# IvanIZ/BenchPush

Hardware: AMD Instinct MI355X
Metric: env-steps/sec at N=4096 envs (ship-ice-v0), 1/2/4/8 MI355X (higher is better)
Workload: dtype f64

## Files before the change

benchpush_amd/csrc/bp_capi.hip:

```cpp
#include <hip/hip_runtime.h>

#include <cstdio>
#include <cstdlib>
#include <algorithm>
#include <cstring>
#include <map>
#include <mutex>
#include <string>
#include <vector>

#include <fcntl.h>
#include <sys/file.h>
#include <sys/stat.h>
#include <unistd.h>

#include "bp_host_bd.hpp"
#include "bp_boxdelivery.hpp"
#include "bp_policy.hpp"
#include "bp_render.hpp"
#include "bp_state.hpp"
#include "bp_swath.hpp"
#include "bp_lattice.hpp"
#include "bp_track.hpp"
#include "bp_rrt.hpp"
#include "bp_gtsp.hpp"
#include "bp_asyncq.hpp"
#include "bp_replay.hpp"

typedef void (*StepKernel)(const DevParams, const DevPtrs, const double *, double *, unsigned char *, unsigned char *, double *);
typedef void (*ResidentKernel)(const DevParams *, const DevPtrs *, const double *, double *, unsigned char *, unsigned char *, double *);
typedef void (*ResetKernel)(const DevParams, const DevPtrs, const unsigned char *, double *, const int);
struct RigidKernels {
    StepKernel step = nullptr;
    StepKernel sched = nullptr;
    ResidentKernel resident = nullptr;
    ResetKernel reset = nullptr;
};

struct bp_handle {
    bp_config cfg;
    int num_envs = 0;
    long long env_offset = 0;
    int device = 0;
    int nbcap = 0;
    int num_trials = 0;
    bool loaded = false, was_reset = false;
    int *order_buf = nullptr;
    bool steps_done = false;
    bool resettle = false;
    bool damp = false;
    RigidKernels k;
    BpLaunchPolicy pol = {};
    int pair_mode = 0;
    int pair_resident = 0;
    int sched_persist = 0;
    void *pd_buf = nullptr;
    int sched_chunk = 0;
    std::string dev_lock_key;
    bool resident_auto = false;
    bool device_shared = false;
    unsigned launches = 0;
    int num_cus = 0;
    hipStream_t st_aux = nullptr;
    hipStream_t st_aux2 = nullptr;
    hipEvent_t ev_fork = nullptr, ev_join = nullptr, ev_join2 = nullptr;
    hipStream_t st_aux3 = nullptr;
    hipEvent_t ev_join3 = nullptr;
    int bd_budget = 0;
    bool async_open = false;
    int as_epoch = 0;
    int q_batch = 0;
    BdQueue q = {};
    DevParams P;
    DevPtrs D;
    std::vector<void *> allocs;
    size_t lds_bytes = 0, obs_lds_bytes = 0;
    size_t sched_lds = 0;
    std::string err;
    std::vector<double> goal_raw;
    bp_bd_config bdcfg;
    BdParams B;
    BdPtrs Q;
    size_t bd_rmap_lds = 0;
    size_t bd_lds = 0, bd_obs_lds = 0;
    std::vector<bpgeom::BdMaps> bd_maps;
    std::vector<int> bd_map_of_trial;
    bool timing = false;
    std::vector<hipEvent_t> ev;
    size_t ev_used = 0;
    unsigned long long *cost_ring = nullptr;
    int cost_n = 0;
    int *r_order = nullptr;
    unsigned *r_rgb = nullptr;
    bp_render_prim *r_prims = nullptr;
    int r_nunder = 0, r_nover = 0;
    bool r_table = false;
    unsigned long long scen_hash = 0xCBF29CE484222325ull;
    BpStateLayout st_layout;
    BpStateSeg *st_table = nullptr;
    unsigned long long st_layout_id = 0;
};
#define BP_COST_RING 1024

static int fail(bp_handle *h, int code, const std::string &msg)
{
    if (h) h->err = msg;
    return code;
}
#define HIPCHK(h, call)                                                                                       \
    do {                                                                                                      \
        hipError_t _e = (call);                                                                               \
        if (_e != hipSuccess) return fail((h), BP_EHIP, std::string(#call) + ": " + hipGetErrorString(_e));    \
    } while (0)

struct DevGuard {
    int prev = -1;
    bool changed = false, ok = true;
    explicit DevGuard(int d)
    {
        if (hipGetDevice(&prev) != hipSuccess) prev = -1;
        if (prev != d) { ok = hipSetDevice(d) == hipSuccess; changed = ok; }
    }
    ~DevGuard() { if (changed && prev >= 0) (void)hipSetDevice(prev); }
};
#define BP_DEVICE(h) DevGuard _dg((h)->device); if (!_dg.ok) return fail((h), BP_EHIP, "hipSetDevice failed")

template <typename T>
static int dalloc(bp_handle *h, T **p, size_t n, int fill_byte = 0)
{
    void *q = nullptr;
    const size_t bytes = (n ? n : 1) * sizeof(T);
    hipError_t e = hipMalloc(&q, bytes);
    if (e != hipSuccess) return fail(h, BP_ENOMEM, std::string("hipMalloc: ") + hipGetErrorString(e));
    e = hipMemset(q, fill_byte, bytes);
    if (e != hipSuccess) return fail(h, BP_EHIP, std::string("hipMemset: ") + hipGetErrorString(e));
    h->allocs.push_back(q);
    *p = (T *)q;
    return BP_OK;
}

struct DevTable { const void *src; size_t bytes; void *dev; };
template <typename T>
static DevTable dev_table(const std::vector<T> &v) { return {v.data(), sizeof(T) * v.size(), nullptr}; }
static int upload_tables(bp_handle *h, DevTable *tab, int n)
{
    for (int k = 0; k < n; k++) {
        unsigned char *q;
        if (int rc = dalloc(h, &q, tab[k].bytes)) return rc;
        tab[k].dev = q;
    }
    for (int k = 0; k < n; k++) HIPCHK(h, hipMemcpy(tab[k].dev, tab[k].src, tab[k].bytes, hipMemcpyHostToDevice));
    return BP_OK;
}

static int mvcap_for(int nbcap) { return nbcap > 192 ? nbcap : 192; }
#ifdef BP_PROF
#define BP_PROF_HOST true
#else
#define BP_PROF_HOST false
#endif
static size_t lds_bytes_for(int nbcap, bool box) { return bp_lds_map(nbcap, mvcap_for(nbcap), box, BP_PROF_HOST).total; }

static unsigned sched_yield_mask(bool solo_launch, int steps, int chunk)
{
    if (const char *ev = getenv("BP_SCHED_YMASK")) return (unsigned)strtoul(ev, nullptr, 0);
    if (!solo_launch || chunk <= 0) return 0xFFFFFFFFu;
    const int first = (2 * steps + 5 * chunk - 1) / (5 * chunk);
    return first >= 32 ? 0u : (0xFFFFFFFFu << first);
}
static int sched_image_setup(bp_handle *h)
{
    const int want = getenv("BP_SCHED_IMAGE") ? atoi(getenv("BP_SCHED_IMAGE")) : 0;
    h->P.sq_image = 0; h->D.sq_img = nullptr;
    if (!want || h->P.pair_mode == 2) return BP_OK;
    h->P.sq_img_lds = (unsigned)h->sched_lds;
    h->P.sq_img_stride = bp_img_bytes(h->P.sq_img_lds);
    unsigned char *d_img;
    int rc = dalloc(h, &d_img, (size_t)h->num_envs * h->P.sq_img_stride);
    if (rc) return rc;
    h->D.sq_img = d_img; h->P.sq_image = 1;
    return BP_OK;
}
struct ResidentLock { int fd = -1; int refs = 0; };
static std::mutex g_res_mu;
static std::map<std::string, ResidentLock> g_res_locks;

static void resident_acquire(bp_handle *h)
{
    char bus[64] = {0};
    if (hipDeviceGetPCIBusId(bus, (int)sizeof(bus), h->device) != hipSuccess) return;
    for (char *c = bus; *c; c++) if (*c == ':' || *c == '/' || *c == '.') *c = '_';
    const char *dir = getenv("BP_LOCK_DIR");
    const std::string key = std::string(dir ? dir : "/tmp") + "/benchpush_amd.resident." + bus + ".lock";
    std::lock_guard<std::mutex> g(g_res_mu);
    ResidentLock &L = g_res_locks[key];
    if (L.fd < 0) {
        const mode_t um = umask(0);
        L.fd = open(key.c_str(), O_RDWR | O_CREAT | O_CLOEXEC, 0666);
        umask(um);
        if (L.fd < 0) { g_res_locks.erase(key); return; }
// ... 215 lines not shown
    if ((rc = dalloc(h, &D.wv, EB * BP_MAXV))) return rc;
    if ((rc = dalloc(h, &D.wn, EB * BP_MAXV))) return rc;
    if ((rc = dalloc(h, &D.pv, EB * BP_MAXV))) return rc;
    if ((rc = dalloc(h, &D.bb, EB))) return rc;
    if ((rc = dalloc(h, &D.fat, EB))) return rc;
    if ((rc = dalloc(h, &D.adj, EB * BP_KADJ))) return rc;
    if ((rc = dalloc(h, &D.adjn, EB))) return rc;
    if ((rc = dalloc(h, &D.hint, EB * BP_KADJ))) return rc;
    if ((rc = dalloc(h, &D.a_key, E * BP_ACAP, 0xFF))) return rc;
    if ((rc = dalloc(h, &D.a_stamp, E * BP_ACAP))) return rc;
    if ((rc = dalloc(h, &D.a_sc, E * BP_ACAP))) return rc;
    if ((rc = dalloc(h, &D.a_h0, E * BP_ACAP))) return rc;
    if ((rc = dalloc(h, &D.a_h1, E * BP_ACAP))) return rc;
    if ((rc = dalloc(h, &D.a_d, E * BP_ACAP * 14))) return rc;
    if ((rc = dalloc(h, &D.e_lastrew, E))) return rc;
    if ((rc = dalloc(h, &D.e_lastflag, E))) return rc;
    if ((rc = dalloc(h, &D.m_acc, E * 8))) return rc;
    if ((rc = dalloc(h, &D.m_rows, E * BP_EPM_COUNT))) return rc;
    if ((rc = dalloc(h, &D.m_ring, E * BP_EPM_RING * BP_EPM_COUNT))) return rc;
    if ((rc = dalloc(h, &D.m_sum, E * BP_EPM_COUNT))) return rc;
    if ((rc = dalloc(h, &D.m_count, E))) return rc;
    if ((rc = dalloc(h, &D.m_open, E))) return rc;
    if ((rc = dalloc(h, &D.clk, (size_t)16))) return rc;
    HIPCHK(h, hipMemset(D.clk, 0, 16 * sizeof(unsigned long long)));
    D.dbg = nullptr; D.dbg_env = -1; D.prof = nullptr;
    return BP_OK;
}
static void pair_limits(bp_handle *h)
{
    auto envint = [](const char *name, int dflt) { const char *v = getenv(name); return v ? atoi(v) : dflt; };
    h->P.pair_mode = 2;
    BpLaunchPolicy &pol = h->pol;
    if (pol.pair_mode != 2)
        bp_policy_pair_limits(pol, 2LL * h->num_envs < (long long)BP_POLICY_LOOSE_FROM_HALF_ROUNDS * pol.wave_slots, h->num_envs);
    h->P.pair_solo = std::min(h->num_envs, std::max(0, envint("BP_PAIR_SOLO", pol.pair_solo)));
    h->P.pp_max_keys = std::min(30, envint("BP_PP_KEYS", 26));
    h->P.pp_max_slots = std::min(PP_NSLOT - 4, envint("BP_PP_SLOTS", 34));
    h->P.pp_max_mv = std::min(PP_MVCAP - 4, envint("BP_PP_MV", 40));
    h->P.pp_max_act = envint("BP_PP_ACT", pol.pp_max_act);
    h->P.pp_max_work = envint("BP_PP_WORK", pol.pp_max_work);
    h->P.pp_rate = envint("BP_PP_RATE", pol.pp_rate);
    h->P.pp_snake = envint("BP_PP_SNAKE", 0);
    h->P.pp_heavy_only = envint("BP_PP_HEAVY_ONLY", 0);
}
static int pair_resident_setup(bp_handle *h)
{
    HIPCHK(h, hipFuncSetAttribute((const void *)k_physics_step_schedr, hipFuncAttributeMaxDynamicSharedMemorySize, (int)h->sched_lds));
    const int pr = getenv("BP_PAIR_RESIDENT") ? atoi(getenv("BP_PAIR_RESIDENT")) : 1;
    if (pr > 0) {
        h->pair_resident = std::min(h->num_envs, h->pol.wave_slots * pr);
        if (!h->pd_buf) HIPCHK(h, hipMalloc(&h->pd_buf, sizeof(DevParams) + sizeof(DevPtrs)));
        if (!getenv("BP_PAIR_RESIDENT")) { h->resident_auto = true; resident_acquire(h); h->device_shared = resident_device_shared(h); }
    }
    return BP_OK;
}
static int sched_setup(bp_handle *h, bool maze)
{
    int rc;
    int ch = h->pol.chunk ? h->pol.chunk : (h->pair_mode == 2 ? 100 : 0);
    if (const char *ev = getenv("BP_SCHED")) ch = atoi(ev);
    if (!(ch > 0 && (h->P.steps + ch - 1) / ch <= SQ_MAXLEV && h->num_envs < (1 << 24))) return BP_OK;
    h->sched_chunk = ch;
    h->P.sq_chunk = ch; h->P.sq_levels = (h->P.steps + ch - 1) / ch;
    if (!maze) {
        h->P.sq_hold = 0;
        h->P.sq_lrpt = 0;
        h->P.sq_bw = 9000;
        h->P.sq_hyst = 1;
        h->P.sq_floor = 150;
        h->P.sq_cls = 0;
        h->P.sq_parts = 1;
        h->P.sq_part = 0;
    }
    h->P.sq_dynprio = getenv("BP_SCHED_DYNPRIO") ? atoi(getenv("BP_SCHED_DYNPRIO")) : 115;
    h->P.sq_cap = h->num_envs;
    int *d_items, *d_ctr; unsigned *d_carry; unsigned char *d_moved;
    if ((rc = dalloc(h, &d_items, (size_t)SQ_NX * SQ_MAXLEV * h->P.sq_cap))) return rc;
    if ((rc = dalloc(h, &d_ctr, (size_t)SQ_NX * (SQ_MAXLEV + 2) * 2))) return rc;
    if ((rc = dalloc(h, &d_carry, (size_t)h->num_envs * 4))) return rc;
    if ((rc = dalloc(h, &d_moved, (size_t)h->num_envs * h->nbcap))) return rc;
    h->D.sq_items = d_items; h->D.sq_ctr = d_ctr; h->D.sq_carry = d_carry; h->D.sq_moved = d_moved;
    int *d_done, *d_lev, *d_warn, *d_resc;
    if ((rc = dalloc(h, &d_resc, (size_t)1 + SQ_RESCUE))) return rc;
    h->D.sq_rescue = d_resc;
    if ((rc = dalloc(h, &d_done, (size_t)h->num_envs))) return rc;
    if ((rc = dalloc(h, &d_lev, (size_t)h->num_envs))) return rc;
    if ((rc = dalloc(h, &d_warn, (size_t)2))) return rc;
    HIPCHK(h, hipMemset(d_warn, 0, 2 * sizeof(int)));
    h->D.sq_done = d_done; h->D.sq_lev = d_lev; h->D.sq_warn = d_warn;
    unsigned *d_thr;
    if ((rc = dalloc(h, &d_thr, (size_t)1))) return rc;
    HIPCHK(h, hipMemset(d_thr, 0xFF, sizeof(unsigned)));
    h->D.sq_thr = d_thr;
    int *d_sub;
    if ((rc = dalloc(h, &d_sub, (size_t)h->num_envs))) return rc;
    h->D.sq_sub = d_sub;
    if (!maze) {
        int *d_pst;
        if ((rc = dalloc(h, &d_pst, (size_t)8))) return rc;
        HIPCHK(h, hipMemset(d_pst, 0, 8 * sizeof(int)));
        h->D.sq_pairstat = d_pst;
    }
#ifdef BP_DEBUG_PATHS
    if (const char *ev2 = getenv("BP_SCHED_DEBUG_DROP")) h->P.sq_debug = atoi(ev2);
#endif
    if (h->pair_mode == 2) pair_limits(h);
    h->sched_lds = h->pair_mode == 2 ? std::max(h->lds_bytes, (size_t)(2 * PL_HALF)) : h->lds_bytes;
    h->P.sq_ymask = sched_yield_mask(h->P.pair_mode != 2, h->P.steps, h->P.sq_chunk);
    if ((rc = sched_image_setup(h))) return rc;
    if (maze) {
        HIPCHK(h, hipFuncSetAttribute((const void *)k_physics_step_sched_maze, hipFuncAttributeMaxDynamicSharedMemorySize, (int)h->sched_lds));
        HIPCHK(h, hipFuncSetAttribute((const void *)k_physics_step_schedl_maze, hipFuncAttributeMaxDynamicSharedMemorySize, (int)h->sched_lds));
    } else {
        HIPCHK(h, hipFuncSetAttribute((const void *)k_physics_step_sched, hipFuncAttributeMaxDynamicSharedMemorySize, (int)h->sched_lds));
        HIPCHK(h, hipFuncSetAttribute((const void *)k_physics_step_schedp, hipFuncAttributeMaxDynamicSharedMemorySize, (int)h->sched_lds));
        HIPCHK(h, hipFuncSetAttribute((const void *)k_physics_step_schedl, hipFuncAttributeMaxDynamicSharedMemorySize, (int)h->sched_lds));
    }
    return h->P.pair_mode == 2 ? pair_resident_setup(h) : sched_persist_setup(h);
}
static int ship_plan(bp_handle *h, const std::vector<std::vector<bpgeom::Shape>> &trials)
{
    const int T = (int)trials.size(), nbcap = h->nbcap;
    bool plain = true;
    for (int t = 0; t < T && plain; t++)
        for (int b = 0; b < (int)trials[t].size(); b++) {
            const int kd = trials[t][b].kind;
            const int bt = (kd >> 16) & 3, grp = (kd >> 8) & 0xFF;
            if (grp != 0 || bt != (b == 0 ? 1 : 0)) { plain = false; break; }
        }
    const bool can_pair = plain && nbcap <= PP_NBCAP &&
                          ((size_t)h->num_envs + (size_t)T) * (size_t)nbcap * BP_MAXV * sizeof(d2) < (size_t)0xFFFFFFFF &&
                          ((size_t)h->num_envs + (size_t)T) * (size_t)nbcap * BP_KADJ * sizeof(unsigned long long) < (size_t)0xFFFFFFFF;
    if (int rc = device_cus(h)) return rc;
    h->pol = bp_launch_policy(h->num_envs, h->num_cus, can_pair, false);
    h->pair_mode = h->pol.pair_mode;
    if (const char *evp = getenv("BP_PAIR")) h->pair_mode = can_pair ? atoi(evp) : 0;
    if (h->pair_mode == 1) {
        h->P.pair_mode = 1;
        if (const char *evs = getenv("BP_PAIR_SNAKE")) h->P.pair_solo = atoi(evs);
        HIPCHK(h, hipFuncSetAttribute((const void *)k_physics_step_pair, hipFuncAttributeMaxDynamicSharedMemorySize, (int)(2 * PL_HALF)));
    }
    if (plain) { if (int rc = sched_setup(h, false)) return rc; }
    if (h->pair_mode == 2 && h->P.pair_mode != 2) h->pair_mode = 0;
    return BP_OK;
}
static RigidKernels rigid_kernels(const bp_handle *h, bool maze8)
{
    RigidKernels k;
    if (h->damp) { k.step = k_physics_step_damp; k.reset = k_physics_reset_damp; }
    else if (maze8) { k.step = k_physics_step_maze; k.sched = k_physics_step_sched_maze; k.resident = k_physics_step_schedl_maze; k.reset = k_physics_reset_maze; }
    else { k.step = k_physics_step; k.sched = k_physics_step_sched; k.resident = h->P.pair_mode == 2 ? k_physics_step_schedr : k_physics_step_schedl; k.reset = k_physics_reset; }
    return k;
}
static int settle_templates(bp_handle *h)
{
    hipLaunchKernelGGL(h->k.reset, dim3(h->num_trials), dim3(64), h->lds_bytes, 0, h->P, h->D, (const unsigned char *)nullptr, (double *)nullptr, 1);
    HIPCHK(h, hipGetLastError());
    HIPCHK(h, hipDeviceSynchronize());
    h->loaded = true;
    return BP_OK;
}
static int upload_trials(bp_handle *h, const std::vector<std::vector<bpgeom::Shape>> &trials, bool settle = true)
{
    const int T = (int)trials.size();
    int maxnb = 1;
    for (const auto &b : trials) maxnb = std::max(maxnb, (int)b.size());
    if (maxnb > 60000) return fail(h, BP_EINVAL, "too many bodies");
    const int nbcap = (maxnb + 7) / 8 * 8;
    h->nbcap = nbcap;
    h->num_trials = T;
    h->P.nbcap = nbcap;
    h->P.mvcap = mvcap_for(nbcap);
    h->P.num_trials = T;
    h->lds_bytes = lds_bytes_for(nbcap, h->P.env_kind == BP_ENV_BOX);
    if (h->lds_bytes > 160 * 1024) return fail(h, BP_EINVAL, "nb_cap too large for LDS");
    if (nbcap >= (1 << BP_CC_IDX_BITS)) return fail(h, BP_EINVAL, "nb_cap exceeds the candidate cache's body-index field (16384 bodies per env)");
    int rc;
    TrialTables tt;
    if ((rc = pack_trials(h, trials, nbcap, tt))) return rc;
    if ((rc = upload_trial_tables(h, tt))) return rc;
    if ((rc = alloc_env_state(h, T))) return rc;
    HIPCHK(h, hipDeviceSynchronize());
    HIPCHK(h, hipFuncSetAttribute((const void *)k_physics_step, hipFuncAttributeMaxDynamicSharedMemorySize, (int)h->lds_bytes));
    HIPCHK(h, hipFuncSetAttribute((const void *)k_physics_reset, hipFuncAttributeMaxDynamicSharedMemorySize, (int)h->lds_bytes));
    h->damp = h->P.damping_pow != 0.0;
    if (h->damp) {
        HIPCHK(h, hipFuncSetAttribute((const void *)k_physics_step_damp, hipFuncAttributeMaxDynamicSharedMemorySize, (int)h->lds_bytes));
        HIPCHK(h, hipFuncSetAttribute((const void *)k_physics_reset_damp, hipFuncAttributeMaxDynamicSharedMemorySize, (int)h->lds_bytes));
    } else if (h->P.env_kind == BP_ENV_SHIP_ICE && h->P.nkin == 1 && nbcap < 16384) {
        if ((rc = ship_plan(h, trials))) return rc;
    }
    if (!settle) return BP_OK;
    bool maze8 = !h->damp && h->P.env_kind == BP_ENV_MAZE;
    for (int v : tt.nv) if (v > 8) maze8 = false;
    if (maze8) {
        if ((rc = device_cus(h))) return rc;
        h->pol = bp_launch_policy(h->num_envs, h->num_cus, false, true);
        if ((rc = sched_setup(h, true))) return rc;
        HIPCHK(h, hipFuncSetAttribute((const void *)k_physics_step_maze, hipFuncAttributeMaxDynamicSharedMemorySize, (int)h->lds_bytes));
        HIPCHK(h, hipFuncSetAttribute((const void *)k_physics_reset_maze, hipFuncAttributeMaxDynamicSharedMemorySize, (int)h->lds_bytes));
    }
    h->k = rigid_kernels(h, maze8);
    return settle_templates(h);
}

static int state_setup(bp_handle *h)
{
    const bool box = h->P.env_kind == BP_ENV_BOX;
    const int cells = box ? h->B.SH * h->B.SW : 0;
    h->st_layout = bp_state_layout(h->D, h->Q, h->nbcap, box, cells);
    const BpStateLayout &L = h->st_layout;
    if (L.nseg >= BP_STATE_MAXSEG || (L.bytes >> 4) >= 0xFFFFFFFFull) return fail(h, BP_EINVAL, "state record layout out of range");
    unsigned long long id = bp_state_structure_id(L, h->P.env_kind, box ? h->bdcfg.task : 0, h->nbcap, cells);
    if (box) id = bp_fnv1a(&h->bdcfg, sizeof(h->bdcfg), id);
    else id = bp_fnv1a(&h->cfg, sizeof(h->cfg), id);
    h->st_layout_id = bp_fnv1a_i64((long long)h->scen_hash, id);
    int rc = dalloc(h, &h->st_table, (size_t)BP_STATE_MAXSEG);
    if (rc) return rc;
    HIPCHK(h, hipMemcpy(h->st_table, L.seg, sizeof(BpStateSeg) * L.nseg, hipMemcpyHostToDevice));
    return BP_OK;
}

static int kind_of(int ctype, int group, int btype) { return ctype | (group << 8) | (btype << 16); }

int bp_load_scenarios(bp_handle *h, int32_t T, int32_t F, int32_t V, const double *verts, const int32_t *counts,
                      const double *centres, const double *starts, const int32_t *nfloes)
{
    if (!h || T <= 0 || F < 0 || V <= 0 || !starts || !nfloes) return BP_EINVAL;
    if (h->loaded) return fail(h, BP_ESTATE, "scenarios already loaded");
    if (h->P.env_kind != BP_ENV_SHIP_ICE) return fail(h, BP_ESTATE, "handle was created for another environment");
    BP_DEVICE(h);
    using namespace bpgeom;
    std::vector<std::vector<Shape>> trials(T);
    for (int t = 0; t < T; t++) {
        std::vector<Shape> &bodies = trials[t];
        Shape ship;
        build_ship(h->cfg.ship_verts, h->cfg.num_ship_verts, starts[3 * t], starts[3 * t + 1], starts[3 * t + 2], ship);
        ship.radius = h->cfg.poly_radius; ship.e = h->cfg.elasticity; ship.u = h->cfg.friction;
        ship.kind = kind_of(1, 0, BODY_KINEMATIC);
        bodies.push_back(ship);
        if (nfloes[t] > F) return fail(h, BP_EINVAL, "nfloes > F");
        for (int f = 0; f < nfloes[t]; f++) {
            const int n = counts[(size_t)t * F + f];
            if (n < 3) continue;
            if (n > V) return fail(h, BP_EINVAL, "vertex count > V");
            Shape s;
            if (!build_floe(verts + ((size_t)t * F + f) * V * 2, n, centres[((size_t)t * F + f) * 2],
                            centres[((size_t)t * F + f) * 2 + 1], h->cfg.density, h->cfg.poly_radius, s))
                continue;
            s.radius = h->cfg.poly_radius; s.e = h->cfg.elasticity; s.u = h->cfg.friction;
            s.kind = kind_of(2, 0, BODY_DYNAMIC);
            bodies.push_back(s);
        }
    }
    const int rc_up = upload_trials(h, trials);
    return rc_up ? rc_up : state_setup(h);
}

int bp_load_maze(bp_handle *h, int32_t T, int32_t nbox, const double *centres, int32_t nwalls, const double *walls, const double *start)
{
    if (!h || T <= 0 || nbox < 0 || nwalls < 0 || nwalls > 16 || !walls || !start || (nbox > 0 && !centres)) return BP_EINVAL;
    if (h->loaded) return fail(h, BP_ESTATE, "scenarios already loaded");
    if (h->P.env_kind != BP_ENV_MAZE) return fail(h, BP_ESTATE, "handle was created for another environment");
    BP_DEVICE(h);
    using namespace bpgeom;
    const bp_config &cf = h->cfg;
    std::vector<std::vector<Shape>> trials(T);
    for (int t = 0; t < T; t++) {
        std::vector<Shape> &bodies = trials[t];
        for (int k = 0; k <= cf.num_wheels; k++) {
            Shape s;
            const double *st3 = start + 3 * (size_t)t;
            if (k == 0) build_kinematic_part(cf.ship_verts, cf.num_ship_verts, st3[0], st3[1], st3[2], s);
            else build_kinematic_part(cf.wheel_verts[k - 1], 4, st3[0], st3[1], st3[2], s);
            s.radius = cf.poly_radius; s.e = cf.elasticity; s.u = 0.0;
            s.kind = kind_of(k == 0 ? 1 : 0, 1, BODY_KINEMATIC);
            bodies.push_back(s);
        }
        for (int b = 0; b < nbox; b++) {
            const double ox = centres[((size_t)t * nbox + b) * 2], oy = centres[((size_t)t * nbox + b) * 2 + 1], sz = cf.obstacle_size;
            const double raw[8] = {ox + sz, oy + sz, ox - sz, oy + sz, ox - sz, oy - sz, ox + sz, oy - sz};
            Shape s;
            if (!build_floe(raw, 4, ox, oy, cf.density, cf.poly_radius, s)) continue;
            s.radius = cf.poly_radius; s.e = cf.elasticity; s.u = cf.friction;
            s.kind = kind_of(2, 0, BODY_DYNAMIC);
            bodies.push_back(s);
        }
        for (int w = 0; w < nwalls; w++) {
            Shape s;
            build_wall(walls[4 * w], walls[4 * w + 1], walls[4 * w + 2], walls[4 * w + 3], s);
            s.radius = cf.wall_radius; s.e = 0.5; s.u = 0.5;
            s.kind = kind_of(3, 0, BODY_STATIC);
            bodies.push_back(s);
        }
    }
    std::vector<unsigned char> wall;
    std::vector<double> norm;
    maze_maps(walls, nwalls, cf.wall_radius, cf.map_w, cf.map_h, h->P.grid_h, h->P.grid_w, cf.goal_x, cf.goal_y, wall, norm, h->goal_raw);
    int rc;
    DevTable maps[2] = {dev_table(norm), dev_table(wall)};
    if ((rc = upload_tables(h, maps, 2))) return rc;
    h->D.dist_map = (const double *)maps[0].dev; h->D.wall_map = (const unsigned char *)maps[1].dev;
    {
        std::vector<double> packed(norm.size());
        for (size_t i = 0; i < norm.size(); i++) packed[i] = wall[i] ? -norm[i] : norm[i];
        DevTable pk = dev_table(packed);
        if ((rc = upload_tables(h, &pk, 1))) return rc;
        h->D.maze_obs_map = (const double *)pk.dev;
    }
    DevTable raw = dev_table(h->goal_raw);
    if ((rc = upload_tables(h, &raw, 1))) return rc;
    h->D.goal_raw = (const double *)raw.dev;
    h->scen_hash = bp_fnv1a(wall.data(), wall.size(), h->scen_hash);
    h->scen_hash = bp_fnv1a(norm.data(), sizeof(double) * norm.size(), h->scen_hash);
    h->scen_hash = bp_fnv1a(h->goal_raw.data(), sizeof(double) * h->goal_raw.size(), h->scen_hash);
    const int rc_up = upload_trials(h, trials);
    return rc_up ? rc_up : state_setup(h);
}

int bp_get_goal_map(bp_handle *h, double *out_host, int32_t *grid_h, int32_t *grid_w)
{
    if (!h) return BP_EINVAL;
    if (h->goal_raw.empty()) return fail(h, BP_ESTATE, "no goal map (not a maze handle or not loaded)");
    if (out_host) memcpy(out_host, h->goal_raw.data(), sizeof(double) * h->goal_raw.size());
    if (grid_h) *grid_h = h->P.grid_h;
    if (grid_w) *grid_w = h->P.grid_w;
    return BP_OK;
}

__device__ __forceinline__ double bp_round2(double x)
{
    const double y = x * 100.0;
    const double e = __builtin_fma(x, 100.0, -y);
    double k = __builtin_rint(y);
    if (__builtin_fabs(y - k) == 0.5 && e != 0.0) { const double lo = __builtin_floor(y); k = (e > 0.0) ? lo + 1.0 : lo; }
    return k / 100.0;
}
__global__ __launch_bounds__(256) void k_debug_round2(const double *__restrict__ in, double *__restrict__ out, int n)
{
    const int i = blockIdx.x * blockDim.x + threadIdx.x;
    if (i < n) out[i] = bp_round2(in[i]);
}

__device__ __forceinline__ void episode_metrics_env(const DevParams &P, const DevPtrs &D, const int mode, const unsigned char *__restrict__ mask, const int env)
{
    if (env >= P.num_envs) return;
    double *a = D.m_acc + (size_t)env * 8;
    const d2 p = D.pxy[(size_t)env * P.nbcap];
    const double x = bp_round2(p.x), y = bp_round2(p.y);
    auto emit = [&](double success) {
        const double l0 = a[1], L = a[4], work = a[6];
        const double own = P.ship_mass * l0;
        double *r = D.m_rows + (size_t)env * BP_EPM_COUNT;
        r[BP_EPM_EFFICIENCY] = (success != 0.0) ? L / l0 : 0.0;
        r[BP_EPM_EFFORT] = own / (own + work);
// ... 40 lines not shown
}

#include "bp_taskmetric.hpp"

enum { MODE_ASYNC = 2, MODE_DRAIN = 3 };
struct StepOut { unsigned char *obs; double *reward; unsigned char *term, *trunc; double *info; };
struct AsyncArgs {
    int budget;
    unsigned char *ready;
    int *slices;
};
static int bd_side_streams(bp_handle *h, bool two_pass)
{
    if (!h->st_aux) HIPCHK(h, hipStreamCreateWithFlags(&h->st_aux, hipStreamNonBlocking));
    if (!h->ev_fork) HIPCHK(h, hipEventCreateWithFlags(&h->ev_fork, hipEventDisableTiming));
    if (!h->ev_join) HIPCHK(h, hipEventCreateWithFlags(&h->ev_join, hipEventDisableTiming));
    if (!two_pass) return BP_OK;
    if (!h->st_aux2) HIPCHK(h, hipStreamCreateWithFlags(&h->st_aux2, hipStreamNonBlocking));
    if (!h->ev_join2) HIPCHK(h, hipEventCreateWithFlags(&h->ev_join2, hipEventDisableTiming));
    if (!h->st_aux3) HIPCHK(h, hipStreamCreateWithFlags(&h->st_aux3, hipStreamNonBlocking));
    if (!h->ev_join3) HIPCHK(h, hipEventCreateWithFlags(&h->ev_join3, hipEventDisableTiming));
    return BP_OK;
}
static int bd_finish(bp_handle *h, const BdParams &Bx, hipStream_t s, const StepOut &out, int init = 0)
{
    const dim3 grid(init ? h->num_trials : h->num_envs);
    if (h->B.task == 1) hipLaunchKernelGGL(k_ac_finish, grid, dim3(64), h->bd_lds, s, h->P, h->D, Bx, h->Q, init, init, out.reward, out.term, out.trunc, out.info);
    else hipLaunchKernelGGL(k_bd_finish, grid, dim3(64), h->bd_lds, s, h->P, h->D, Bx, h->Q, init, init, out.reward, out.term, out.trunc, out.info);
    HIPCHK(h, hipGetLastError());
    return BP_OK;
}
static int bd_observe(bp_handle *h, const BdParams &Bx, hipStream_t s, const unsigned char *mask, unsigned char *obs)
{
    hipLaunchKernelGGL(k_bd_observe, dim3(h->num_envs), dim3(BDO_THREADS), h->bd_obs_lds, s, h->P, h->D, Bx, h->Q, mask, obs);
    HIPCHK(h, hipGetLastError());
    return BP_OK;
}
static int bd_tail(bp_handle *h, const BdParams &Bx, hipStream_t st, hipStream_t side, const StepOut &out, unsigned char *obs)
{
    if (side != st) HIPCHK(h, hipStreamWaitEvent(side, h->ev_fork, 0));
    hipLaunchKernelGGL(k_bd_robot_map, dim3(h->num_envs), dim3(BDR_THREADS), h->bd_rmap_lds, side, h->P, h->D, Bx, h->Q, 0);
    if (side != st) {
        HIPCHK(h, hipGetLastError());
        HIPCHK(h, hipEventRecord(h->ev_join, side));
    }
    if (int rc = bd_finish(h, Bx, st, out)) return rc;
    if (side != st) HIPCHK(h, hipStreamWaitEvent(st, h->ev_join, 0));
    return obs ? bd_observe(h, Bx, st, nullptr, obs) : BP_OK;
}
static int bd_physics(bp_handle *h, const BdParams &Bx, hipStream_t s)
{
    if (h->damp) hipLaunchKernelGGL(k_bd_physics_damp, dim3(h->num_envs), dim3(64), h->lds_bytes, s, h->P, h->D, Bx, h->Q);
    else hipLaunchKernelGGL(k_bd_physics, dim3(h->num_envs), dim3(64), h->lds_bytes, s, h->P, h->D, Bx, h->Q);
    HIPCHK(h, hipGetLastError());
    return BP_OK;
}
static int bd_step_two_pass(bp_handle *h, hipStream_t st, const StepOut &out, unsigned char *obs)
{
    const int E = h->num_envs;
    BdParams B0 = h->B, B1 = h->B, Bs0 = h->B, Bs1 = h->B;
    B0.budget = h->bd_budget; B0.pass = 0; B1.pass = 1; Bs0.sel_want = 0; Bs1.sel_want = 1;
    if (int rc = bd_physics(h, B0, st)) return rc;
    HIPCHK(h, hipEventRecord(h->ev_fork, st));
    HIPCHK(h, hipStreamWaitEvent(h->st_aux2, h->ev_fork, 0));
    if (!h->damp && h->B.cycle_skip > 0) {
        BdParams B1p = B1, B1s = B1;
        B1p.resume_sel = 1; B1s.resume_sel = 2;
        HIPCHK(h, hipStreamWaitEvent(h->st_aux3, h->ev_fork, 0));
        hipLaunchKernelGGL(k_bd_physics_resume, dim3(E), dim3(64), h->lds_bytes, h->st_aux3, h->P, h->D, B1p, h->Q);
        HIPCHK(h, hipGetLastError());
        HIPCHK(h, hipEventRecord(h->ev_join3, h->st_aux3));
        hipLaunchKernelGGL(k_bd_physics, dim3(E), dim3(64), h->lds_bytes, h->st_aux2, h->P, h->D, B1s, h->Q);
        HIPCHK(h, hipGetLastError());
        HIPCHK(h, hipStreamWaitEvent(h->st_aux2, h->ev_join3, 0));
        HIPCHK(h, hipGetLastError());
    } else if (int rc = bd_physics(h, B1, h->st_aux2)) return rc;
    if (int rc = bd_tail(h, Bs1, h->st_aux2, h->st_aux2, out, obs)) return rc;
    HIPCHK(h, hipEventRecord(h->ev_join2, h->st_aux2));
    if (int rc = bd_tail(h, Bs0, st, h->st_aux, out, obs)) return rc;
    HIPCHK(h, hipStreamWaitEvent(st, h->ev_join2, 0));
    return BP_OK;
}
static int bd_step_slice(bp_handle *h, int mode, const double *actions, hipStream_t st, const StepOut &out, unsigned char *obs, const AsyncArgs &as)
{
    const int E = h->num_envs;
    if (int rc = bd_side_streams(h, false)) return rc;
    const int epoch = ++h->as_epoch;
    BdParams Bp = h->B, Bl = h->B, Bt = h->B;
    Bp.pass = Bl.pass = (mode == MODE_ASYNC) ? 2 : 3;
    Bp.budget = Bl.budget = (mode == MODE_ASYNC) ? as.budget : 0;
    Bp.resume_sel = 1; Bl.resume_sel = 2; Bt.sel_want = 0;
    if (mode == MODE_ASYNC) {
        hipLaunchKernelGGL(k_bd_plan_async, dim3(E), dim3(64), h->bd_lds, st, h->P, h->D, h->B, h->Q, actions);
        HIPCHK(h, hipGetLastError());
    }
    if (h->B.cycle_skip > 0) {
        hipLaunchKernelGGL(k_bd_slice_resume, dim3(E), dim3(64), h->lds_bytes, st, h->P, h->D, Bp, h->Q, as.ready, as.slices, epoch);
        HIPCHK(h, hipGetLastError());
    } else Bl.resume_sel = 0;
    hipLaunchKernelGGL(k_bd_slice, dim3(E), dim3(64), h->lds_bytes, st, h->P, h->D, Bl, h->Q, as.ready, as.slices, epoch);
    HIPCHK(h, hipGetLastError());
    HIPCHK(h, hipEventRecord(h->ev_fork, st));
    if (int rc = bd_tail(h, Bt, st, h->st_aux, out, nullptr)) return rc;
    hipLaunchKernelGGL(k_task_metrics, dim3((E + 255) / 256), dim3(256), 0, st, h->P, h->B, h->D, h->Q, 0, (const unsigned char *)nullptr, (const unsigned char *)as.ready);
    HIPCHK(h, hipGetLastError());
    return obs ? bd_observe(h, Bt, st, nullptr, obs) : BP_OK;
}
static int launch_box(bp_handle *h, int mode, const double *actions, const unsigned char *mask, const StepOut &out, hipStream_t st, bool physics, bool raster,
                      const AsyncArgs *as, hipEvent_t e1, hipEvent_t e2)
{
    const int E = h->num_envs;
    unsigned char *obs = raster ? out.obs : nullptr;
    if (physics && mode == MODE_STEP) {
        if (h->steps_done) {
            hipLaunchKernelGGL(k_make_order, dim3(1), dim3(1024), 0, st, (const unsigned *)h->D.e_cost, h->order_buf, E, (unsigned *)nullptr);
            HIPCHK(h, hipGetLastError());
            h->D.order = h->order_buf;
        }
        h->steps_done = true;
        hipLaunchKernelGGL(k_bd_plan, dim3(E), dim3(64), h->bd_lds, st, h->P, h->D, h->B, h->Q, actions);
        HIPCHK(h, hipGetLastError());
        if (int rc = bd_side_streams(h, true)) return rc;
        if (h->bd_budget > 0) {
            if (int rc = bd_step_two_pass(h, st, out, obs)) return rc;
            obs = nullptr;
        } else {
            if (int rc = bd_physics(h, h->B, st)) return rc;
            HIPCHK(h, hipEventRecord(h->ev_fork, st));
            if (int rc = bd_tail(h, h->B, st, h->st_aux, out, nullptr)) return rc;
        }
        hipLaunchKernelGGL(k_task_metrics, dim3((E + 255) / 256), dim3(256), 0, st, h->P, h->B, h->D, h->Q, 0, (const unsigned char *)nullptr, (const unsigned char *)nullptr);
        HIPCHK(h, hipGetLastError());
    } else if (physics && (mode == MODE_ASYNC || mode == MODE_DRAIN)) {
        if (int rc = bd_step_slice(h, mode, actions, st, out, obs, *as)) return rc;
        obs = nullptr;
    } else if (physics) {
        hipLaunchKernelGGL(k_reset_copy, dim3(E), dim3(256), 0, st, h->P, h->D, mask, (double *)nullptr);
        HIPCHK(h, hipGetLastError());
        hipLaunchKernelGGL(k_bd_reset_copy, dim3(E), dim3(256), 0, st, h->P, h->D, h->B, h->Q, mask, out.info);
        HIPCHK(h, hipGetLastError());
        hipLaunchKernelGGL(k_task_metrics, dim3((E + 255) / 256), dim3(256), 0, st, h->P, h->B, h->D, h->Q, 1, mask, (const unsigned char *)nullptr);
        HIPCHK(h, hipGetLastError());
    }
    if (e1) HIPCHK(h, hipEventRecord(e1, st));
    if (obs) { if (int rc = bd_observe(h, h->B, st, mask, obs)) return rc; }
    if (e2) HIPCHK(h, hipEventRecord(e2, st));
    return BP_OK;
}
static int launch_rigid(bp_handle *h, int mode, const double *actions, const unsigned char *mask, const StepOut &out, hipStream_t st, bool physics, bool raster,
                        hipEvent_t e1, hipEvent_t e2)
{
    unsigned char *obs = out.obs, *term = out.term, *trunc = out.trunc;
    double *reward = out.reward, *info = out.info;
    if (physics) {
        if (mode == MODE_STEP && h->steps_done) {
            hipLaunchKernelGGL(k_make_order, dim3(1), dim3(1024), 0, st, (const unsigned *)h->D.e_cost, h->order_buf, h->num_envs, h->D.sq_thr);
            HIPCHK(h, hipGetLastError());
            h->D.order = h->order_buf;
        }
        if (mode == MODE_STEP) h->steps_done = true;
        if (mode == MODE_STEP && h->pair_mode == 1 && h->D.dbg == nullptr)
            hipLaunchKernelGGL(k_physics_step_pair, dim3((h->num_envs + 1) / 2), dim3(64), 2 * PL_HALF, st, h->P, h->D, actions, reward, term, trunc, info);
        else if (mode == MODE_STEP && h->sched_chunk > 0 && h->D.dbg == nullptr) {
            hipLaunchKernelGGL(k_sched_init, dim3(16), dim3(1024), 0, st, h->P, h->D);
            HIPCHK(h, hipGetLastError());
            if (h->resident_auto && (++h->launches & 63u) == 0) h->device_shared = resident_device_shared(h);
            const bool resident_ok = !(h->resident_auto && h->device_shared);
            const int resident = !resident_ok ? 0 : h->P.pair_mode == 2 ? h->pair_resident : h->sched_persist;
            if (resident > 0) {
                DevParams *Pg = (DevParams *)h->pd_buf;
                DevPtrs *Dg = (DevPtrs *)((char *)h->pd_buf + sizeof(DevParams));
                hipLaunchKernelGGL(k_store_params, dim3(1), dim3(64), 0, st, h->P, h->D, Pg, Dg);
                HIPCHK(h, hipGetLastError());
                hipLaunchKernelGGL(h->k.resident, dim3(resident), dim3(64), h->sched_lds, st, Pg, Dg, actions, reward, term, trunc, info);
            } else if (h->P.pair_mode == 2) {
                if (!h->st_aux) {
                    HIPCHK(h, hipStreamCreateWithFlags(&h->st_aux, hipStreamNonBlocking));
                    HIPCHK(h, hipEventCreateWithFlags(&h->ev_fork, hipEventDisableTiming));
                    HIPCHK(h, hipEventCreateWithFlags(&h->ev_join, hipEventDisableTiming));
                }
                if (h->P.pair_solo > 0) {
                    HIPCHK(h, hipEventRecord(h->ev_fork, st));
                    HIPCHK(h, hipStreamWaitEvent(h->st_aux, h->ev_fork, 0));
                    hipLaunchKernelGGL(k_physics_step_sched, dim3(h->P.pair_solo), dim3(64), h->sched_lds, h->st_aux, h->P, h->D, actions, reward, term, trunc, info);
                    HIPCHK(h, hipGetLastError());
                    HIPCHK(h, hipEventRecord(h->ev_join, h->st_aux));
                }
                hipLaunchKernelGGL(k_physics_step_schedp, dim3(h->num_envs * h->P.sq_levels), dim3(64), h->sched_lds, st, h->P, h->D, actions, reward, term, trunc, info);
                HIPCHK(h, hipGetLastError());
                if (h->P.pair_solo > 0) HIPCHK(h, hipStreamWaitEvent(st, h->ev_join, 0));
            } else
                hipLaunchKernelGGL(h->k.sched, dim3(h->num_envs * h->P.sq_levels), dim3(64), h->sched_lds, st, h->P, h->D, actions, reward, term, trunc, info);
            HIPCHK(h, hipGetLastError());
#ifdef BP_DEBUG_PATHS
            static const bool completion = !(getenv("BP_SCHED_COMPLETION") && atoi(getenv("BP_SCHED_COMPLETION")) == 0);
#else
            constexpr bool completion = true;
#endif
            if (completion) {
                hipLaunchKernelGGL(k_sched_scan, dim3(1), dim3(256), 0, st, h->P, h->D);
                HIPCHK(h, hipGetLastError());
                DevParams PC = h->P;
                PC.sq_mode = 1;
                hipLaunchKernelGGL(h->k.sched, dim3(std::min(h->num_envs, SQ_RESCUE)), dim3(64), h->sched_lds, st, PC, h->D, actions, reward, term, trunc, info);
            }
        }
        else if (mode == MODE_STEP)
            hipLaunchKernelGGL(h->k.step, dim3(h->num_envs), dim3(64), h->lds_bytes, st, h->P, h->D, actions, reward, term, trunc, info);
        else if (h->resettle)
            hipLaunchKernelGGL(h->k.reset, dim3(h->num_envs), dim3(64), h->lds_bytes, st, h->P, h->D, mask, info, 0);
        else
            hipLaunchKernelGGL(k_reset_copy, dim3(h->num_envs), dim3(256), 0, st, h->P, h->D, mask, info);
        HIPCHK(h, hipGetLastError());
        if (mode == MODE_STEP && h->timing && h->cost_ring && h->cost_n < BP_COST_RING) {
            hipLaunchKernelGGL(k_cost_stats, dim3(1), dim3(1024), 0, st, (const unsigned *)h->D.e_cost, h->num_envs, h->cost_ring, h->cost_n);
            HIPCHK(h, hipGetLastError());
            h->cost_n++;
        }
        hipLaunchKernelGGL(k_episode_metrics, dim3((h->num_envs + 255) / 256), dim3(256), 0, st, h->P, h->D, mode == MODE_STEP ? 0 : 1, mask);
        HIPCHK(h, hipGetLastError());
    }
    if (h->timing) HIPCHK(h, hipEventRecord(e1, st));
    if (raster && obs) {
        if (h->P.env_kind == BP_ENV_MAZE)
            hipLaunchKernelGGL(k_observe_maze, dim3(h->num_envs), dim3(OBS_THREADS), h->obs_lds_bytes, st, h->P, h->D, mask, obs);
        else
            hipLaunchKernelGGL(k_observe, dim3(h->num_envs), dim3(OBS_THREADS_SHIP), h->obs_lds_bytes, st, h->P, h->D, mask, obs);
        HIPCHK(h, hipGetLastError());
    }
    if (h->timing) HIPCHK(h, hipEventRecord(e2, st));
    return BP_OK;
}
static int launch(bp_handle *h, int mode, const double *actions, const unsigned char *mask, const StepOut &out, hipStream_t st, bool physics, bool raster,
                  const AsyncArgs *as = nullptr)
{
    hipEvent_t e0 = nullptr, e1 = nullptr, e2 = nullptr;
    if (h->timing) {
        if (h->ev_used + 3 > h->ev.size()) {
            for (int k = 0; k < 3; k++) { hipEvent_t e; HIPCHK(h, hipEventCreate(&e)); h->ev.push_back(e); }
        }
        e0 = h->ev[h->ev_used]; e1 = h->ev[h->ev_used + 1]; e2 = h->ev[h->ev_used + 2];
        h->ev_used += 3;
        HIPCHK(h, hipEventRecord(e0, st));
    }
    if (h->P.env_kind == BP_ENV_BOX) return launch_box(h, mode, actions, mask, out, st, physics, raster, as, e1, e2);
    return launch_rigid(h, mode, actions, mask, out, st, physics, raster, e1, e2);
}
static int launch_reset_untimed(bp_handle *h, const unsigned char *mask, unsigned char *obs, double *info, hipStream_t st)
{
    const bool save = h->timing;
    h->timing = false;
    const int rc = launch(h, MODE_RESET, nullptr, mask, StepOut{obs, nullptr, nullptr, nullptr, info}, st, true, true);
    h->timing = save;
    return rc;
}

int bp_reset(bp_handle *h, const uint8_t *env_mask, uint8_t *obs, double *info, void *stream)
{
    if (!h) return BP_EINVAL;
    if (!h->loaded) return fail(h, BP_ESTATE, "bp_load_scenarios has not been called");
    if (h->q_batch > 0 && env_mask != nullptr)
        return fail(h, BP_ESTATE, "bp_reset with a mask while a ready queue is open: envs are reset through bp_bd_queue_send (bp_bd_queue_close or a reset of all envs closes the queue)");
    BP_DEVICE(h);
    if (h->async_open && env_mask != nullptr) {
        hipLaunchKernelGGL(k_bd_async_cancel, dim3((h->num_envs + 255) / 256), dim3(256), 0, (hipStream_t)stream, h->Q, env_mask, h->num_envs);
        HIPCHK(h, hipGetLastError());
    }
    const int rc = launch_reset_untimed(h, env_mask, obs, info, (hipStream_t)stream);
    if (rc == BP_OK) h->was_reset = true;
    if (rc == BP_OK && env_mask == nullptr) { h->async_open = false; h->q_batch = 0; }
    return rc;
}

int bp_step(bp_handle *h, const double *actions, uint8_t *obs, double *reward, uint8_t *terminated, uint8_t *truncated,
            double *info, void *stream)
{
    if (!h || !actions) return BP_EINVAL;
    if (!h->loaded || !h->was_reset) return fail(h, BP_ESTATE, "bp_step before bp_load_scenarios/bp_reset");
    if (h->async_open) return fail(h, BP_ESTATE, "bp_step while an asynchronous slice is open (bp_bd_async_drain or a reset of all envs closes it)");
    BP_DEVICE(h);
    return launch(h, MODE_STEP, actions, nullptr, StepOut{obs, reward, terminated, truncated, info}, (hipStream_t)stream, true, true);
}

int bp_step_physics(bp_handle *h, const double *actions, double *reward, uint8_t *terminated, uint8_t *truncated, double *info,
                    void *stream)
{
    if (!h || !actions) return BP_EINVAL;
    if (!h->loaded || !h->was_reset) return fail(h, BP_ESTATE, "bp_step_physics before bp_load_scenarios/bp_reset");
    if (h->async_open) return fail(h, BP_ESTATE, "bp_step_physics while an asynchronous slice is open (bp_bd_async_drain or a reset of all envs closes it)");
    BP_DEVICE(h);
    return launch(h, MODE_STEP, actions, nullptr, StepOut{nullptr, reward, terminated, truncated, info}, (hipStream_t)stream, true, false);
}

static int async_ready(bp_handle *h, const char *what)
{
    if (!h->loaded || !h->was_reset) return fail(h, BP_ESTATE, std::string(what) + " before bp_bd_load / bp_reset");
    if (h->P.env_kind != BP_ENV_BOX || h->Q.unfin == nullptr) return fail(h, BP_EINVAL, std::string(what) + ": not a box-delivery / area-clearing handle (the steps of the other environments have a fixed length)");
    if (h->damp) return fail(h, BP_EINVAL, std::string(what) + ": handles with sim.damping != 0 have no asynchronous step");
    return BP_OK;
}

static int slice_open(bp_handle *h, bool clear_unfin, hipStream_t st)
{
    if (!h->async_open) {
        if (clear_unfin) HIPCHK(h, hipMemsetAsync(h->Q.unfin, 0, (size_t)h->num_envs, st));
        if (h->as_epoch > 0x7FFF0000) {
            HIPCHK(h, hipMemsetAsync(h->Q.rs_i, 0, sizeof(int) * 16 * (size_t)h->num_envs, st));
            h->as_epoch = 0;
        }
    }
    h->async_open = true;
    return BP_OK;
}
static int launch_drain(bp_handle *h, const StepOut &out, unsigned char *ready, int *slices, hipStream_t st)
{
    const AsyncArgs as = {0, ready, slices};
    return launch(h, MODE_DRAIN, nullptr, nullptr, out, st, true, true, &as);
}

int bp_bd_step_async(bp_handle *h, const double *actions, int32_t budget, uint8_t *obs, double *reward, uint8_t *terminated, uint8_t *truncated,
                     double *info, uint8_t *ready, int32_t *slices, void *stream)
{
    if (!h || !actions || !reward || !terminated || !truncated || !info || !ready || !slices) return BP_EINVAL;
    if (int rc = async_ready(h, "bp_bd_step_async")) return rc;
    if (budget < 1) return fail(h, BP_EINVAL, "bp_bd_step_async: budget < 1 sim step");
    if (h->q_batch > 0) return fail(h, BP_ESTATE, "bp_bd_step_async while a ready queue is open (bp_bd_queue_recv steps the envs; bp_bd_queue_close or a reset of all envs closes it)");
    BP_DEVICE(h);
    if (int rc = slice_open(h, true, (hipStream_t)stream)) return rc;
    const AsyncArgs as = {budget, ready, slices};
    return launch(h, MODE_ASYNC, actions, nullptr, StepOut{obs, reward, terminated, truncated, info}, (hipStream_t)stream, true, true, &as);
}

int bp_bd_async_drain(bp_handle *h, uint8_t *obs, double *reward, uint8_t *terminated, uint8_t *truncated, double *info, uint8_t *ready,
                      int32_t *slices, void *stream)
{
    if (!h || !reward || !terminated || !truncated || !info || !ready || !slices) return BP_EINVAL;
    if (int rc = async_ready(h, "bp_bd_async_drain")) return rc;
    if (h->q_batch > 0) return fail(h, BP_ESTATE, "bp_bd_async_drain while a ready queue is open (bp_bd_queue_close drains and closes it)");
    BP_DEVICE(h);
    if (!h->async_open) {
        HIPCHK(h, hipMemsetAsync(ready, 0, (size_t)h->num_envs, (hipStream_t)stream));
        return BP_OK;
    }
    const int rc = launch_drain(h, StepOut{obs, reward, terminated, truncated, info}, ready, slices, (hipStream_t)stream);
    if (rc == BP_OK) h->async_open = false;
    return rc;
}

int32_t bp_bd_async_open(bp_handle *h) { return (h && h->async_open) ? 1 : 0; }

static int queue_ready(bp_handle *h, const char *what)
{
    if (int rc = async_ready(h, what)) return rc;
    if (h->q_batch < 1) return fail(h, BP_ESTATE, std::string(what) + ": no ready queue is open (bp_bd_queue_open)");
    return BP_OK;
}
static int queue_action_dim(const bp_handle *h) { return h->B.action_type == 2 ? 2 : 1; }

int bp_bd_queue_open(bp_handle *h, int32_t batch, void *stream)
{
    if (!h) return BP_EINVAL;
    if (int rc = async_ready(h, "bp_bd_queue_open")) return rc;
    if (h->async_open) return fail(h, BP_ESTATE, "bp_bd_queue_open while an asynchronous slice is open (bp_bd_async_drain, bp_bd_queue_close or a reset of all envs closes it)");
    const int E = h->num_envs;
    if (batch < 1 || batch > E) return fail(h, BP_EINVAL, "bp_bd_queue_open: batch outside [1, num_envs]");
    BP_DEVICE(h);
    hipStream_t st = (hipStream_t)stream;
    if (h->q.ring == nullptr) {
        BdQueue q = {};
        int rc;
        if ((rc = dalloc(h, &q.hdr, (size_t)4))) return rc;
        if ((rc = dalloc(h, &q.where, (size_t)E))) return rc;
        if ((rc = dalloc(h, &q.fresh, (size_t)E))) return rc;
        if ((rc = dalloc(h, &q.rmask, (size_t)E))) return rc;
        if ((rc = dalloc(h, &q.win, (size_t)E))) return rc;
        if ((rc = dalloc(h, &q.actions, (size_t)E * 2))) return rc;
// ... 1337 lines not shown
```

benchpush_amd/csrc/bp_kernels.hpp:

```cpp
#pragma once
#include "bp_physics.hpp"

enum { MODE_STEP = 0, MODE_RESET = 1 };

extern __shared__ double2 bp_smem[];

__device__ __forceinline__ double poly_area_seq(const d2 *v, int n)
{
    double d1 = 0.0, d2_ = 0.0;
    for (int i = 0; i < n; i++) {
        const int p = (i - 1 + n) % n;
        d1 += v[i].x * v[p].y;
        d2_ += v[i].y * v[p].x;
    }
    return 0.5 * __builtin_fabs(d1 - d2_);
}
__device__ __forceinline__ d2 poly_centroid_seq(const d2 *v, int n)
{
    const double A = poly_area_seq(v, n);
    double sx = 0.0, sy = 0.0;
    for (int i = 0; i < n; i++) {
        const int p = (i - 1 + n) % n;
        const double u = v[i].x * v[p].y - v[p].x * v[i].y;
        sx += (v[i].x + v[p].x) * u;
// ... 612 lines not shown
                const double d = __builtin_sqrt((ca.x - cb.x) * (ca.x - cb.x) + (ca.y - cb.y) * (ca.y - cb.y));
                contrib = d * area;
                for (int q = 0; q < n; q++) prev[q] = nowv[q];
            }
            unsigned long long m = ballot(mvd);
            while (m) {
                const int l = __ffsll((long long)m) - 1;
                m &= m - 1;
                work += __shfl(contrib, l);
            }
        }
    } else {
        for (int base = 0; base < E.nb * BP_MAXV; base += 64) {
            const int q = base + lane;
            if (q < E.nb * BP_MAXV) gE(E.pv, q) = gE(E.wv, q);
        }
    }
    __syncthreads();

    store_state(P, D, L, A, env);
#ifdef BP_PRED
    if (D.prof != nullptr && lane == 0 && mode == MODE_STEP) {
        unsigned long long *o = D.prof + (size_t)env * BP_PROFN;
        o[0] = S.costp; o[1] = S.costp - pr_c200; o[2] = S.costp - pr_c100; o[3] = S.costp - pr_c50; o[4] = S.costp - pr_c10;
        o[5] = (unsigned long long)S.nmv; o[6] = (unsigned long long)__popcll(S.prev_amask); o[7] = (unsigned long long)S.nslots;
        o[8] = __builtin_amdgcn_s_memtime() - t_begin;
    }
#endif
#ifdef BP_PROF
    if (D.prof != nullptr) {
        if (lane == 0) L.prof[23] = __builtin_amdgcn_s_memtime() - _t_kernel0;
        lds_sync();
        if (lane < BP_PROFN) D.prof[(size_t)env * BP_PROFN + lane] += L.prof[lane];
    }
#endif
    const int err_any = (ballot((S.err & BP_ERR_ADJ_OVERFLOW) != 0) ? BP_ERR_ADJ_OVERFLOW : 0) |
                        (ballot((S.err & BP_ERR_ARB_OVERFLOW) != 0) ? BP_ERR_ARB_OVERFLOW : 0) |
                        (ballot((S.err & BP_ERR_LEVEL_OVERFLOW) != 0) ? BP_ERR_LEVEL_OVERFLOW : 0);
    if (lane == 0) {
        const d2 sp = gE(E.pxy, 0);
        const double sa = gE(E.ang, 0);
        D.e_stamp[env] = S.stamp; D.e_currdt[env] = S.curr_dt;
        if (mode == MODE_STEP) D.e_cost[env] = (unsigned)((__builtin_amdgcn_s_memtime() - t_begin) >> 8) + ((CHUNKED && c_sub > 0) ? D.sq_carry[(size_t)env * 4 + 3] : 0u);
        D.e_ke[env] = S.total_ke; D.e_imp[env] = S.total_imp;
        D.e_cnt[env * 4 + 0] = S.n_post; D.e_cnt[env * 4 + 1] = S.n_contact; D.e_cnt[env * 4 + 2] = S.n_first;
        if (err_any) atomicOr(&D.e_err[env], err_any);
        double total_work;
        if (mode == MODE_RESET) {
            D.e_trial[env] = trial; D.e_episode[env] = episode; D.e_nb[env] = E.nb;
            total_work = 0.0;
            D.e_total_work[env] = 0.0;
            D.e_flags[env] = 0; D.e_prevdist[env] = 0.0;
            if (KIND == BP_ENV_BOX) D.e_flags[env] = S.robot_hit;
            if (info) {
                double *o = info + (size_t)env * BP_INFO_COUNT;
                for (int k = 0; k < BP_INFO_COUNT; k++) o[k] = 0.0;
                o[BP_I_X] = sp.x; o[BP_I_Y] = sp.y; o[BP_I_THETA] = sa;
                o[BP_I_KE] = S.total_ke; o[BP_I_IMPULSE] = S.total_imp;
                o[BP_I_NPOST] = (double)S.n_post; o[BP_I_NCONTACT] = (double)S.n_contact; o[BP_I_NFIRST] = (double)S.n_first;
            }
        } else if (P.env_kind == BP_ENV_MAZE) {
            total_work = D.e_total_work[env] + work;
            D.e_total_work[env] = total_work;
            const double gdx = sp.x - P.goal_x, gdy = sp.y - P.goal_y;
            const double gd = __builtin_sqrt(gdx * gdx + gdy * gdy);
            const int goal = gd <= P.goal_reach;
            const int wall = S.wall_flag;
            const int term = goal || wall;
            int px = (int)(sp.x * P.m_to_pix), py = (int)(sp.y * P.m_to_pix);
            px = px < 0 ? 0 : (px > P.grid_w - 1 ? P.grid_w - 1 : px);
            py = py < 0 ? 0 : (py > P.grid_h - 1 ? P.grid_h - 1 : py);
            const double dist_value = D.dist_map[(size_t)py * P.grid_w + px];
            int fl = D.e_flags[env];
            double dinc = 0.0;
            if (sp.x != P.goal_x || sp.y != P.goal_y) {
                if (fl & 2) dinc = (D.e_prevdist[env] - dist_value) * P.k_increment;
                D.e_prevdist[env] = dist_value;
                fl |= 2;
            }
            D.e_flags[env] = (fl & ~1) | (wall ? 1 : 0);
            const double coll = -work;
            double rwd = P.beta * coll + dinc;
            if (S.boundary_violated || wall) rwd += P.boundary_penalty;
            int success = 0;
            if (term && !wall) { rwd += P.terminal_reward; success = 1; }
            if (reward) reward[env] = rwd;
            if (terminated) terminated[env] = (unsigned char)term;
            if (truncated) truncated[env] = 0;
            D.e_lastrew[env] = rwd; D.e_lastflag[env] = term | (success << 1);
            if (info) {
                double *o = info + (size_t)env * BP_INFO_COUNT;
                o[BP_I_X] = sp.x; o[BP_I_Y] = sp.y; o[BP_I_THETA] = sa; o[BP_I_TOTAL_WORK] = total_work; o[BP_I_WORK] = work;
                o[BP_I_COLL_REWARD] = coll; o[BP_I_SCALED_COLL] = coll * P.beta; o[BP_I_DIST_REWARD] = dinc;
                o[BP_I_SUCCESS] = success; o[BP_I_BOUNDARY] = S.boundary_violated; o[BP_I_YAW] = wall;
                o[BP_I_KE] = S.total_ke; o[BP_I_IMPULSE] = S.total_imp;
                o[BP_I_NPOST] = (double)S.n_post; o[BP_I_NCONTACT] = (double)S.n_contact; o[BP_I_NFIRST] = (double)S.n_first;
            }
        } else {
            total_work = D.e_total_work[env] + work;
            D.e_total_work[env] = total_work;
            int boundary_terminal = 0;
            if (sp.x < 0.0 && __builtin_fabs(sp.x - 0.0) >= 0.0) boundary_terminal = 1;
            if (sp.x > P.map_w && __builtin_fabs(sp.x - P.map_w) >= 0.0) boundary_terminal = 1;
            int term = 0;
            if (sp.y >= P.goal_y) term = 1;
            else if (boundary_terminal) term = 1;
            double dist_reward = 0.0;
            if (sp.y < P.goal_y) {
                const d2 r = gE(E.rot, 0);
                dist_reward = 1.0 * (r.x * 0.0 + r.y * 1.0);
            }
            const double coll = -work;
            double rwd = P.beta * coll + dist_reward;
            if (S.yaw_violated) rwd += 0.0;
            if (S.boundary_violated) rwd += P.boundary_penalty;
            int success = 0;
            if (term && !boundary_terminal) { rwd += P.terminal_reward; success = 1; }
            if (reward) reward[env] = rwd;
            if (terminated) terminated[env] = (unsigned char)term;
            if (truncated) truncated[env] = 0;
            D.e_lastrew[env] = rwd; D.e_lastflag[env] = term | (success << 1);
            if (info) {
                double *o = info + (size_t)env * BP_INFO_COUNT;
                o[BP_I_X] = sp.x; o[BP_I_Y] = sp.y; o[BP_I_THETA] = sa; o[BP_I_TOTAL_WORK] = total_work; o[BP_I_WORK] = work;
                o[BP_I_COLL_REWARD] = coll; o[BP_I_SCALED_COLL] = coll * P.beta; o[BP_I_DIST_REWARD] = dist_reward;
                o[BP_I_SUCCESS] = success; o[BP_I_BOUNDARY] = S.boundary_violated; o[BP_I_YAW] = S.yaw_violated;
                o[BP_I_KE] = S.total_ke; o[BP_I_IMPULSE] = S.total_imp;
                o[BP_I_NPOST] = (double)S.n_post; o[BP_I_NCONTACT] = (double)S.n_contact; o[BP_I_NFIRST] = (double)S.n_first;
            }
        }
    }
    return true;
}

__global__ __launch_bounds__(64, 2) void k_physics_step(const DevParams P, const DevPtrs D, const double *__restrict__ actions,
                                                     double *__restrict__ reward, unsigned char *__restrict__ terminated,
                                                     unsigned char *__restrict__ truncated, double *__restrict__ info)
{
    physics_body<MODE_STEP, 0>(P, D, actions, nullptr, reward, terminated, truncated, info, 0);
}
__global__ __launch_bounds__(64, 2) void k_physics_step_pair(const DevParams P, const DevPtrs D, const double *__restrict__ actions,
                                                          double *__restrict__ reward, unsigned char *__restrict__ terminated,
                                                          unsigned char *__restrict__ truncated, double *__restrict__ info)
{
    const int p0 = P.pair_solo ? (int)blockIdx.x : 2 * (int)blockIdx.x, p1 = P.pair_solo ? P.num_envs - 1 - (int)blockIdx.x : p0 + 1;
    const int e0 = D.order != nullptr ? D.order[p0] : p0;
    const int e1 = (p1 < P.num_envs && p1 != p0) ? (D.order != nullptr ? D.order[p1] : p1) : -1;
    PairLimits Q;
    Q.max_keys = Q.max_slots = Q.max_mv = Q.max_act = Q.max_work = 0x7FFFFFFF;
    Q.gc_slots = PP_NSLOT - 12; Q.max_rate = 0x7FFFFFFF;
    int it, score, heavy;
    pair_task<false>(P, D, actions, reward, terminated, truncated, info, e0, e1, Q, it, score, heavy, [](const int) { return false; });
}
__global__ void k_sched_init(const DevParams P, const DevPtrs D)
{
    const int tid = blockIdx.x * blockDim.x + threadIdx.x, nthr = gridDim.x * blockDim.x;
    const int nrows = P.sq_lrpt ? SQ_MAXLEV : P.sq_levels;
    for (int i = tid; i < SQ_NX * nrows * P.sq_cap; i += nthr) {
        const int xk = i / (nrows * P.sq_cap), r = i - xk * (nrows * P.sq_cap);
        D.sq_items[(size_t)xk * SQ_MAXLEV * P.sq_cap + r] = -1;
    }
    for (int i = tid; i < SQ_NX * (SQ_MAXLEV + 2) * 2; i += nthr) D.sq_ctr[i] = 0;
    for (int i = tid; i < P.num_envs; i += nthr) { D.sq_done[i] = 0; D.sq_lev[i] = 0; D.sq_sub[i] = 0; }
}
#define SQ_RESCUE 256
__global__ __launch_bounds__(256) void k_sched_scan(const DevParams P, const DevPtrs D)
{
    __shared__ int cnt;
    if (threadIdx.x == 0) cnt = 0;
    __syncthreads();
    if (sq_ld(sq_finished(D)) < P.num_envs)
        for (int e = threadIdx.x; e < P.num_envs; e += blockDim.x)
            if (D.sq_done[e] == 0) { const int pos = atomicAdd(&cnt, 1); if (pos < SQ_RESCUE) D.sq_rescue[1 + pos] = e; }
    __syncthreads();
    if (threadIdx.x == 0) {
        D.sq_rescue[0] = min(cnt, SQ_RESCUE);
        if (cnt > SQ_RESCUE) atomicOr(&D.e_err[0], BP_ERR_SCHED_TIMEOUT);
    }
}
struct SchedTraceCtx { unsigned long long trw; int idle, first, home; };
template <int KIND>
__device__ __forceinline__ int sched_paired_block(const DevParams &P, const DevPtrs &D, const double *__restrict__ actions, double *__restrict__ reward,
                                                  unsigned char *__restrict__ terminated, unsigned char *__restrict__ truncated, double *__restrict__ info,
                                                  const int pe0, const int pe1, const int x, const bool first)
{
    const int lane = lane_id();
    {
        __builtin_amdgcn_fence(__ATOMIC_ACQUIRE, "agent");
        PairLimits Q;
        Q.max_keys = P.pp_max_keys; Q.max_slots = P.pp_max_slots; Q.max_mv = P.pp_max_mv; Q.max_act = P.pp_max_act; Q.max_work = P.pp_max_work;
        Q.gc_slots = P.pp_max_slots - 6; Q.max_rate = P.pp_rate;
        int it_half = 0, score_half = 0, heavy_half = 0;
        auto behind = [&](const int level) -> bool {
            int y = 0;
            if (lane == 0) y = (((P.sq_ymask >> level) & 1u) && sq_someone_behind(P, D, x, level)) ? 1 : 0;
            return __builtin_amdgcn_readfirstlane(y) != 0;
        };
        const int st_half = pair_task<true>(P, D, actions, reward, terminated, truncated, info, pe0, pe1, Q, it_half, score_half, heavy_half, behind);
        const int st0 = __builtin_amdgcn_readlane(st_half, 0), st1 = __builtin_amdgcn_readlane(st_half, 32);
        const int it0 = __builtin_amdgcn_readlane(it_half, 0), it1 = __builtin_amdgcn_readlane(it_half, 32);
        const int sc0 = __builtin_amdgcn_readlane(score_half, 0), sc1 = __builtin_amdgcn_readlane(score_half, 32);
        const int hv0 = __builtin_amdgcn_readlane(heavy_half, 0), hv1 = __builtin_amdgcn_readlane(heavy_half, 32);
        pair_gsync();
        __builtin_amdgcn_fence(__ATOMIC_RELEASE, "agent");
        const int nfin = (st0 == 1 ? 1 : 0) + (st1 == 1 ? 1 : 0);
        if (lane == 0) {
            if (st0 == 1) D.sq_done[pe0] = 1;
            if (st1 == 1) D.sq_done[pe1] = 1;
            if (nfin) atomicAdd(sq_finished(D), nfin);
        }
        const bool pk0 = st0 == 2, pk1 = st1 == 2;
        if (lane == 0 && D.sq_pairstat != nullptr) {
            atomicAdd(&D.sq_pairstat[first ? 0 : 1], 1);
            if (nfin) atomicAdd(&D.sq_pairstat[2], nfin);
        }
        if (!pk0 && !pk1) return -1;
        const bool c0 = pk0 && hv0 && (!(pk1 && hv1) || sc0 >= sc1), c1 = !c0 && pk1 && hv1;
        if (lane == 0) {
            if (pk0 && !c0) { D.sq_lev[pe0] = it0 / P.sq_chunk; sq_push(P, D, x + (hv0 ? 0 : 8), it0 / P.sq_chunk, pe0); }
            if (pk1 && !c1) { D.sq_lev[pe1] = it1 / P.sq_chunk; sq_push(P, D, x + (hv1 ? 0 : 8), it1 / P.sq_chunk, pe1); }
            if (D.sq_pairstat != nullptr) {
                if (c0 || c1) atomicAdd(&D.sq_pairstat[3], 1);
                const int qh = ((pk0 && !c0 && hv0) ? 1 : 0) + ((pk1 && !c1 && hv1) ? 1 : 0), ql = ((pk0 && !c0 && !hv0) ? 1 : 0) + ((pk1 && !c1 && !hv1) ? 1 : 0);
                if (qh) atomicAdd(&D.sq_pairstat[4], qh);
                if (ql) atomicAdd(&D.sq_pairstat[5], ql);
            }
        }
        if (!c0 && !c1) return -1;
        __syncthreads();
        return ((c0 ? pe0 : pe1) | (3 << 24)) | (((c0 ? it0 : it1) / P.sq_chunk) << 26);
    }
}
template <int KIND>
__device__ __forceinline__ void sched_solo_block(const DevParams &P, const DevPtrs &D, const double *__restrict__ actions, double *__restrict__ reward,
                                                 unsigned char *__restrict__ terminated, unsigned char *__restrict__ truncated, double *__restrict__ info,
                                                 const int item, const int lev, const int x, const bool completion, const SchedTraceCtx &T)
{
    const int lane = lane_id();
    const int env = item & 0xFFFFFF;
    if ((item >> 24) == 3) __builtin_amdgcn_s_setprio(3);
    else if ((item >> 24) == 1) __builtin_amdgcn_s_setprio(1);
    __builtin_amdgcn_fence(__ATOMIC_ACQUIRE, "agent");
#ifdef BP_SCHED_TRACE
    const unsigned long long _tr0 = __builtin_amdgcn_s_memrealtime();
#endif
    int lev_out = lev + 1, light_out = 0;
    const bool done = physics_body<MODE_STEP, KIND, true>(P, D, actions, nullptr, reward, terminated, truncated, info, 0, 0, env, lev, x, &lev_out, completion,
                                                          &light_out, P.sq_hold != 0 && (item >> 24) == 3);
    __syncthreads();
    __builtin_amdgcn_fence(__ATOMIC_RELEASE, "agent");
#ifdef BP_SCHED_TRACE
    if (lane == 0 && D.prof != nullptr) {
        const unsigned long long _tr1 = __builtin_amdgcn_s_memrealtime();
        const unsigned long long idx = atomicAdd(&D.prof[0], 1ull);
        unsigned long long *o = D.prof + 8 + 4 * idx;
        o[0] = (unsigned long long)(unsigned)env | ((unsigned long long)(unsigned)lev << 32) | ((unsigned long long)(unsigned)(done ? 255 : lev_out) << 40) | ((unsigned long long)(unsigned)T.home << 48) |
               ((unsigned long long)(unsigned)x << 52) | ((unsigned long long)(T.first ? 1u : 0u) << 56);
        unsigned hwid;
        asm volatile("s_getreg_b32 %0, hwreg(HW_REG_HW_ID)" : "=s"(hwid));
        o[1] = _tr0; o[2] = _tr1;
        o[3] = ((_tr0 - T.trw) << 32) | ((unsigned long long)(hwid & 0xFFFFu) << 16) | (unsigned long long)(unsigned)min(T.idle, 65535);
    }
#endif
    if (lane == 0) {
        if (done) { D.sq_done[env] = 1; if (!completion) atomicAdd(sq_finished(D), 1); }
        else {
            D.sq_lev[env] = lev_out;
            if (!(P.sq_debug && env == 1 && lev_out == 1)) sq_push(P, D, x + ((P.pair_mode == 2 && !completion && light_out) ? 8 : 0), lev_out, item);
        }
    }
}
template <int KIND, int ROLE = 0>
__device__ __forceinline__ bool sched_body(const DevParams &P, const DevPtrs &D, const double *__restrict__ actions,
                                           double *__restrict__ reward, unsigned char *__restrict__ terminated,
                                           unsigned char *__restrict__ truncated, double *__restrict__ info, const int bid_in = -1)
{
    const int lane = lane_id();
    const int home = sq_xcc_id();
#ifdef BP_SCHED_TRACE
    const unsigned long long _trw = __builtin_amdgcn_s_memrealtime();
    int _tr_idle = 0;
#endif
    int item = -1, lev = 0, x = home;
    int pe0 = -1, pe1 = -1;
    const bool completion = P.sq_mode == 1;
    const bool pairing = ROLE == 1 && KIND == BP_ENV_SHIP_ICE && P.pair_mode == 2 && !completion;
    const int npairs = pairing ? (P.num_envs - P.pair_solo + 1) / 2 : 0;
    const int nfirst_part = (ROLE == 0 && P.sq_parts > 1) ? (P.num_envs - P.sq_part + P.sq_parts - 1) / P.sq_parts : 0;
    const int bid = (bid_in >= 0) ? bid_in : (ROLE == 1) ? (int)blockIdx.x + P.pair_solo
                  : (P.sq_parts > 1) ? (((int)blockIdx.x < nfirst_part) ? (int)blockIdx.x * P.sq_parts + P.sq_part : P.num_envs + (int)blockIdx.x)
                  : (int)blockIdx.x;
    const int nfirst = pairing ? P.pair_solo + npairs : P.num_envs;
    if (completion) {
        if ((int)blockIdx.x >= D.sq_rescue[0]) return true;
        item = D.sq_rescue[1 + blockIdx.x]; lev = D.sq_lev[item];
        if (lane == 0) atomicAdd(&D.sq_warn[1], 1);
    } else if (pairing && bid >= P.pair_solo && bid < nfirst) {
        const int p0 = P.pp_snake ? bid : P.pair_solo + 2 * (bid - P.pair_solo), p1 = P.pp_snake ? P.num_envs - 1 - (bid - P.pair_solo) : p0 + 1;
        pe0 = D.order != nullptr ? D.order[p0] : p0;
        pe1 = (p1 < P.num_envs && p1 != p0) ? (D.order != nullptr ? D.order[p1] : p1) : -1;
        if (lane == 0) atomicAdd(sq_started(D), pe1 >= 0 ? 2 : 1);
    } else if (bid < nfirst) {
        const int pos = bid;
        const int cls = (pos < P.num_envs / 4) ? 3 : (pos < P.num_envs / 2) ? 1 : 0;
        item = (D.order != nullptr ? D.order[pos] : pos) | (cls << 24);
        if (lane == 0) atomicAdd(sq_started(D), 1);
    } else {
        int kind = 0, mate = -1;
        if (lane == 0) {
// ... 2 lines not shown
                item = sq_pop(P, D, home, lev, kind);
                if (item < 0 && (idle & 3) == 3)
                    for (int o = 1; o < 8 && item < 0; o++) { const int y = (home + o) & 7; item = sq_pop(P, D, y, lev, kind); if (item >= 0) x = y; }
#ifdef BP_SCHED_TRACE
                _tr_idle = idle;
#endif
                if (item >= 0 || sq_ld(sq_finished(D)) >= P.num_envs || sq_ld(sq_abort(D)) != 0) break;
                if (idle > limit) { if (atomicExch(sq_abort(D), 1) == 0) atomicAdd(&D.sq_warn[0], 1); break; }
                for (int q = 0; q < 4; q++) __builtin_amdgcn_s_sleep(127);
            }
            if (ROLE == 1 && item >= 0 && kind == 1 && sq_ld(sq_waiting(D, x + 8)) > 0)
                for (int l = lev; l < P.sq_levels && mate < 0; l++) mate = sq_pop_level(P, D, x + 8, l);
        }
        item = __builtin_amdgcn_readfirstlane(item); lev = __builtin_amdgcn_readfirstlane(lev); x = __builtin_amdgcn_readfirstlane(x);
        mate = __builtin_amdgcn_readfirstlane(mate);
        if (item < 0) return true;
        if (mate >= 0) { pe0 = item & 0xFFFFFF; pe1 = mate & 0xFFFFFF; item = -1; }
    }
    SchedTraceCtx T;
    T.trw = 0ull; T.idle = 0; T.first = bid < nfirst ? 1 : 0; T.home = home;
#ifdef BP_SCHED_TRACE
    T.trw = _trw; T.idle = _tr_idle;
#endif
    if (ROLE == 1 && pe0 >= 0) {
        const int r = sched_paired_block<KIND>(P, D, actions, reward, terminated, truncated, info, pe0, pe1, x, bid < nfirst);
        if (r < 0) return false;
        item = r & 0x3FFFFFF; lev = (int)((unsigned)r >> 26);
    }
    sched_solo_block<KIND>(P, D, actions, reward, terminated, truncated, info, item, lev, x, completion, T);
    return false;
}
__device__ __forceinline__ int *sq_nextpos(const DevPtrs &D) { return sq_row(D, 2, SQ_MAXLEV + 1); }
template <int KIND, int ROLE>
__device__ __forceinline__ void sched_resident(const DevParams *Pg, const DevPtrs *Dg, const double *__restrict__ actions,
                                               double *__restrict__ reward, unsigned char *__restrict__ terminated,
                                               unsigned char *__restrict__ truncated, double *__restrict__ info)
{
    for (;;) {
        unsigned long long pa = (unsigned long long)Pg, da = (unsigned long long)Dg;
        asm volatile("" : "+s"(pa), "+s"(da));
        const DevParams &P = *(const DevParams *)(const __attribute__((address_space(4))) DevParams *)pa;
        const DevPtrs &D = *(const DevPtrs *)(const __attribute__((address_space(4))) DevPtrs *)da;
        __builtin_amdgcn_s_setprio(0);
        const bool pairing = ROLE == 1 && KIND == BP_ENV_SHIP_ICE && P.pair_mode == 2;
        const int nfirst = pairing ? P.pair_solo + (P.num_envs - P.pair_solo + 1) / 2 : P.num_envs;
        int bid = nfirst;
        if (lane_id() == 0 && sq_ld(sq_nextpos(D)) < nfirst) bid = min(atomicAdd(sq_nextpos(D), 1), nfirst);
        bid = __builtin_amdgcn_readfirstlane(bid);
        if (sched_body<KIND, ROLE>(P, D, actions, reward, terminated, truncated, info, bid)) return;
        __syncthreads();
    }
}
#ifndef BP_SCHED_WAVES
#define BP_SCHED_WAVES 2
#endif
__global__ __launch_bounds__(64, BP_SCHED_WAVES) void k_physics_step_schedl(const DevParams *Pg, const DevPtrs *Dg, const double *__restrict__ actions,
                                                             double *__restrict__ reward, unsigned char *__restrict__ terminated,
                                                             unsigned char *__restrict__ truncated, double *__restrict__ info)
{
    sched_resident<0, 0>(Pg, Dg, actions, reward, terminated, truncated, info);
}
__global__ __launch_bounds__(64, 2) void k_physics_step_schedl_maze(const DevParams *Pg, const DevPtrs *Dg, const double *__restrict__ actions,
                                                                 double *__restrict__ reward, unsigned char *__restrict__ terminated,
                                                                 unsigned char *__restrict__ truncated, double *__restrict__ info)
{
    sched_resident<BP_ENV_MAZE, 0>(Pg, Dg, actions, reward, terminated, truncated, info);
}
#define BP_UNIFORM_PTR(T, p) ((T)(((unsigned long long)(unsigned)__builtin_amdgcn_readfirstlane((int)((unsigned long long)(p) >> 32)) << 32) | \
                                  (unsigned long long)(unsigned)__builtin_amdgcn_readfirstlane((int)(unsigned long long)(p))))
template <int KIND>
__device__ __attribute__((noinline)) int sched_fn_pair(const DevParams *Pg_, const DevPtrs *Dg_, const double *actions_, double *reward_, unsigned char *terminated_,
                                                       unsigned char *truncated_, double *info_, int pe0, int pe1, int x, int first)
{
    const DevParams &P = *(const DevParams *)(const __attribute__((address_space(4))) DevParams *)BP_UNIFORM_PTR(unsigned long long, Pg_);
    const DevPtrs &D = *(const DevPtrs *)(const __attribute__((address_space(4))) DevPtrs *)BP_UNIFORM_PTR(unsigned long long, Dg_);
    return sched_paired_block<KIND>(P, D, BP_UNIFORM_PTR(const double *, actions_), BP_UNIFORM_PTR(double *, reward_), BP_UNIFORM_PTR(unsigned char *, terminated_),
                                    BP_UNIFORM_PTR(unsigned char *, truncated_), BP_UNIFORM_PTR(double *, info_), __builtin_amdgcn_readfirstlane(pe0),
                                    __builtin_amdgcn_readfirstlane(pe1), __builtin_amdgcn_readfirstlane(x), __builtin_amdgcn_readfirstlane(first) != 0);
}
template <int KIND>
__device__ __attribute__((noinline)) void sched_fn_solo(const DevParams *Pg_, const DevPtrs *Dg_, const double *actions_, double *reward_, unsigned char *terminated_,
                                                        unsigned char *truncated_, double *info_, int item, int lev, int x)
{
    const DevParams &P = *(const DevParams *)(const __attribute__((address_space(4))) DevParams *)BP_UNIFORM_PTR(unsigned long long, Pg_);
    const DevPtrs &D = *(const DevPtrs *)(const __attribute__((address_space(4))) DevPtrs *)BP_UNIFORM_PTR(unsigned long long, Dg_);
    SchedTraceCtx T;
    T.trw = 0ull; T.idle = 0; T.first = 0; T.home = 0;
    sched_solo_block<KIND>(P, D, BP_UNIFORM_PTR(const double *, actions_), BP_UNIFORM_PTR(double *, reward_), BP_UNIFORM_PTR(unsigned char *, terminated_),
                           BP_UNIFORM_PTR(unsigned char *, truncated_), BP_UNIFORM_PTR(double *, info_), __builtin_amdgcn_readfirstlane(item),
                           __builtin_amdgcn_readfirstlane(lev), __builtin_amdgcn_readfirstlane(x), false, T);
}
template <int KIND>
__device__ __forceinline__ void sched_resident_pairing(const DevParams *Pg, const DevPtrs *Dg, const double *__restrict__ actions,
                                                       double *__restrict__ reward, unsigned char *__restrict__ terminated,
                                                       unsigned char *__restrict__ truncated, double *__restrict__ info)
{
    const int lane = lane_id();
    const int home = sq_xcc_id();
    for (;;) {
        unsigned long long pa = (unsigned long long)Pg, da = (unsigned long long)Dg;
        asm volatile("" : "+s"(pa), "+s"(da));
        const DevParams &P = *(const DevParams *)(const __attribute__((address_space(4))) DevParams *)pa;
        const DevPtrs &D = *(const DevPtrs *)(const __attribute__((address_space(4))) DevPtrs *)da;
        __builtin_amdgcn_s_setprio(0);
        const int npairs = (P.num_envs - P.pair_solo + 1) / 2, nfirst = P.pair_solo + npairs;
        int bid = nfirst;
        if (lane == 0 && sq_ld(sq_nextpos(D)) < nfirst) bid = min(atomicAdd(sq_nextpos(D), 1), nfirst);
        bid = __builtin_amdgcn_readfirstlane(bid);
        int item = -1, lev = 0, x = home, pe0 = -1, pe1 = -1;
        if (bid >= P.pair_solo && bid < nfirst) {
            const int p0 = P.pp_snake ? bid : P.pair_solo + 2 * (bid - P.pair_solo), p1 = P.pp_snake ? P.num_envs - 1 - (bid - P.pair_solo) : p0 + 1;
            pe0 = D.order != nullptr ? D.order[p0] : p0;
            pe1 = (p1 < P.num_envs && p1 != p0) ? (D.order != nullptr ? D.order[p1] : p1) : -1;
            if (lane == 0) atomicAdd(sq_started(D), pe1 >= 0 ? 2 : 1);
        } else if (bid < nfirst) {
            const int cls = (bid < P.num_envs / 4) ? 3 : (bid < P.num_envs / 2) ? 1 : 0;
            item = (D.order != nullptr ? D.order[bid] : bid) | (cls << 24);
            if (lane == 0) atomicAdd(sq_started(D), 1);
        } else {
            int kind = 0, mate = -1;
            if (lane == 0) {
                const int limit = P.sq_debug ? 64 : (1 << 20);
                for (int idle = 0;; idle++) {
                    item = sq_pop(P, D, home, lev, kind);
                    if (item < 0 && (idle & 3) == 3)
                        for (int o = 1; o < 8 && item < 0; o++) { const int y = (home + o) & 7; item = sq_pop(P, D, y, lev, kind); if (item >= 0) x = y; }
                    if (item >= 0 || sq_ld(sq_finished(D)) >= P.num_envs || sq_ld(sq_abort(D)) != 0) break;
                    if (idle > limit) { if (atomicExch(sq_abort(D), 1) == 0) atomicAdd(&D.sq_warn[0], 1); break; }
                    for (int q = 0; q < 4; q++) __builtin_amdgcn_s_sleep(127);
                }
                if (item >= 0 && kind == 1 && sq_ld(sq_waiting(D, x + 8)) > 0)
                    for (int l = lev; l < P.sq_levels && mate < 0; l++) mate = sq_pop_level(P, D, x + 8, l);
            }
            item = __builtin_amdgcn_readfirstlane(item); lev = __builtin_amdgcn_readfirstlane(lev); x = __builtin_amdgcn_readfirstlane(x);
            mate = __builtin_amdgcn_readfirstlane(mate);
            if (item < 0) return;
            if (mate >= 0) { pe0 = item & 0xFFFFFF; pe1 = mate & 0xFFFFFF; item = -1; }
        }
        if (pe0 >= 0) {
            const int r = sched_fn_pair<KIND>(Pg, Dg, actions, reward, terminated, truncated, info, pe0, pe1, x, bid < nfirst ? 1 : 0);
            if (r < 0) { __syncthreads(); continue; }
            item = r & 0x3FFFFFF; lev = (int)((unsigned)r >> 26);
        }
        sched_fn_solo<KIND>(Pg, Dg, actions, reward, terminated, truncated, info, item, lev, x);
        __syncthreads();
    }
}
__global__ __launch_bounds__(64, 2) void k_physics_step_schedr(const DevParams *Pg, const DevPtrs *Dg, const double *__restrict__ actions,
                                                            double *__restrict__ reward, unsigned char *__restrict__ terminated,
                                                            unsigned char *__restrict__ truncated, double *__restrict__ info)
{
    sched_resident_pairing<0>(Pg, Dg, actions, reward, terminated, truncated, info);
}
__global__ void k_store_params(const DevParams P, const DevPtrs D, DevParams *Pg, DevPtrs *Dg)
{
    static_assert(sizeof(DevParams) % 4 == 0 && sizeof(DevPtrs) % 4 == 0, "copied as 32-bit words");
    const unsigned *sp = (const unsigned *)&P, *sd = (const unsigned *)&D;
    for (unsigned i = threadIdx.x; i < sizeof(DevParams) / 4; i += blockDim.x) ((unsigned *)Pg)[i] = sp[i];
    for (unsigned i = threadIdx.x; i < sizeof(DevPtrs) / 4; i += blockDim.x) ((unsigned *)Dg)[i] = sd[i];
}
__global__ __launch_bounds__(64, BP_SCHED_WAVES) void k_physics_step_sched(const DevParams P, const DevPtrs D, const double *__restrict__ actions,
                                                           double *__restrict__ reward, unsigned char *__restrict__ terminated,
                                                           unsigned char *__restrict__ truncated, double *__restrict__ info)
{
    sched_body<0, 0>(P, D, actions, reward, terminated, truncated, info);
}
__global__ __launch_bounds__(64, 2) void k_physics_step_schedp(const DevParams P, const DevPtrs D, const double *__restrict__ actions,
                                                            double *__restrict__ reward, unsigned char *__restrict__ terminated,
                                                            unsigned char *__restrict__ truncated, double *__restrict__ info)
{
    sched_body<0, 1>(P, D, actions, reward, terminated, truncated, info);
}
__global__ __launch_bounds__(64, 2) void k_physics_step_sched_maze(const DevParams P, const DevPtrs D, const double *__restrict__ actions,
                                                                double *__restrict__ reward, unsigned char *__restrict__ terminated,
                                                                unsigned char *__restrict__ truncated, double *__restrict__ info)
{
    sched_body<BP_ENV_MAZE>(P, D, actions, reward, terminated, truncated, info);
}
__global__ __launch_bounds__(64, 2) void k_physics_reset(const DevParams P, const DevPtrs D, const unsigned char *__restrict__ mask,
                                                      double *__restrict__ info, const int tmpl)
{
    physics_body<MODE_RESET, 0>(P, D, nullptr, mask, nullptr, nullptr, nullptr, tmpl ? nullptr : info, tmpl);
}
__global__ __launch_bounds__(64, 2) void k_physics_step_damp(const DevParams P, const DevPtrs D, const double *__restrict__ actions,
                                                          double *__restrict__ reward, unsigned char *__restrict__ terminated,
                                                          unsigned char *__restrict__ truncated, double *__restrict__ info)
{
    physics_body<MODE_STEP, 0, false, true>(P, D, actions, nullptr, reward, terminated, truncated, info, 0);
}
__global__ __launch_bounds__(64, 2) void k_physics_reset_damp(const DevParams P, const DevPtrs D, const unsigned char *__restrict__ mask,
                                                           double *__restrict__ info, const int tmpl)
{
    physics_body<MODE_RESET, 0, false, true>(P, D, nullptr, mask, nullptr, nullptr, nullptr, tmpl ? nullptr : info, tmpl);
}
__global__ __launch_bounds__(64, 2) void k_physics_step_maze(const DevParams P, const DevPtrs D, const double *__restrict__ actions,
                                                          double *__restrict__ reward, unsigned char *__restrict__ terminated,
                                                          unsigned char *__restrict__ truncated, double *__restrict__ info)
{
    physics_body<MODE_STEP, BP_ENV_MAZE>(P, D, actions, nullptr, reward, terminated, truncated, info, 0);
}
__global__ __launch_bounds__(64, 2) void k_physics_reset_maze(const DevParams P, const DevPtrs D, const unsigned char *__restrict__ mask,
                                                           double *__restrict__ info, const int tmpl)
{
    physics_body<MODE_RESET, BP_ENV_MAZE>(P, D, nullptr, mask, nullptr, nullptr, nullptr, tmpl ? nullptr : info, tmpl);
}
__global__ __launch_bounds__(64, 2) void k_bd_settle(const DevParams P, const DevPtrs D, const unsigned char *__restrict__ mask,
                                                  double *__restrict__ info, const int tmpl)
{
    physics_body<MODE_RESET, BP_ENV_BOX>(P, D, nullptr, mask, nullptr, nullptr, nullptr, tmpl ? nullptr : info, tmpl);
}
__global__ __launch_bounds__(64, 2) void k_bd_settle_damp(const DevParams P, const DevPtrs D, const unsigned char *__restrict__ mask,
                                                       double *__restrict__ info, const int tmpl)
{
    physics_body<MODE_RESET, BP_ENV_BOX, false, true>(P, D, nullptr, mask, nullptr, nullptr, nullptr, tmpl ? nullptr : info, tmpl);
}

__global__ __launch_bounds__(1024) void k_make_order(const unsigned *__restrict__ cost, int *__restrict__ order, int n, unsigned *__restrict__ thr)
{
    __shared__ unsigned hist[257];
    __shared__ unsigned smax;
    const int tid = threadIdx.x;
    if (tid < 257) hist[tid] = 0;
    if (tid == 0) smax = 1;
    __syncthreads();
    unsigned mx = 0;
    for (int i = tid; i < n; i += blockDim.x) mx = max(mx, cost[i]);
    atomicMax(&smax, mx);
    __syncthreads();
    const unsigned long long m = smax;
    for (int i = tid; i < n; i += blockDim.x) {
        const unsigned b = 255u - (unsigned)(((unsigned long long)cost[i] * 255ull) / m);
        atomicAdd(&hist[b], 1u);
    }
    __syncthreads();
    if (tid == 0) {
        unsigned acc = 0;
        const unsigned rank = (unsigned)max(1, n / 256);
        int tb = -1;
        for (int b = 0; b < 256; b++) { const unsigned c = hist[b]; hist[b] = acc; acc += c; if (tb < 0 && acc >= rank) tb = b; }
        if (thr != nullptr) thr[0] = (unsigned)((m * (unsigned long long)(255 - max(tb, 0))) / 255ull);
    }
    __syncthreads();
    for (int i = tid; i < n; i += blockDim.x) {
        const unsigned b = 255u - (unsigned)(((unsigned long long)cost[i] * 255ull) / m);
        const unsigned pos = atomicAdd(&hist[b], 1u);
        order[pos] = i;
    }
}


__global__ __launch_bounds__(1024) void k_cost_stats(const unsigned *__restrict__ cost, int n, unsigned long long *__restrict__ ring, int slot)
{
    __shared__ unsigned long long ssum;
    __shared__ unsigned smax;
    if (threadIdx.x == 0) { ssum = 0ull; smax = 0u; }
    __syncthreads();
    unsigned long long s = 0ull;
    unsigned mx = 0u;
    for (int i = threadIdx.x; i < n; i += blockDim.x) { const unsigned c = cost[i]; s += c; mx = max(mx, c); }
    atomicAdd(&ssum, s);
    atomicMax(&smax, mx);
    __syncthreads();
    if (threadIdx.x == 0) { ring[2 * slot] = ssum; ring[2 * slot + 1] = smax; }
}

template <typename T>
__device__ __forceinline__ void copy_span(T *dst, const T *src, size_t n, int tid, int nt)
{
    for (size_t i = tid; i < n; i += nt) dst[i] = src[i];
}
__global__ __launch_bounds__(256) void k_reset_copy(const DevParams P, const DevPtrs D, const unsigned char *__restrict__ mask,
                                                    double *__restrict__ info)
{
    const int env = blockIdx.x;
    if (mask != nullptr && mask[env] == 0) return;
    const int tid = threadIdx.x, nt = blockDim.x;
    const int episode = D.e_episode[env] + 1;
    const int trial = (int)(((long long)P.env_offset + env + episode) % P.num_trials);
    const size_t nb = P.nbcap, d = (size_t)env * nb, s = (size_t)(P.num_envs + trial) * nb;
    copy_span(D.pxy + d, D.pxy + s, nb, tid, nt);
    copy_span(D.ang + d, D.ang + s, nb, tid, nt);
    copy_span(D.rot + d, D.rot + s, nb, tid, nt);
    copy_span(D.velv + d, D.velv + s, nb, tid, nt);
    copy_span(D.velw + d, D.velw + s, nb, tid, nt);
    copy_span(D.velb + d, D.velb + s, nb, tid, nt);
    copy_span(D.wv + d * BP_MAXV, D.wv + s * BP_MAXV, nb * BP_MAXV, tid, nt);
    copy_span(D.wn + d * BP_MAXV, D.wn + s * BP_MAXV, nb * BP_MAXV, tid, nt);
    copy_span(D.pv + d * BP_MAXV, D.pv + s * BP_MAXV, nb * BP_MAXV, tid, nt);
    copy_span(D.bb + d, D.bb + s, nb, tid, nt);
    copy_span(D.fat + d, D.fat + s, nb, tid, nt);
    copy_span((unsigned long long *)(D.adj + d * BP_KADJ), (const unsigned long long *)(D.adj + s * BP_KADJ), nb * BP_KADJ / 4, tid, nt);
    copy_span(D.hint + d * BP_KADJ, D.hint + s * BP_KADJ, nb * BP_KADJ, tid, nt);
    copy_span((unsigned long long *)(D.adjn + d), (const unsigned long long *)(D.adjn + s), nb / 8, tid, nt);
    const size_t ad = (size_t)env * BP_ACAP, as = (size_t)(P.num_envs + trial) * BP_ACAP;
    copy_span(D.a_key + ad, D.a_key + as, BP_ACAP, tid, nt);
    copy_span(D.a_stamp + ad, D.a_stamp + as, BP_ACAP, tid, nt);
    copy_span(D.a_sc + ad, D.a_sc + as, BP_ACAP, tid, nt);
    copy_span(D.a_h0 + ad, D.a_h0 + as, BP_ACAP, tid, nt);
    copy_span(D.a_h1 + ad, D.a_h1 + as, BP_ACAP, tid, nt);
    copy_span(D.a_d + ad * 14, D.a_d + as * 14, (size_t)BP_ACAP * 14, tid, nt);
    if (tid == 0) {
        const int se = P.num_envs + trial;
        D.e_trial[env] = trial; D.e_episode[env] = episode; D.e_nb[env] = D.e_nb[se];
        D.e_stamp[env] = D.e_stamp[se]; D.e_currdt[env] = D.e_currdt[se];
        D.e_total_work[env] = 0.0; D.e_ke[env] = D.e_ke[se]; D.e_imp[env] = D.e_imp[se];
        D.e_flags[env] = 0; D.e_prevdist[env] = 0.0;
        for (int q = 0; q < 4; q++) D.e_cnt[env * 4 + q] = D.e_cnt[se * 4 + q];
        if (D.e_err[se]) atomicOr(&D.e_err[env], D.e_err[se]);
        if (info) {
            double *o = info + (size_t)env * BP_INFO_COUNT;
            for (int q = 0; q < BP_INFO_COUNT; q++) o[q] = 0.0;
            o[BP_I_X] = D.pxy[s].x; o[BP_I_Y] = D.pxy[s].y; o[BP_I_THETA] = D.ang[s];
            o[BP_I_KE] = D.e_ke[se]; o[BP_I_IMPULSE] = D.e_imp[se];
            o[BP_I_NPOST] = (double)D.e_cnt[se * 4 + 0]; o[BP_I_NCONTACT] = (double)D.e_cnt[se * 4 + 1]; o[BP_I_NFIRST] = (double)D.e_cnt[se * 4 + 2];
        }
    }
}

#define OBS_THREADS 256
#ifndef OBS_THREADS_SHIP
#define OBS_THREADS_SHIP 512
#endif
#define OBS_MAXCAND 96
#define OBS_CHUNK 32
#ifndef OBS_SNAP_Y
#define OBS_SNAP_Y 1e-6
#define OBS_SNAP_X 1e-6
#endif

__device__ __forceinline__ bool pip_arrays(const double *xp, const double *yp, int n, double x, double y)
{
    const double eps = 1e-12;
    unsigned l_cross = 0, r_cross = 0;
    double x1 = xp[n - 1] - x, y1 = yp[n - 1] - y;
    for (int i = 0; i < n; i++) {
        const double x0 = xp[i] - x, y0 = yp[i] - y;
        if ((-eps < x0 && x0 < eps) && (-eps < y0 && y0 < eps)) return true;
        const bool up = (y0 > 0) != (y1 > 0), dn = (y0 < 0) != (y1 < 0);
        if (up || dn) {
            const double num = x0 * y1 - x1 * y0, den = y1 - y0;
            const bool pos = (num > 0 && den > 0) || (num < 0 && den < 0);
            const bool neg = (num > 0 && den < 0) || (num < 0 && den > 0);
            if (up && pos) r_cross++;
            if (dn && neg) l_cross++;
        }
        x1 = x0; y1 = y0;
    }
    if ((r_cross & 1) != (l_cross & 1)) return true;
    return (r_cross & 1) != 0;
}

__device__ __forceinline__ long long to_u16(double v) { return ((long long)v) & 0xFFFF; }

__device__ __forceinline__ bool clip_line(long long W, long long H, long long &x1, long long &y1, long long &x2, long long &y2)
{
    const long long right = W - 1, bottom = H - 1;
    int c1 = (x1 < 0) + (x1 > right) * 2 + (y1 < 0) * 4 + (y1 > bottom) * 8;
    int c2 = (x2 < 0) + (x2 > right) * 2 + (y2 < 0) * 4 + (y2 > bottom) * 8;
    if ((c1 & c2) == 0 && (c1 | c2) != 0) {
        long long a;
        if (c1 & 12) {
            a = c1 < 8 ? 0 : bottom;
            x1 += (long long)((double)(a - y1) * (double)(x2 - x1) / (double)(y2 - y1));
            y1 = a;
            c1 = (x1 < 0) + (x1 > right) * 2;
        }
        if (c2 & 12) {
            a = c2 < 8 ? 0 : bottom;
            x2 += (long long)((double)(a - y2) * (double)(x2 - x1) / (double)(y2 - y1));
            y2 = a;
            c2 = (x2 < 0) + (x2 > right) * 2;
        }
        if ((c1 & c2) == 0 && (c1 | c2) != 0) {
            if (c1) {
                a = c1 == 1 ? 0 : right;
                y1 += (long long)((double)(a - x1) * (double)(y2 - y1) / (double)(x2 - x1));
                x1 = a;
                c1 = 0;
            }
            if (c2) {
                a = c2 == 1 ? 0 : right;
                y2 += (long long)((double)(a - x2) * (double)(y2 - y1) / (double)(x2 - x1));
                x2 = a;
                c2 = 0;
            }
        }
    }
    return (c1 | c2) == 0;
}

struct LineSpec { int valid; long long x0, y0, dx, dy, sx, sy; int vert; };

__device__ __forceinline__ LineSpec make_line(long long W, long long H, long long x1, long long y1, long long x2, long long y2)
{
    LineSpec s;
    s.valid = 1;
    if ((unsigned long long)x1 >= (unsigned long long)W || (unsigned long long)x2 >= (unsigned long long)W ||
        (unsigned long long)y1 >= (unsigned long long)H || (unsigned long long)y2 >= (unsigned long long)H) {
        if (!clip_line(W, H, x1, y1, x2, y2)) { s.valid = 0; }
    }
    long long dx = x2 - x1, dy = y2 - y1;
    long long px = x1, py = y1;
    if (dx < 0) { dx = -dx; dy = -dy; px = x2; py = y2; }
    long long sy = 1;
    if (dy < 0) { dy = -dy; sy = -1; }
    s.x0 = px; s.y0 = py; s.dx = dx; s.dy = dy; s.sx = 1; s.sy = sy; s.vert = dy > dx;
    return s;
}
__device__ __forceinline__ bool on_line(const LineSpec &s, long long x, long long y)
{
    if (!s.valid) return false;
    const long long ax = (x - s.x0) * s.sx, ay = (y - s.y0) * s.sy;
    long long t, m, dmaj, dmin;
    if (!s.vert) { t = ax; m = ay; dmaj = s.dx; dmin = s.dy; }
    else { t = ay; m = ax; dmaj = s.dy; dmin = s.dx; }
    if (t < 0 || t > dmaj || m < 0 || m > dmin) return false;
    if (dmaj == 0) return m == 0;
    const long long mt = (2 * dmin * t + dmaj - 1) / (2 * dmaj);
    return m == mt;
}

__device__ __forceinline__ d2 poly_centroid_xy(const double *x, const double *y, int n)
{
    double d1 = 0.0, d2_ = 0.0;
    for (int i = 0; i < n; i++) {
        const int p = (i == 0) ? n - 1 : i - 1;
        d1 += x[i] * y[p];
        d2_ += y[i] * x[p];
    }
    const double A = 0.5 * __builtin_fabs(d1 - d2_);
    double sx = 0.0, sy = 0.0;
    for (int i = 0; i < n; i++) {
        const int p = (i == 0) ? n - 1 : i - 1;
        const double u = x[i] * y[p] - x[p] * y[i];
        sx += (x[i] + x[p]) * u;
        sy += (y[i] + y[p]) * u;
    }
    const double f = 1.0 / (6.0 * A);
    return mk2(__builtin_fabs(f * sx), __builtin_fabs(f * sy));
}

__device__ __forceinline__ unsigned obs_upto(int k) { return k <= 0 ? 0u : (k >= 4 ? 0xFFFFFFFFu : ((1u << (8 * k)) - 1u)); }
__device__ __forceinline__ void obs_or_bytes(unsigned *img32, int b0, int b1, unsigned char flag)
{
    for (int w = b0 >> 2; w <= (b1 >> 2); w++) {
        const int lo = max(b0, 4 * w) - 4 * w, hi = min(b1, 4 * w + 3) - 4 * w;
        atomicOr(&img32[w], (obs_upto(hi + 1) & ~obs_upto(lo)) & ((unsigned)flag * 0x01010101u));
    }
}

template <bool OR_BITS>
__device__ __forceinline__ void raster_row_convex(const double *xp, const double *yp, int n, int gi, int c0, int c1, unsigned char *row,
                                                  unsigned char flag, const int off = 0)
{
    const double y = (double)gi;
    bool slow = false;
    int ncross = 0, ia = 0, ib = 0;
    double y1 = yp[n - 1] - y;
    for (int i = 0; i < n; i++) {
        const double y0 = yp[i] - y;
        if (__builtin_fabs(y0) < OBS_SNAP_Y) slow = true;
        if ((y0 > 0) != (y1 > 0)) {
            if (ncross == 0) ia = i; else ib = i;
            ncross++;
        }
        y1 = y0;
    }
    double xa = 0.0, xb = 0.0;
    if (ncross == 2) {
        const int pa = (ia == 0) ? n - 1 : ia - 1, pb = (ib == 0) ? n - 1 : ib - 1;
        { const double x0 = xp[ia], y0 = yp[ia] - y, x1 = xp[pa], y1_ = yp[pa] - y; xa = x0 - y0 * ((x1 - x0) / (y1_ - y0)); }
        { const double x0 = xp[ib], y0 = yp[ib] - y, x1 = xp[pb], y1_ = yp[pb] - y; xb = x0 - y0 * ((x1 - x0) / (y1_ - y0)); }
    }
    if (slow || (ncross != 0 && ncross != 2)) {
        for (int gj = c0; gj <= c1; gj++)
            if (pip_arrays(xp, yp, n, (double)gj, y)) { if (OR_BITS) obs_or_bytes((unsigned *)row, off + gj, off + gj, flag); else row[gj] = flag; }
        return;
    }
    if (ncross == 0) return;
    const double xl = fmin(xa, xb), xr = fmax(xa, xb);
    int first, last;
    {
        const double rl = __builtin_rint(xl);
        if (__builtin_fabs(xl - rl) < OBS_SNAP_X) first = pip_arrays(xp, yp, n, rl, y) ? (int)rl : (int)rl + 1;
        else first = (int)__builtin_ceil(xl);
        const double rr = __builtin_rint(xr);
        if (__builtin_fabs(xr - rr) < OBS_SNAP_X) last = pip_arrays(xp, yp, n, rr, y) ? (int)rr : (int)rr - 1;
        else last = (int)__builtin_floor(xr);
    }
    first = max(first, c0); last = min(last, c1);
    if (OR_BITS) { if (last >= first) obs_or_bytes((unsigned *)row, off + first, off + last, flag); return; }
    unsigned char *p = row + first, *const pe = row + last + 1;
    while (p < pe && ((uintptr_t)p & 3u)) *p++ = flag;
    const unsigned w4 = (unsigned)flag * 0x01010101u;
    for (; p + 4 <= pe; p += 4) *(unsigned *)p = w4;
    while (p < pe) *p++ = flag;
}


#ifdef BP_PROF
#define OPROF(k) { if (tid == 0 && D.prof != nullptr) D.prof[(size_t)env * BP_PROFN + 56 + (k)] = __builtin_amdgcn_s_memtime(); }
#else
#define OPROF(k)
#endif
#define OBS_F_OCC 1u
#define OBS_F_SHIP 2u
#define OBS_F_LINE 4u
#define OBS_F_HEAD 8u

__global__ __launch_bounds__(OBS_THREADS_SHIP, 8) void k_observe(const DevParams P, const DevPtrs D, const unsigned char *__restrict__ mask,
                                                         unsigned char *__restrict__ obs)
{
    const int env = blockIdx.x;
    if (mask != nullptr && mask[env] == 0) return;
    const int tid = threadIdx.x;
    const int nbcap = P.nbcap;
    const size_t eb = (size_t)env * nbcap;
    const int nb = D.e_nb[env];
    const d2 *wv = D.wv + eb * BP_MAXV;
    const int *nv = D.sc_nv + (size_t)D.e_trial[env] * nbcap;
    const int Hg = P.grid_h, Wg = P.grid_w, LH = P.obs_h, LW = P.obs_w;
    const int npix = LH * LW;

    extern __shared__ double2 obs_smem[];
    unsigned char *s_img = (unsigned char *)obs_smem;
    unsigned char *s_edt = s_img + ((npix + 15) & ~15);
    double *s_px = (double *)(s_edt + ((LH + 15) & ~15));
    double *s_py = s_px + OBS_CHUNK * BP_MAXV;
    __shared__ int s_npass;
    __shared__ unsigned short s_list[OBS_MAXCAND];
    __shared__ int s_bbx[OBS_CHUNK][4];
    __shared__ unsigned char s_cn[OBS_CHUNK];
    __shared__ double s_fr[BP_MAX_SHIP_VERTS], s_fc[BP_MAX_SHIP_VERTS];
    __shared__ int s_fcnt, s_fbb[4];
    OPROF(0)
    const double4 bb_first = D.bb[eb + min(1 + tid, nbcap - 1)];
    if (tid == 0) s_npass = 0;
    for (int w = tid; w < (npix + 3) / 4; w += OBS_THREADS_SHIP) ((unsigned *)s_img)[w] = 0u;
    __syncthreads();
    OPROF(1)

    const d2 sp = D.pxy[eb];
    const d2 srot = D.rot[eb];
    const double m2gx = (double)Wg / P.map_w, m2gy = (double)Hg / P.map_h;
    const int wx = (int)(sp.x * m2gx);
    const int wy = (int)((sp.y + P.vshift) * m2gy);
    const int gi0 = (int)((double)(0 + wy) - ((double)LH / 2)), gj0 = (int)((double)(0 + wx) - ((double)LW / 2));
    const int gi1 = gi0 + LH - 1, gj1 = gj0 + LW - 1;
    const int bh = (int)(P.map_h * P.m_to_pix), bw = (int)(P.map_w * P.m_to_pix);
    for (int s = 1 + tid; s < nb; s += OBS_THREADS_SHIP) {
        const double4 b = (s == 1 + tid) ? bb_first : D.bb[eb + s];
        if (__builtin_floor(b.y * P.m_to_pix) - 1.0 > (double)gi1 || __builtin_ceil(b.w * P.m_to_pix) + 1.0 < (double)gi0 ||
            __builtin_floor(b.x * P.m_to_pix) - 1.0 > (double)gj1 || __builtin_ceil(b.z * P.m_to_pix) + 1.0 < (double)gj0) continue;
        const int slot = atomicAdd(&s_npass, 1);
        if (slot < OBS_MAXCAND) s_list[slot] = (unsigned short)s;
    }
    LineSpec line;
    long long hpx, hpy;
    {
        const double ch = srot.x, sh = srot.y;
        if (tid == 0) {
            int cnt = 0;
            double rmin = BP_INF, rmax = -BP_INF, cmin = BP_INF, cmax = -BP_INF;
            for (int i = 0; i < P.num_ship_verts; i++) {
                const double vx = P.ship_verts[i][0] * ch + P.ship_verts[i][1] * -sh + sp.x;
                const double vy = P.ship_verts[i][0] * sh + P.ship_verts[i][1] * ch + sp.y;
                const double gx = vx * m2gx, gy = vy * m2gy;
                if (gy < 0 || gy >= Hg || gx < 0 || gx >= Wg) continue;
                s_fr[cnt] = gy; s_fc[cnt] = gx; cnt++;
                rmin = fmin(rmin, gy); rmax = fmax(rmax, gy); cmin = fmin(cmin, gx); cmax = fmax(cmax, gx);
            }
            s_fcnt = cnt;
            if (cnt > 0) {
                s_fbb[0] = (int)(long long)fmax(0.0, rmin); s_fbb[1] = (int)(long long)__builtin_ceil(rmax);
                s_fbb[2] = (int)(long long)fmax(0.0, cmin); s_fbb[3] = (int)(long long)__builtin_ceil(cmax);
            }
        }
        line.valid = 0; hpx = hpy = 0;
        if (tid >= 64 && tid < 128) {
            const double hx = P.ship_head[0] * ch + P.ship_head[1] * -sh + sp.x, hy = P.ship_head[0] * sh + P.ship_head[1] * ch + sp.y;
            const double tx = P.ship_tail[0] * ch + P.ship_tail[1] * -sh + sp.x, ty = P.ship_tail[0] * sh + P.ship_tail[1] * ch + sp.y;
            hpx = to_u16(hx * m2gx); hpy = to_u16(hy * m2gy);
            const long long tpx = to_u16(tx * m2gx), tpy = to_u16(ty * m2gy);
            line = make_line(Wg, Hg, hpx, hpy, tpx, tpy);
            hpx = hpx < 0 ? 0 : (hpx > Wg - 1 ? Wg - 1 : hpx);
            hpy = hpy < 0 ? 0 : (hpy > Hg - 1 ? Hg - 1 : hpy);
        }
    }
    const double g2m = P.map_h / (double)Hg;
    for (int li = tid; li < LH; li += OBS_THREADS_SHIP) {
        const int gi = gi0 + li;
        unsigned char e = 255;
        if (gi >= 0 && gi < Hg) {
            double dd = P.goal_y - gi * g2m;
            if (dd < 0) dd = 0;
            e = (unsigned char)((dd / P.goal_y) * 255);
        }
        s_edt[li] = e;
    }
    __syncthreads();
    OPROF(2)
    const int ncand_all = min(s_npass, OBS_MAXCAND);
    if (tid == 0 && s_npass > OBS_MAXCAND) atomicOr(&D.e_err[env], BP_ERR_LEVEL_OVERFLOW);
    for (int cbase = 0; cbase < ncand_all; cbase += OBS_CHUNK) {
    const int ncand = min(OBS_CHUNK, ncand_all - cbase);
    for (int idx = tid; idx < ncand * BP_MAXV; idx += OBS_THREADS_SHIP) {
        const int k = idx / BP_MAXV, q = idx - k * BP_MAXV;
        const int s = s_list[cbase + k];
        const d2 v = wv[(size_t)s * BP_MAXV + q];
        const int n = nv[s];
        if (q == 0) s_cn[k] = (unsigned char)n;
        if (q < n) { s_px[idx] = v.x; s_py[idx] = v.y; }
    }
    __syncthreads();
    OPROF(3)
    if (tid < ncand) {
        const int k = tid;
        const int n = s_cn[k];
        double *xp = s_px + k * BP_MAXV, *yp = s_py + k * BP_MAXV;
        bool keep = true;
        double d1 = 0.0, d2_ = 0.0, sx = 0.0, sy = 0.0;
        double rmin = BP_INF, rmax = -BP_INF, cmin = BP_INF, cmax = -BP_INF;
        double xq = xp[n - 1], yq = yp[n - 1];
        for (int i = 0; i < n; i++) {
            const double xi = xp[i], yi = yp[i];
            const double a = xi * yq, b = yi * xq;
            d1 += a; d2_ += b;
            const double u = a - xq * yi;
            sx += (xi + xq) * u;
            sy += (yi + yq) * u;
            const double r = yi * P.m_to_pix, cc = xi * P.m_to_pix;
            xp[i] = cc; yp[i] = r;
            rmin = fmin(rmin, r); rmax = fmax(rmax, r); cmin = fmin(cmin, cc); cmax = fmax(cmax, cc);
            xq = xi; yq = yi;
        }
        {
            const double A = 0.5 * __builtin_fabs(d1 - d2_);
            const double f = 1.0 / (6.0 * A);
            const double cx = __builtin_fabs(__builtin_fabs(f * sx)), cy = __builtin_fabs(__builtin_fabs(f * sy));
            if (__builtin_fabs(sp.x - cx) > P.obs_range || __builtin_fabs(sp.y - cy) > P.obs_range) keep = false;
        }
        long long minr = (long long)fmax(0.0, rmin), maxr = (long long)__builtin_ceil(rmax);
        long long minc = (long long)fmax(0.0, cmin), maxc = (long long)__builtin_ceil(cmax);
        if (maxr > bh - 1) maxr = bh - 1;
        if (maxc > bw - 1) maxc = bw - 1;
        if (maxr < gi0 || minr > gi1 || maxc < gj0 || minc > gj1 || maxr < minr || maxc < minc) keep = false;
        if (keep) {
            s_bbx[k][0] = (int)max(minr, (long long)gi0); s_bbx[k][1] = (int)min(maxr, (long long)gi1);
            s_bbx[k][2] = (int)max(minc, (long long)gj0); s_bbx[k][3] = (int)min(maxc, (long long)gj1);
        } else { s_bbx[k][0] = 0; s_bbx[k][1] = -1; s_bbx[k][2] = 0; s_bbx[k][3] = -1; }
    }
    __syncthreads();
    OPROF(4)
    {
        int TPC = OBS_THREADS_SHIP / OBS_CHUNK;
        while (TPC * ncand * 2 <= OBS_THREADS_SHIP) TPC *= 2;
        const int k = tid / TPC, sub = tid - k * TPC;
        if (k < ncand && s_bbx[k][1] >= s_bbx[k][0]) {
            const int c0 = max(s_bbx[k][2], 0), c1 = min(s_bbx[k][3], Wg - 1);
            const int n = s_cn[k];
            const double *xp = s_px + k * BP_MAXV, *yp = s_py + k * BP_MAXV;
            for (int gi = s_bbx[k][0] + sub; gi <= s_bbx[k][1]; gi += TPC) {
                if (gi < 0 || gi >= Hg) continue;
                raster_row_convex<false>(xp, yp, n, gi, c0, c1, s_img + (gi - gi0) * LW - gj0, (unsigned char)OBS_F_OCC);
            }
        }
    }
    __syncthreads();
    }
    OPROF(5)
    if (tid < 64) {
        if (s_fcnt > 0) {
            const int r0 = max(s_fbb[0], max(gi0, 0)), r1 = min(s_fbb[1], min(gi1, Hg - 1));
            const int c0 = max(s_fbb[2], max(gj0, 0)), c1 = min(s_fbb[3], min(gj1, Wg - 1));
            if (c1 >= c0)
                for (int gi = r0 + tid; gi <= r1; gi += 64)
                    raster_row_convex<true>(s_fc, s_fr, s_fcnt, gi, c0, c1, s_img, (unsigned char)OBS_F_SHIP, (gi - gi0) * LW - gj0);
        }
    } else if (tid < 128) {
        const int l2 = tid - 64;
        if (line.valid) {
            const long long dmaj = line.vert ? line.dy : line.dx, dmin = line.vert ? line.dx : line.dy;
            for (long long t = l2; t <= dmaj; t += 64) {
                const long long mt = (dmaj == 0) ? 0 : ((dmaj < 32768 && dmin < 32768)
                                         ? (long long)(((unsigned)(2 * dmin * t) + (unsigned)dmaj - 1u) / (unsigned)(2 * dmaj))
                                         : (2 * dmin * t + dmaj - 1) / (2 * dmaj));
                const long long ax = line.vert ? mt : t, ay = line.vert ? t : mt;
                const long long gj = line.x0 + ax * line.sx, gi = line.y0 + ay * line.sy;
                if (gi >= gi0 && gi <= gi1 && gj >= gj0 && gj <= gj1 && gi >= 0 && gi < Hg && gj >= 0 && gj < Wg) {
                    const int b = ((int)gi - gi0) * LW + ((int)gj - gj0);
                    obs_or_bytes((unsigned *)s_img, b, b, (unsigned char)OBS_F_LINE);
                }
            }
        }
        if (l2 == 0 && hpy >= gi0 && hpy <= gi1 && hpx >= gj0 && hpx <= gj1) {
            const int b = ((int)hpy - gi0) * LW + ((int)hpx - gj0);
            obs_or_bytes((unsigned *)s_img, b, b, (unsigned char)OBS_F_HEAD);
        }
    }
    __syncthreads();
    OPROF(6)
    const size_t plane = (size_t)npix;
    unsigned *o32 = (unsigned *)(obs + (size_t)env * BP_OBS_C * plane);
    const int nwords = npix / 4;
    const int WP = LW / 2, G = OBS_THREADS_SHIP / WP;
    const int g = tid / WP, j = tid - g * WP;
    const int ljlo = max(0, -gj0), ljhi = min(LW - 1, Wg - 1 - gj0);
    if (g < G) {
        const int bs = LW - 4 * j;
        const unsigned mlo = obs_upto(bs);
        const unsigned mA = mlo & obs_upto(ljhi - 4 * j + 1) & ~obs_upto(ljlo - 4 * j);
        const unsigned mB = ~mlo & obs_upto(bs + ljhi + 1) & ~obs_upto(bs + ljlo);
        for (int rp = g; 2 * rp < LH; rp += G) {
            const int w = rp * WP + j;
            const unsigned f = ((const unsigned *)s_img)[w];
            const int giA = gi0 + 2 * rp, giB = giA + 1;
            const unsigned rowA = (giA >= 0 && giA < Hg) ? 0xFFFFFFFFu : 0u, rowB = (giB >= 0 && giB < Hg) ? 0xFFFFFFFFu : 0u;
            const unsigned inb = (rowA & mA) | (rowB & mB);
            const unsigned e2 = ((const unsigned short *)s_edt)[rp];
            const unsigned eA = (e2 & 0xFFu) * 0x01010101u, eB = (e2 >> 8) * 0x01010101u;
            const unsigned e = ((eA & mlo) | (eB & ~mlo)) & inb;
            const unsigned ship = (f >> 1) & 0x01010101u, ln = (f >> 2) & 0x01010101u, hd = (f >> 3) & 0x01010101u;
            o32[w] = inb & (0x7F7F7F7Fu + ship * 0x80u);
            o32[nwords + w] = e | ~inb;
            o32[2 * nwords + w] = inb & ((ln & ~hd) * 127u + hd * 255u);
            o32[3 * nwords + w] = (f & 0x01010101u) * 255u;
        }
    }
    OPROF(7)
}

#define MZ_MAXBOX 64
__global__ __launch_bounds__(OBS_THREADS) void k_observe_maze(const DevParams P, const DevPtrs D, const unsigned char *__restrict__ mask,
                                                              unsigned char *__restrict__ obs)
{
    const int env = blockIdx.x;
    if (mask != nullptr && mask[env] == 0) return;
    const int tid = threadIdx.x;
    const int nbcap = P.nbcap;
    const size_t eb = (size_t)env * nbcap;
    const int nb = D.e_nb[env];
    const size_t tb = (size_t)D.e_trial[env] * nbcap;
    const d2 *wv = D.wv + eb * BP_MAXV;
    const int *nv = D.sc_nv + tb;
    const int *kind = D.sc_kind + tb;
    const int Hg = P.grid_h, Wg = P.grid_w, LH = P.obs_h, LW = P.obs_w;
    const int infl = (LW > LH ? LW : LH) / 2;
    const int IH = LH + infl, IW = LW + infl;
    const int nwords = (IH * IW + 31) / 32;

    extern __shared__ double2 obs_smem[];
    unsigned *s_box = (unsigned *)obs_smem;
    unsigned *s_foot = s_box + nwords;
    double *s_px = (double *)(s_foot + ((nwords + 1) & ~1));
    double *s_py = s_px + MZ_MAXBOX * 4;
    __shared__ int s_nbox;
    __shared__ int s_bbx[MZ_MAXBOX][4];
    __shared__ double s_fr[BP_MAX_SHIP_VERTS], s_fc[BP_MAX_SHIP_VERTS];
    __shared__ int s_fcnt, s_fbb[4];
    if (tid == 0) s_nbox = 0;
    for (int w = tid; w < nwords; w += OBS_THREADS) { s_box[w] = 0u; s_foot[w] = 0u; }
    __syncthreads();

    const d2 sp = D.pxy[eb];
    const double sa = D.ang[eb];
    const d2 srot = D.rot[eb];
    const int wx = (int)(sp.x * P.m_to_pix), wy = (int)(sp.y * P.m_to_pix);
    const int gi0 = (int)((double)(0 + wy) - ((double)IH / 2)), gj0 = (int)((double)(0 + wx) - ((double)IW / 2));
    const int gi1 = gi0 + IH - 1, gj1 = gj0 + IW - 1;
    for (int s = tid; s < nb; s += OBS_THREADS) {
        if (kind_ctype(kind[s]) != 2) continue;
        const int n = nv[s];
        const d2 *v = wv + (size_t)s * BP_MAXV;
        double rmin = v[0].y * P.m_to_pix, rmax = rmin, cmin = v[0].x * P.m_to_pix, cmax = cmin;
        for (int i = 1; i < n; i++) {
            const double r = v[i].y * P.m_to_pix, cc = v[i].x * P.m_to_pix;
            rmin = fmin(rmin, r); rmax = fmax(rmax, r); cmin = fmin(cmin, cc); cmax = fmax(cmax, cc);
        }
        long long minr = (long long)fmax(0.0, rmin), maxr = (long long)__builtin_ceil(rmax);
        long long minc = (long long)fmax(0.0, cmin), maxc = (long long)__builtin_ceil(cmax);
        if (maxr > Hg - 1) maxr = Hg - 1;
        if (maxc > Wg - 1) maxc = Wg - 1;
        if (maxr < gi0 || minr > gi1 || maxc < gj0 || minc > gj1 || maxr < minr || maxc < minc) continue;
        const int slot = atomicAdd(&s_nbox, 1);
        if (slot < MZ_MAXBOX && n <= 4) {
            s_bbx[slot][0] = (int)max(minr, (long long)gi0); s_bbx[slot][1] = (int)min(maxr, (long long)gi1);
            s_bbx[slot][2] = (int)max(minc, (long long)gj0); s_bbx[slot][3] = (int)min(maxc, (long long)gj1);
            for (int i = 0; i < 4; i++) { s_px[slot * 4 + i] = v[i].x * P.m_to_pix; s_py[slot * 4 + i] = v[i].y * P.m_to_pix; }
        }
    }
    if (tid == 0) {
        const double ch = srot.x, sh = srot.y;
        const double m2gx = (double)Wg / P.map_w, m2gy = (double)Hg / P.map_h;
        int cnt = 0;
        double rmin = BP_INF, rmax = -BP_INF, cmin = BP_INF, cmax = -BP_INF;
        for (int i = 0; i < P.num_ship_verts; i++) {
            const double vx = P.ship_verts[i][0] * ch + P.ship_verts[i][1] * -sh + sp.x;
            const double vy = P.ship_verts[i][0] * sh + P.ship_verts[i][1] * ch + sp.y;
            const double gx = vx * m2gx, gy = vy * m2gy;
            if (gy < 0 || gy >= Hg || gx < 0 || gx >= Wg) continue;
            s_fr[cnt] = gy; s_fc[cnt] = gx; cnt++;
            rmin = fmin(rmin, gy); rmax = fmax(rmax, gy); cmin = fmin(cmin, gx); cmax = fmax(cmax, gx);
        }
        s_fcnt = cnt;
        if (cnt > 0) {
            s_fbb[0] = max((int)(long long)fmax(0.0, rmin), gi0); s_fbb[1] = min((int)(long long)__builtin_ceil(rmax), gi1);
            s_fbb[2] = max((int)(long long)fmax(0.0, cmin), gj0); s_fbb[3] = min((int)(long long)__builtin_ceil(cmax), gj1);
        }
    }
    __syncthreads();
    const int nbox = min(s_nbox, MZ_MAXBOX);
    if (tid == 0 && s_nbox > MZ_MAXBOX) atomicOr(&D.e_err[env], BP_ERR_LEVEL_OVERFLOW);

    for (int kx = 0; kx < nbox; kx++) {
        const int r0 = s_bbx[kx][0], r1 = s_bbx[kx][1], c0 = s_bbx[kx][2], c1 = s_bbx[kx][3];
        const int wbox = c1 - c0 + 1, npx = (r1 - r0 + 1) * wbox;
        for (int q = tid; q < npx; q += OBS_THREADS) {
            const int rr = q / wbox, cc = q - rr * wbox;
            const int gi = r0 + rr, gj = c0 + cc;
            if (gi < 0 || gi >= Hg || gj < 0 || gj >= Wg) continue;
            if (pip_arrays(s_px + kx * 4, s_py + kx * 4, 4, (double)gj, (double)gi)) {
                const int bit = (gi - gi0) * IW + (gj - gj0);
                atomicOr(&s_box[bit >> 5], 1u << (bit & 31));
            }
        }
    }
    if (s_fcnt > 0) {
        const int r0 = s_fbb[0], r1 = s_fbb[1], c0 = s_fbb[2], c1 = s_fbb[3];
        const int wbox = c1 - c0 + 1, npx = (r1 >= r0 && c1 >= c0) ? (r1 - r0 + 1) * wbox : 0;
        for (int q = tid; q < npx; q += OBS_THREADS) {
            const int rr = q / wbox, cc = q - rr * wbox;
            const int gi = r0 + rr, gj = c0 + cc;
            if (gi < 0 || gi >= Hg || gj < 0 || gj >= Wg) continue;
            if (pip_arrays(s_fc, s_fr, s_fcnt, (double)gj, (double)gi)) {
                const int bit = (gi - gi0) * IW + (gj - gj0);
                atomicOr(&s_foot[bit >> 5], 1u << (bit & 31));
            }
        }
    }
    __syncthreads();
    double rs, rc;
    bp_sincos(sa - BP_PI / 2, rs, rc);
    const double ctr = ((double)IH - 1) / 2;
    const double oc0 = rc * ctr + rs * ctr, oc1 = -rs * ctr + rc * ctr;
    const double off0 = ctr - oc0, off1 = ctr - oc1;
    const int half = infl / 2;
    const size_t plane = (size_t)LH * LW;
    unsigned char *o = obs + (size_t)env * BP_OBS_C * plane;
    const int nbits = IH * IW;
    auto sample = [&](const double di, const double dj, unsigned &b0, unsigned &b1, unsigned &b2, unsigned &b3) {
        double c0 = 0.0, c1 = 0.0;
        c0 += di * rc; c0 += dj * rs; c0 += off0;
        c1 += di * -rs; c1 += dj * rc; c1 += off1;
        const bool outside = (c0 < 0 || c0 > IH - 1 || c1 < 0 || c1 > IW - 1);
        const double c0c = outside ? 0.0 : c0, c1c = outside ? 0.0 : c1;
        const double fl0 = __builtin_floor(c0c), fl1 = __builtin_floor(c1c);
        const int s0 = (int)fl0, s1 = (int)fl1;
        const double x0 = c0c - fl0, x1 = c1c - fl1;
        const double w0[2] = {1.0 - x0, x0}, w1[2] = {1.0 - x1, x1};
        double pm[4];
        unsigned wf[4], wb[4];
        bool in[4];
        int sh[4];
#pragma unroll
        for (int k = 0; k < 4; k++) {
            const int ii = s0 + (k >> 1), jj = s1 + (k & 1);
            const int gi = gi0 + ii, gj = gj0 + jj;
            in[k] = !(ii > IH - 1 || jj > IW - 1) && !(gi < 0 || gi >= Hg || gj < 0 || gj >= Wg);
            const int gic = min(max(gi, 0), Hg - 1), gjc = min(max(gj, 0), Wg - 1);
            const int bit = min(max(ii * IW + jj, 0), nbits - 1);
            sh[k] = bit & 31;
            pm[k] = *(const double *)((const char *)D.maze_obs_map + (size_t)((unsigned)(gic * Wg + gjc) * 8u));
            wf[k] = s_foot[bit >> 5]; wb[k] = s_box[bit >> 5];
        }
        double t0 = 0.0, t1 = 0.0, t2 = 0.0, t3 = 0.0;
#pragma unroll
        for (int k = 0; k < 4; k++) {
            const int a = k >> 1, b = k & 1;
            const double ww = w0[a] * w1[b];
            const bool f0 = in[k] && ((wf[k] >> sh[k]) & 1u) != 0u, f1 = in[k] && ((wb[k] >> sh[k]) & 1u) != 0u, f2 = in[k] && pm[k] < 0.0;
            const double v3 = in[k] ? __builtin_fabs(pm[k]) : 1.0;
            t0 += f0 ? ww : 0.0;
            t1 += f1 ? ww : 0.0;
            t2 += f2 ? ww : 0.0;
            double q3 = v3;
            q3 *= w0[a]; q3 *= w1[b]; t3 += q3;
        }
        if (outside) { t0 = 0.0; t1 = 0.0; t2 = 0.0; t3 = 1.0; }
        b0 = (unsigned)(unsigned char)(t0 * 255); b1 = (unsigned)(unsigned char)(t1 * 255);
        b2 = (unsigned)(unsigned char)(t2 * 255); b3 = (unsigned)(unsigned char)(t3 * 255);
    };
    if ((LW & 3) == 0) {
        unsigned *o32 = (unsigned *)o;
        const int wpr = LW / 4;
        for (int w = tid; w < LH * wpr; w += OBS_THREADS) {
            const int oi = w / wpr, oj = (w - oi * wpr) * 4;
            const double di = (double)(half + oi), dj = (double)(half + oj);
            unsigned p0 = 0, p1 = 0, p2 = 0, p3 = 0;
#pragma unroll
            for (int k = 0; k < 4; k++) {
                unsigned b0, b1, b2, b3;
                sample(di, dj + (double)k, b0, b1, b2, b3);
                p0 |= b0 << (8 * k); p1 |= b1 << (8 * k); p2 |= b2 << (8 * k); p3 |= b3 << (8 * k);
            }
            const size_t wi = (size_t)oi * wpr + (oj >> 2);
            o32[0 * (plane / 4) + wi] = p0; o32[1 * (plane / 4) + wi] = p1; o32[2 * (plane / 4) + wi] = p2; o32[3 * (plane / 4) + wi] = p3;
        }
    } else {
        for (int px = tid; px < LH * LW; px += OBS_THREADS) {
            const int oi = px / LW, oj = px - oi * LW;
            unsigned b0, b1, b2, b3;
            sample((double)(half + oi), (double)(half + oj), b0, b1, b2, b3);
            o[0 * plane + px] = (unsigned char)b0; o[1 * plane + px] = (unsigned char)b1; o[2 * plane + px] = (unsigned char)b2; o[3 * plane + px] = (unsigned char)b3;
        }
    }
}


__global__ __launch_bounds__(OBS_THREADS) void k_observe_global(const DevParams P, const DevPtrs D, const unsigned char *__restrict__ mask,
                                                                unsigned char *__restrict__ obs, const int cell_px)
{
    const int env = blockIdx.x;
    if (mask != nullptr && mask[env] == 0) return;
    const int tid = threadIdx.x;
    const int nbcap = P.nbcap;
    const size_t eb = (size_t)env * nbcap;
    const int nb = D.e_nb[env];
    const d2 *wv = D.wv + eb * BP_MAXV;
    const int *nv = D.sc_nv + (size_t)D.e_trial[env] * nbcap;
    const int bh = P.grid_h, bw = P.grid_w;
    const int Hc = bh / cell_px, Wc = bw / cell_px;
    const int nwords = (bh * bw + 31) / 32;
    extern __shared__ double2 obs_smem[];
    unsigned *s_bits = (unsigned *)obs_smem;
    __shared__ double s_x[BP_MAXV], s_y[BP_MAXV];
    __shared__ int s_box[4];
    __shared__ double s_fr[BP_MAX_SHIP_VERTS], s_fc[BP_MAX_SHIP_VERTS];
    __shared__ int s_fcnt;
    for (int w = tid; w < nwords; w += OBS_THREADS) s_bits[w] = 0u;
    __syncthreads();
    for (int s = 1; s < nb; s++) {
        const int n = nv[s];
        if (tid < n) { const d2 v = wv[(size_t)s * BP_MAXV + tid]; s_x[tid] = v.x * P.m_to_pix; s_y[tid] = v.y * P.m_to_pix; }
        __syncthreads();
        if (tid == 0) {
            double rmin = s_y[0], rmax = rmin, cmin = s_x[0], cmax = cmin;
            for (int i = 1; i < n; i++) { rmin = fmin(rmin, s_y[i]); rmax = fmax(rmax, s_y[i]); cmin = fmin(cmin, s_x[i]); cmax = fmax(cmax, s_x[i]); }
            long long minr = (long long)fmax(0.0, rmin), maxr = (long long)__builtin_ceil(rmax);
            long long minc = (long long)fmax(0.0, cmin), maxc = (long long)__builtin_ceil(cmax);
            if (maxr > bh - 1) maxr = bh - 1;
            if (maxc > bw - 1) maxc = bw - 1;
            s_box[0] = (int)minr; s_box[1] = (int)maxr; s_box[2] = (int)minc; s_box[3] = (int)maxc;
        }
        __syncthreads();
        const int r0 = s_box[0], r1 = s_box[1], c0 = s_box[2], c1 = s_box[3];
        if (r1 >= r0 && c1 >= c0) {
            const int wbox = c1 - c0 + 1, npx = (r1 - r0 + 1) * wbox;
            for (int q = tid; q < npx; q += OBS_THREADS) {
                const int rr = q / wbox, cc = q - rr * wbox;
                const int gi = r0 + rr, gj = c0 + cc;
                if (pip_arrays(s_x, s_y, n, (double)gj, (double)gi)) {
                    const int bit = gi * bw + gj;
                    atomicOr(&s_bits[bit >> 5], 1u << (bit & 31));
                }
            }
        }
        __syncthreads();
    }
    const d2 sp = D.pxy[eb];
    const d2 srot = D.rot[eb];
    if (tid == 0) {
        const double ch = srot.x, sh = srot.y;
        const double m2gx = (double)Wc / P.map_w, m2gy = (double)Hc / P.map_h;
        int cnt = 0;
        for (int i = 0; i < P.num_ship_verts; i++) {
            const double vx = P.ship_verts[i][0] * ch + P.ship_verts[i][1] * -sh + sp.x;
            const double vy = P.ship_verts[i][0] * sh + P.ship_verts[i][1] * ch + sp.y;
            const double gx = vx * m2gx, gy = vy * m2gy;
            if (gy < 0 || gy >= Hc || gx < 0 || gx >= Wc) continue;
            s_fr[cnt] = gy; s_fc[cnt] = gx; cnt++;
        }
        s_fcnt = cnt;
    }
    __syncthreads();
    const size_t plane = (size_t)Hc * Wc;
    unsigned char *o = obs + (size_t)env * 2 * plane;
    const double denom = (double)(cell_px * cell_px);
    for (int cidx = tid; cidx < Hc * Wc; cidx += OBS_THREADS) {
        const int gi = cidx / Wc, gj = cidx - gi * Wc;
        int cnt = 0;
        for (int a = 0; a < cell_px; a++)
            for (int b = 0; b < cell_px; b++) {
                const int bit = (gi * cell_px + a) * bw + (gj * cell_px + b);
                cnt += (s_bits[bit >> 5] >> (bit & 31)) & 1u;
            }
        const double mean = (double)cnt / denom;
        o[cidx] = (unsigned char)(mean * 255);
        unsigned char f = 0;
        if (s_fcnt > 0 && pip_arrays(s_fc, s_fr, s_fcnt, (double)gj, (double)gi)) f = 255;
        o[plane + cidx] = f;
    }
}

#define BP_MAX_COST 1e10
__global__ __launch_bounds__(256) void k_costmap_init(double *__restrict__ out, int E, int H, int W, int margin)
{
    const size_t total = (size_t)E * H * W;
    for (size_t i = (size_t)blockIdx.x * blockDim.x + threadIdx.x; i < total; i += (size_t)gridDim.x * blockDim.x) {
        const int j = (int)(i % W);
        out[i] = (margin && (j < margin || j >= W - margin)) ? BP_MAX_COST : 0.0;
    }
}
__global__ __launch_bounds__(256) void k_costmap(const DevParams P, const DevPtrs D, const double scale, const int H, const int W,
                                                 const double alpha, const double ship_mass, const double hz,
                                                 const double *__restrict__ ship_pos_y, const double vs, double *__restrict__ out)
{
    const int env = blockIdx.x;
    const int wave = threadIdx.x >> 6, lane = threadIdx.x & 63;
    const int s = P.nkin + blockIdx.y * 4 + wave;
    if (s >= D.e_nb[env]) return;
    __shared__ double s_c[4][BP_MAXV], s_r[4][BP_MAXV];
    const size_t eb = (size_t)env * P.nbcap;
    const int n0 = D.sc_nv[(size_t)D.e_trial[env] * P.nbcap + s];
    const double spy = ship_pos_y ? ship_pos_y[env] : 0.0;
    double ox = 0.0, oy = 0.0;
    if (lane < n0) { const d2 v = D.wv[(eb + s) * BP_MAXV + lane]; ox = v.x * scale; oy = v.y * scale; }
    if (hz != 0.0) {
        const bool inside = (lane < n0) && !(oy > (spy + hz) || oy < spy);
        if (ballot(inside) == 0ull) return;
    }
    const double rx = __builtin_rint(ox), ry = __builtin_rint(oy);
    bool dup = false;
    for (int j = 0; j < n0; j++) {
        const double jx = __shfl(rx, j), jy = __shfl(ry, j);
        if (j < lane && jx == rx && jy == ry) dup = true;
    }
    const bool keep = (lane < n0) && !dup;
    const unsigned long long km = ballot(keep);
    const int k = __popcll(km);
    if (keep) { const int pos = popc_below(km, lane); s_c[wave][pos] = ox; s_r[wave][pos] = oy; }
    lds_sync();
    const double *c = s_c[wave], *r = s_r[wave];
    double rmin = r[0], rmax = r[0], cmin = c[0], cmax = c[0];
    for (int i = 1; i < k; i++) { rmin = fmin(rmin, r[i]); rmax = fmax(rmax, r[i]); cmin = fmin(cmin, c[i]); cmax = fmax(cmax, c[i]); }
    long long minr = (long long)fmax(0.0, rmin), maxr = (long long)__builtin_ceil(rmax);
    long long minc = (long long)fmax(0.0, cmin), maxc = (long long)__builtin_ceil(cmax);
    if (maxr > H - 1) maxr = H - 1;
    if (maxc > W - 1) maxc = W - 1;
    if (maxr < minr || maxc < minc) return;
    const int wbox = (int)(maxc - minc + 1), npx = (int)(maxr - minr + 1) * wbox;
    long long cnt = 0, sr = 0, sc = 0;
    for (int q = lane; q < npx; q += 64) {
        const int rr = q / wbox, cc = q - rr * wbox;
        const long long ri = minr + rr, ci = minc + cc;
        if (pip_arrays(c, r, k, (double)ci, (double)ri)) { cnt++; sr += ri; sc += ci; }
    }
    for (int off = 32; off >= 1; off >>= 1) { cnt += __shfl_xor(cnt, off); sr += __shfl_xor(sr, off); sc += __shfl_xor(sc, off); }
    if (cnt == 0) return;
    const double cx = (double)sc / (double)cnt, cy = (double)sr / (double)cnt;
    double rad = 0.0;
    for (int i = 0; i < k; i++) {
        const double d = __builtin_sqrt((c[i] - cx) * (c[i] - cx) + (r[i] - cy) * (r[i] - cy));
        if (i == 0 || d > rad) rad = d;
    }
    double d1 = 0.0, d2_ = 0.0;
    for (int i = 0; i < k; i++) {
        const int p = (i - 1 + k) % k;
// ... 19 lines not shown
```

Baseline: 299,700.

## Compact reset mask into list and fuse step prologue kernels

On masked resets, a single-block kernel compacts the mask into a list of env indices and episodes. The reset copy and observation kernels then launch a small fixed grid that walks only the listed envs, instead of one block per env that mostly exits early. In the scheduled step path, order building, scheduler-queue init and parameter store are merged into one prologue kernel, cutting launch count. This adds a serial compaction pass and splits each env's copy work across blocks, and it depends on refactored per-env device helpers.

```diff
diff --git a/benchpush_amd/csrc/bp_capi.hip b/benchpush_amd/csrc/bp_capi.hip
--- a/benchpush_amd/csrc/bp_capi.hip
+++ b/benchpush_amd/csrc/bp_capi.hip
@@ -46,6 +46,9 @@
     int num_trials = 0;
     bool loaded = false, was_reset = false;
     int *order_buf = nullptr;
+    int *reset_list = nullptr;
+    int *reset_cnt = nullptr;
+    int reset_grid = 0;
     bool steps_done = false;
     bool resettle = false;
     bool damp = false;
@@ -567,6 +570,22 @@
     else { k.step = k_physics_step; k.sched = k_physics_step_sched; k.resident = h->P.pair_mode == 2 ? k_physics_step_schedr : k_physics_step_schedl; k.reset = k_physics_reset; }
     return k;
 }
+static int reset_list_setup(bp_handle *h)
+{
+    int rc;
+    if (getenv("BP_RESET_LIST") && atoi(getenv("BP_RESET_LIST")) == 0) return BP_OK;
+    if ((rc = device_cus(h))) return rc;
+    int g = 4 * h->num_cus;
+    if (const char *ev = getenv("BP_RESET_GRID")) g = atoi(ev);
+    h->reset_grid = std::max(1, std::min(g, h->num_envs));
+    if ((rc = dalloc(h, &h->reset_list, (size_t)2 * h->num_envs))) return rc;
+    if ((rc = dalloc(h, &h->reset_cnt, (size_t)1))) return rc;
+    if (h->P.env_kind == BP_ENV_MAZE)
+        HIPCHK(h, hipFuncSetAttribute((const void *)k_observe_maze_list, hipFuncAttributeMaxDynamicSharedMemorySize, (int)h->obs_lds_bytes));
+    else
+        HIPCHK(h, hipFuncSetAttribute((const void *)k_observe_list, hipFuncAttributeMaxDynamicSharedMemorySize, (int)h->obs_lds_bytes));
+    return BP_OK;
+}
 static int settle_templates(bp_handle *h)
 {
     hipLaunchKernelGGL(h->k.reset, dim3(h->num_trials), dim3(64), h->lds_bytes, 0, h->P, h->D, (const unsigned char *)nullptr, (double *)nullptr, 1);
@@ -616,6 +635,7 @@
         HIPCHK(h, hipFuncSetAttribute((const void *)k_physics_reset_maze, hipFuncAttributeMaxDynamicSharedMemorySize, (int)h->lds_bytes));
     }
     h->k = rigid_kernels(h, maze8);
+    if ((rc = reset_list_setup(h))) return rc;
     return settle_templates(h);
 }
 
@@ -962,26 +982,34 @@
 {
     unsigned char *obs = out.obs, *term = out.term, *trunc = out.trunc;
     double *reward = out.reward, *info = out.info;
+    const bool by_list = mode == MODE_RESET && mask != nullptr && !h->resettle && h->reset_grid > 0;
+    if (by_list && (physics || (raster && obs))) {
+        hipLaunchKernelGGL(k_reset_list, dim3(1), dim3(1024), 0, st, mask, h->num_envs, (const int *)h->D.e_episode, h->reset_list, h->num_envs, h->reset_cnt);
+        HIPCHK(h, hipGetLastError());
+    }
     if (physics) {
-        if (mode == MODE_STEP && h->steps_done) {
-            hipLaunchKernelGGL(k_make_order, dim3(1), dim3(1024), 0, st, (const unsigned *)h->D.e_cost, h->order_buf, h->num_envs, h->D.sq_thr);
-            HIPCHK(h, hipGetLastError());
+        const bool scheduled = mode == MODE_STEP && !(h->pair_mode == 1 && h->D.dbg == nullptr) && h->sched_chunk > 0 && h->D.dbg == nullptr;
+        const bool with_order = mode == MODE_STEP && h->steps_done;
+        if (with_order) {
+            if (!scheduled) {
+                hipLaunchKernelGGL(k_make_order, dim3(1), dim3(1024), 0, st, (const unsigned *)h->D.e_cost, h->order_buf, h->num_envs, h->D.sq_thr);
+                HIPCHK(h, hipGetLastError());
+            }
             h->D.order = h->order_buf;
         }
         if (mode == MODE_STEP) h->steps_done = true;
         if (mode == MODE_STEP && h->pair_mode == 1 && h->D.dbg == nullptr)
             hipLaunchKernelGGL(k_physics_step_pair, dim3((h->num_envs + 1) / 2), dim3(64), 2 * PL_HALF, st, h->P, h->D, actions, reward, term, trunc, info);
-        else if (mode == MODE_STEP && h->sched_chunk > 0 && h->D.dbg == nullptr) {
-            hipLaunchKernelGGL(k_sched_init, dim3(16), dim3(1024), 0, st, h->P, h->D);
-            HIPCHK(h, hipGetLastError());
+        else if (scheduled) {
             if (h->resident_auto && (++h->launches & 63u) == 0) h->device_shared = resident_device_shared(h);
             const bool resident_ok = !(h->resident_auto && h->device_shared);
             const int resident = !resident_ok ? 0 : h->P.pair_mode == 2 ? h->pair_resident : h->sched_persist;
+            DevParams *Pg = resident > 0 ? (DevParams *)h->pd_buf : nullptr;
+            DevPtrs *Dg = resident > 0 ? (DevPtrs *)((char *)h->pd_buf + sizeof(DevParams)) : nullptr;
+            hipLaunchKernelGGL(k_step_prologue, dim3((with_order ? 1 : 0) + SQ_INIT_BLOCKS + (resident > 0 ? 1 : 0)), dim3(1024), 0, st, h->P, h->D, Pg, Dg,
+                               with_order ? 1 : 0, (const unsigned *)h->D.e_cost, h->order_buf, h->D.sq_thr);
+            HIPCHK(h, hipGetLastError());
             if (resident > 0) {
-                DevParams *Pg = (DevParams *)h->pd_buf;
-                DevPtrs *Dg = (DevPtrs *)((char *)h->pd_buf + sizeof(DevParams));
-                hipLaunchKernelGGL(k_store_params, dim3(1), dim3(64), 0, st, h->P, h->D, Pg, Dg);
-                HIPCHK(h, hipGetLastError());
                 hipLaunchKernelGGL(h->k.resident, dim3(resident), dim3(64), h->sched_lds, st, Pg, Dg, actions, reward, term, trunc, info);
             } else if (h->P.pair_mode == 2) {
                 if (!h->st_aux) {
@@ -1019,6 +1047,8 @@
             hipLaunchKernelGGL(h->k.step, dim3(h->num_envs), dim3(64), h->lds_bytes, st, h->P, h->D, actions, reward, term, trunc, info);
         else if (h->resettle)
             hipLaunchKernelGGL(h->k.reset, dim3(h->num_envs), dim3(64), h->lds_bytes, st, h->P, h->D, mask, info, 0);
+        else if (by_list)
+            hipLaunchKernelGGL(k_reset_copy_list, dim3(h->reset_grid), dim3(256), 0, st, h->P, h->D, (const int *)h->reset_list, (const int *)h->reset_cnt, info);
         else
             hipLaunchKernelGGL(k_reset_copy, dim3(h->num_envs), dim3(256), 0, st, h->P, h->D, mask, info);
         HIPCHK(h, hipGetLastError());
@@ -1031,7 +1061,15 @@
         HIPCHK(h, hipGetLastError());
     }
     if (h->timing) HIPCHK(h, hipEventRecord(e1, st));
-    if (raster && obs) {
+    if (raster && obs && by_list) {
+        if (h->P.env_kind == BP_ENV_MAZE)
+            hipLaunchKernelGGL(k_observe_maze_list, dim3(h->reset_grid), dim3(OBS_THREADS), h->obs_lds_bytes, st, h->P, h->D, (const int *)h->reset_list,
+                               (const int *)h->reset_cnt, obs);
+        else
+            hipLaunchKernelGGL(k_observe_list, dim3(h->reset_grid), dim3(OBS_THREADS_SHIP), h->obs_lds_bytes, st, h->P, h->D, (const int *)h->reset_list,
+                               (const int *)h->reset_cnt, obs);
+        HIPCHK(h, hipGetLastError());
+    } else if (raster && obs) {
         if (h->P.env_kind == BP_ENV_MAZE)
             hipLaunchKernelGGL(k_observe_maze, dim3(h->num_envs), dim3(OBS_THREADS), h->obs_lds_bytes, st, h->P, h->D, mask, obs);
         else
diff --git a/benchpush_amd/csrc/bp_kernels.hpp b/benchpush_amd/csrc/bp_kernels.hpp
--- a/benchpush_amd/csrc/bp_kernels.hpp
+++ b/benchpush_amd/csrc/bp_kernels.hpp
@@ -788,9 +788,10 @@
     int it, score, heavy;
     pair_task<false>(P, D, actions, reward, terminated, truncated, info, e0, e1, Q, it, score, heavy, [](const int) { return false; });
 }
-__global__ void k_sched_init(const DevParams P, const DevPtrs D)
-{
-    const int tid = blockIdx.x * blockDim.x + threadIdx.x, nthr = gridDim.x * blockDim.x;
+#define SQ_INIT_BLOCKS 16
+__device__ __forceinline__ void sched_init_body(const DevParams &P, const DevPtrs &D, const int bid, const int nblk)
+{
+    const int tid = bid * blockDim.x + threadIdx.x, nthr = nblk * blockDim.x;
     const int nrows = P.sq_lrpt ? SQ_MAXLEV : P.sq_levels;
     for (int i = tid; i < SQ_NX * nrows * P.sq_cap; i += nthr) {
         const int xk = i / (nrows * P.sq_cap), r = i - xk * (nrows * P.sq_cap);
@@ -1099,7 +1100,7 @@
 {
     sched_resident_pairing<0>(Pg, Dg, actions, reward, terminated, truncated, info);
 }
-__global__ void k_store_params(const DevParams P, const DevPtrs D, DevParams *Pg, DevPtrs *Dg)
+__device__ __forceinline__ void store_params_body(const DevParams &P, const DevPtrs &D, DevParams *Pg, DevPtrs *Dg)
 {
     static_assert(sizeof(DevParams) % 4 == 0 && sizeof(DevPtrs) % 4 == 0, "copied as 32-bit words");
     const unsigned *sp = (const unsigned *)&P, *sd = (const unsigned *)&D;
@@ -1162,7 +1163,7 @@
     physics_body<MODE_RESET, BP_ENV_BOX, false, true>(P, D, nullptr, mask, nullptr, nullptr, nullptr, tmpl ? nullptr : info, tmpl);
 }
 
-__global__ __launch_bounds__(1024) void k_make_order(const unsigned *__restrict__ cost, int *__restrict__ order, int n, unsigned *__restrict__ thr)
+__device__ __forceinline__ void make_order_body(const unsigned *__restrict__ cost, int *__restrict__ order, int n, unsigned *__restrict__ thr)
 {
     __shared__ unsigned hist[257];
     __shared__ unsigned smax;
@@ -1194,6 +1195,18 @@
         order[pos] = i;
     }
 }
+__global__ __launch_bounds__(1024) void k_make_order(const unsigned *__restrict__ cost, int *__restrict__ order, int n, unsigned *__restrict__ thr)
+{
+    make_order_body(cost, order, n, thr);
+}
+__global__ __launch_bounds__(1024) void k_step_prologue(const DevParams P, const DevPtrs D, DevParams *Pg, DevPtrs *Dg, const int with_order,
+                                                        const unsigned *__restrict__ cost, int *__restrict__ order, unsigned *__restrict__ thr)
+{
+    const int b = (int)blockIdx.x - with_order;
+    if (b < 0) make_order_body(cost, order, P.num_envs, thr);
+    else if (b < SQ_INIT_BLOCKS) sched_init_body(P, D, b, SQ_INIT_BLOCKS);
+    else store_params_body(P, D, Pg, Dg);
+}
 
 
 __global__ __launch_bounds__(1024) void k_cost_stats(const unsigned *__restrict__ cost, int n, unsigned long long *__restrict__ ring, int slot)
@@ -1216,13 +1229,9 @@
 {
     for (size_t i = tid; i < n; i += nt) dst[i] = src[i];
 }
-__global__ __launch_bounds__(256) void k_reset_copy(const DevParams P, const DevPtrs D, const unsigned char *__restrict__ mask,
-                                                    double *__restrict__ info)
-{
-    const int env = blockIdx.x;
-    if (mask != nullptr && mask[env] == 0) return;
-    const int tid = threadIdx.x, nt = blockDim.x;
-    const int episode = D.e_episode[env] + 1;
+__device__ __forceinline__ void reset_copy_env(const DevParams &P, const DevPtrs &D, const int env, const int episode, double *__restrict__ info,
+                                               const int tid, const int nt)
+{
     const int trial = (int)(((long long)P.env_offset + env + episode) % P.num_trials);
     const size_t nb = P.nbcap, d = (size_t)env * nb, s = (size_t)(P.num_envs + trial) * nb;
     copy_span(D.pxy + d, D.pxy + s, nb, tid, nt);
@@ -1263,6 +1272,46 @@
         }
     }
 }
+__global__ __launch_bounds__(256) void k_reset_copy(const DevParams P, const DevPtrs D, const unsigned char *__restrict__ mask,
+                                                    double *__restrict__ info)
+{
+    const int env = blockIdx.x;
+    if (mask != nullptr && mask[env] == 0) return;
+    reset_copy_env(P, D, env, D.e_episode[env] + 1, info, threadIdx.x, blockDim.x);
+}
+__global__ __launch_bounds__(1024) void k_reset_list(const unsigned char *__restrict__ mask, const int n, const int *__restrict__ e_episode, int *__restrict__ list,
+                                                     const int cap, int *__restrict__ cnt)
+{
+    __shared__ int s_w[2][16];
+    const int tid = threadIdx.x, wave = tid >> 6, lane = tid & 63;
+    int base = 0;
+    for (int c0 = 0, buf = 0; c0 < n; c0 += 1024, buf ^= 1) {
+        const int i = c0 + tid;
+        const bool f = i < n && mask[i] != 0;
+        const unsigned long long b = __ballot(f);
+        if (lane == 0) s_w[buf][wave] = __popcll(b);
+        __syncthreads();
+        int before = 0, total = 0;
+        for (int w = 0; w < 16; w++) { const int c = s_w[buf][w]; before += (w < wave) ? c : 0; total += c; }
+        if (f) {
+            const int pos = base + before + __popcll(b & ((1ull << lane) - 1ull));
+            list[pos] = i; list[cap + pos] = e_episode[i] + 1;
+        }
+        base += total;
+    }
+    if (tid == 0) cnt[0] = base;
+}
+#define RESET_COPY_PARTS 16
+__global__ __launch_bounds__(256) void k_reset_copy_list(const DevParams P, const DevPtrs D, const int *__restrict__ list, const int *__restrict__ cnt,
+                                                         double *__restrict__ info)
+{
+    const int n = min(cnt[0], P.num_envs);
+    const int parts = max(1, min(RESET_COPY_PARTS, (int)gridDim.x / max(n, 1)));
+    for (int w = blockIdx.x; w < n * parts; w += gridDim.x) {
+        const int pos = w / parts, part = w - pos * parts;
+        reset_copy_env(P, D, list[pos], list[P.num_envs + pos], info, part * (int)blockDim.x + (int)threadIdx.x, parts * (int)blockDim.x);
+    }
+}
 
 #define OBS_THREADS 256
 #ifndef OBS_THREADS_SHIP
@@ -1460,221 +1509,17 @@
 {
     const int env = blockIdx.x;
     if (mask != nullptr && mask[env] == 0) return;
-    const int tid = threadIdx.x;
-    const int nbcap = P.nbcap;
-    const size_t eb = (size_t)env * nbcap;
-    const int nb = D.e_nb[env];
-    const d2 *wv = D.wv + eb * BP_MAXV;
-    const int *nv = D.sc_nv + (size_t)D.e_trial[env] * nbcap;
-    const int Hg = P.grid_h, Wg = P.grid_w, LH = P.obs_h, LW = P.obs_w;
-    const int npix = LH * LW;
-
-    extern __shared__ double2 obs_smem[];
-    unsigned char *s_img = (unsigned char *)obs_smem;
-    unsigned char *s_edt = s_img + ((npix + 15) & ~15);
-    double *s_px = (double *)(s_edt + ((LH + 15) & ~15));
-    double *s_py = s_px + OBS_CHUNK * BP_MAXV;
-    __shared__ int s_npass;
-    __shared__ unsigned short s_list[OBS_MAXCAND];
-    __shared__ int s_bbx[OBS_CHUNK][4];
-    __shared__ unsigned char s_cn[OBS_CHUNK];
-    __shared__ double s_fr[BP_MAX_SHIP_VERTS], s_fc[BP_MAX_SHIP_VERTS];
-    __shared__ int s_fcnt, s_fbb[4];
-    OPROF(0)
-    const double4 bb_first = D.bb[eb + min(1 + tid, nbcap - 1)];
-    if (tid == 0) s_npass = 0;
-    for (int w = tid; w < (npix + 3) / 4; w += OBS_THREADS_SHIP) ((unsigned *)s_img)[w] = 0u;
-    __syncthreads();
-    OPROF(1)
-
-    const d2 sp = D.pxy[eb];
-    const d2 srot = D.rot[eb];
-    const double m2gx = (double)Wg / P.map_w, m2gy = (double)Hg / P.map_h;
-    const int wx = (int)(sp.x * m2gx);
-    const int wy = (int)((sp.y + P.vshift) * m2gy);
-    const int gi0 = (int)((double)(0 + wy) - ((double)LH / 2)), gj0 = (int)((double)(0 + wx) - ((double)LW / 2));
-    const int gi1 = gi0 + LH - 1, gj1 = gj0 + LW - 1;
-    const int bh = (int)(P.map_h * P.m_to_pix), bw = (int)(P.map_w * P.m_to_pix);
-    for (int s = 1 + tid; s < nb; s += OBS_THREADS_SHIP) {
-        const double4 b = (s == 1 + tid) ? bb_first : D.bb[eb + s];
-        if (__builtin_floor(b.y * P.m_to_pix) - 1.0 > (double)gi1 || __builtin_ceil(b.w * P.m_to_pix) + 1.0 < (double)gi0 ||
-            __builtin_floor(b.x * P.m_to_pix) - 1.0 > (double)gj1 || __builtin_ceil(b.z * P.m_to_pix) + 1.0 < (double)gj0) continue;
-        const int slot = atomicAdd(&s_npass, 1);
-        if (slot < OBS_MAXCAND) s_list[slot] = (unsigned short)s;
-    }
-    LineSpec line;
-    long long hpx, hpy;
-    {
-        const double ch = srot.x, sh = srot.y;
-        if (tid == 0) {
-            int cnt = 0;
-            double rmin = BP_INF, rmax = -BP_INF, cmin = BP_INF, cmax = -BP_INF;
-            for (int i = 0; i < P.num_ship_verts; i++) {
-                const double vx = P.ship_verts[i][0] * ch + P.ship_verts[i][1] * -sh + sp.x;
-                const double vy = P.ship_verts[i][0] * sh + P.ship_verts[i][1] * ch + sp.y;
-                const double gx = vx * m2gx, gy = vy * m2gy;
-                if (gy < 0 || gy >= Hg || gx < 0 || gx >= Wg) continue;
-                s_fr[cnt] = gy; s_fc[cnt] = gx; cnt++;
-                rmin = fmin(rmin, gy); rmax = fmax(rmax, gy); cmin = fmin(cmin, gx); cmax = fmax(cmax, gx);
-            }
-            s_fcnt = cnt;
-            if (cnt > 0) {
-                s_fbb[0] = (int)(long long)fmax(0.0, rmin); s_fbb[1] = (int)(long long)__builtin_ceil(rmax);
-                s_fbb[2] = (int)(long long)fmax(0.0, cmin); s_fbb[3] = (int)(long long)__builtin_ceil(cmax);
-            }
-        }
-        line.valid = 0; hpx = hpy = 0;
-        if (tid >= 64 && tid < 128) {
-            const double hx = P.ship_head[0] * ch + P.ship_head[1] * -sh + sp.x, hy = P.ship_head[0] * sh + P.ship_head[1] * ch + sp.y;
-            const double tx = P.ship_tail[0] * ch + P.ship_tail[1] * -sh + sp.x, ty = P.ship_tail[0] * sh + P.ship_tail[1] * ch + sp.y;
-            hpx = to_u16(hx * m2gx); hpy = to_u16(hy * m2gy);
-            const long long tpx = to_u16(tx * m2gx), tpy = to_u16(ty * m2gy);
-            line = make_line(Wg, Hg, hpx, hpy, tpx, tpy);
-            hpx = hpx < 0 ? 0 : (hpx > Wg - 1 ? Wg - 1 : hpx);
-            hpy = hpy < 0 ? 0 : (hpy > Hg - 1 ? Hg - 1 : hpy);
-        }
-    }
-    const double g2m = P.map_h / (double)Hg;
-    for (int li = tid; li < LH; li += OBS_THREADS_SHIP) {
-        const int gi = gi0 + li;
-        unsigned char e = 255;
-        if (gi >= 0 && gi < Hg) {
-            double dd = P.goal_y - gi * g2m;
-            if (dd < 0) dd = 0;
-            e = (unsigned char)((dd / P.goal_y) * 255);
-        }
-        s_edt[li] = e;
-    }
-    __syncthreads();
-    OPROF(2)
-    const int ncand_all = min(s_npass, OBS_MAXCAND);
-    if (tid == 0 && s_npass > OBS_MAXCAND) atomicOr(&D.e_err[env], BP_ERR_LEVEL_OVERFLOW);
-    for (int cbase = 0; cbase < ncand_all; cbase += OBS_CHUNK) {
-    const int ncand = min(OBS_CHUNK, ncand_all - cbase);
-    for (int idx = tid; idx < ncand * BP_MAXV; idx += OBS_THREADS_SHIP) {
-        const int k = idx / BP_MAXV, q = idx - k * BP_MAXV;
-        const int s = s_list[cbase + k];
-        const d2 v = wv[(size_t)s * BP_MAXV + q];
-        const int n = nv[s];
-        if (q == 0) s_cn[k] = (unsigned char)n;
-        if (q < n) { s_px[idx] = v.x; s_py[idx] = v.y; }
-    }
-    __syncthreads();
-    OPROF(3)
-    if (tid < ncand) {
-        const int k = tid;
-        const int n = s_cn[k];
-        double *xp = s_px + k * BP_MAXV, *yp = s_py + k * BP_MAXV;
-        bool keep = true;
-        double d1 = 0.0, d2_ = 0.0, sx = 0.0, sy = 0.0;
-        double rmin = BP_INF, rmax = -BP_INF, cmin = BP_INF, cmax = -BP_INF;
-        double xq = xp[n - 1], yq = yp[n - 1];
-        for (int i = 0; i < n; i++) {
-            const double xi = xp[i], yi = yp[i];
-            const double a = xi * yq, b = yi * xq;
-            d1 += a; d2_ += b;
-            const double u = a - xq * yi;
-            sx += (xi + xq) * u;
-            sy += (yi + yq) * u;
-            const double r = yi * P.m_to_pix, cc = xi * P.m_to_pix;
-            xp[i] = cc; yp[i] = r;
-            rmin = fmin(rmin, r); rmax = fmax(rmax, r); cmin = fmin(cmin, cc); cmax = fmax(cmax, cc);
-            xq = xi; yq = yi;
-        }
-        {
-            const double A = 0.5 * __builtin_fabs(d1 - d2_);
-            const double f = 1.0 / (6.0 * A);
-            const double cx = __builtin_fabs(__builtin_fabs(f * sx)), cy = __builtin_fabs(__builtin_fabs(f * sy));
-            if (__builtin_fabs(sp.x - cx) > P.obs_range || __builtin_fabs(sp.y - cy) > P.obs_range) keep = false;
-        }
-        long long minr = (long long)fmax(0.0, rmin), maxr = (long long)__builtin_ceil(rmax);
-        long long minc = (long long)fmax(0.0, cmin), maxc = (long long)__builtin_ceil(cmax);
-        if (maxr > bh - 1) maxr = bh - 1;
-        if (maxc > bw - 1) maxc = bw - 1;
-        if (maxr < gi0 || minr > gi1 || maxc < gj0 || minc > gj1 || maxr < minr || maxc < minc) keep = false;
-        if (keep) {
-            s_bbx[k][0] = (int)max(minr, (long long)gi0); s_bbx[k][1] = (int)min(maxr, (long long)gi1);
-            s_bbx[k][2] = (int)max(minc, (long long)gj0); s_bbx[k][3] = (int)min(maxc, (long long)gj1);
-        } else { s_bbx[k][0] = 0; s_bbx[k][1] = -1; s_bbx[k][2] = 0; s_bbx[k][3] = -1; }
-    }
-    __syncthreads();
-    OPROF(4)
-    {
-        int TPC = OBS_THREADS_SHIP / OBS_CHUNK;
-        while (TPC * ncand * 2 <= OBS_THREADS_SHIP) TPC *= 2;
-        const int k = tid / TPC, sub = tid - k * TPC;
-        if (k < ncand && s_bbx[k][1] >= s_bbx[k][0]) {
-            const int c0 = max(s_bbx[k][2], 0), c1 = min(s_bbx[k][3], Wg - 1);
-            const int n = s_cn[k];
-            const double *xp = s_px + k * BP_MAXV, *yp = s_py + k * BP_MAXV;
-            for (int gi = s_bbx[k][0] + sub; gi <= s_bbx[k][1]; gi += TPC) {
-                if (gi < 0 || gi >= Hg) continue;
-                raster_row_convex<false>(xp, yp, n, gi, c0, c1, s_img + (gi - gi0) * LW - gj0, (unsigned char)OBS_F_OCC);
-            }
-        }
-    }
-    __syncthreads();
-    }
-    OPROF(5)
-    if (tid < 64) {
-        if (s_fcnt > 0) {
-            const int r0 = max(s_fbb[0], max(gi0, 0)), r1 = min(s_fbb[1], min(gi1, Hg - 1));
-            const int c0 = max(s_fbb[2], max(gj0, 0)), c1 = min(s_fbb[3], min(gj1, Wg - 1));
-            if (c1 >= c0)
-                for (int gi = r0 + tid; gi <= r1; gi += 64)
-                    raster_row_convex<true>(s_fc, s_fr, s_fcnt, gi, c0, c1, s_img, (unsigned char)OBS_F_SHIP, (gi - gi0) * LW - gj0);
-        }
-    } else if (tid < 128) {
-        const int l2 = tid - 64;
-        if (line.valid) {
-            const long long dmaj = line.vert ? line.dy : line.dx, dmin = line.vert ? line.dx : line.dy;
-            for (long long t = l2; t <= dmaj; t += 64) {
-                const long long mt = (dmaj == 0) ? 0 : ((dmaj < 32768 && dmin < 32768)
-                                         ? (long long)(((unsigned)(2 * dmin * t) + (unsigned)dmaj - 1u) / (unsigned)(2 * dmaj))
-                                         : (2 * dmin * t + dmaj - 1) / (2 * dmaj));
-                const long long ax = line.vert ? mt : t, ay = line.vert ? t : mt;
-                const long long gj = line.x0 + ax * line.sx, gi = line.y0 + ay * line.sy;
-                if (gi >= gi0 && gi <= gi1 && gj >= gj0 && gj <= gj1 && gi >= 0 && gi < Hg && gj >= 0 && gj < Wg) {
-                    const int b = ((int)gi - gi0) * LW + ((int)gj - gj0);
-                    obs_or_bytes((unsigned *)s_img, b, b, (unsigned char)OBS_F_LINE);
-                }
-            }
-        }
-        if (l2 == 0 && hpy >= gi0 && hpy <= gi1 && hpx >= gj0 && hpx <= gj1) {
-            const int b = ((int)hpy - gi0) * LW + ((int)hpx - gj0);
-            obs_or_bytes((unsigned *)s_img, b, b, (unsigned char)OBS_F_HEAD);
-        }
-    }
-    __syncthreads();
-    OPROF(6)
-    const size_t plane = (size_t)npix;
-    unsigned *o32 = (unsigned *)(obs + (size_t)env * BP_OBS_C * plane);
-    const int nwords = npix / 4;
-    const int WP = LW / 2, G = OBS_THREADS_SHIP / WP;
-    const int g = tid / WP, j = tid - g * WP;
-    const int ljlo = max(0, -gj0), ljhi = min(LW - 1, Wg - 1 - gj0);
-    if (g < G) {
-        const int bs = LW - 4 * j;
-        const unsigned mlo = obs_upto(bs);
-        const unsigned mA = mlo & obs_upto(ljhi - 4 * j + 1) & ~obs_upto(ljlo - 4 * j);
-        const unsigned mB = ~mlo & obs_upto(bs + ljhi + 1) & ~obs_upto(bs + ljlo);
-        for (int rp = g; 2 * rp < LH; rp += G) {
-            const int w = rp * WP + j;
-            const unsigned f = ((const unsigned *)s_img)[w];
-            const int giA = gi0 + 2 * rp, giB = giA + 1;
-            const unsigned rowA = (giA >= 0 && giA < Hg) ? 0xFFFFFFFFu : 0u, rowB = (giB >= 0 && giB < Hg) ? 0xFFFFFFFFu : 0u;
-            const unsigned inb = (rowA & mA) | (rowB & mB);
-            const unsigned e2 = ((const unsigned short *)s_edt)[rp];
-            const unsigned eA = (e2 & 0xFFu) * 0x01010101u, eB = (e2 >> 8) * 0x01010101u;
-            const unsigned e = ((eA & mlo) | (eB & ~mlo)) & inb;
-            const unsigned ship = (f >> 1) & 0x01010101u, ln = (f >> 2) & 0x01010101u, hd = (f >> 3) & 0x01010101u;
-            o32[w] = inb & (0x7F7F7F7Fu + ship * 0x80u);
-            o32[nwords + w] = e | ~inb;
-            o32[2 * nwords + w] = inb & ((ln & ~hd) * 127u + hd * 255u);
-            o32[3 * nwords + w] = (f & 0x01010101u) * 255u;
-        }
-    }
-    OPROF(7)
+#include "bp_observe_body.hpp"
+}
+__global__ __launch_bounds__(OBS_THREADS_SHIP, 4) void k_observe_list(const DevParams P, const DevPtrs D, const int *__restrict__ rlist,
+                                                              const int *__restrict__ rcnt, unsigned char *__restrict__ obs)
+{
+    const int rn = min(rcnt[0], P.num_envs);
+    for (int ri = blockIdx.x; ri < rn; ri += gridDim.x) {
+        const int env = rlist[ri];
+#include "bp_observe_body.hpp"
+        __syncthreads();
+    }
 }
 
 #define MZ_MAXBOX 64
@@ -1683,183 +1528,16 @@
 {
     const int env = blockIdx.x;
     if (mask != nullptr && mask[env] == 0) return;
-    const int tid = threadIdx.x;
-    const int nbcap = P.nbcap;
-    const size_t eb = (size_t)env * nbcap;
-    const int nb = D.e_nb[env];
-    const size_t tb = (size_t)D.e_trial[env] * nbcap;
-    const d2 *wv = D.wv + eb * BP_MAXV;
-    const int *nv = D.sc_nv + tb;
-    const int *kind = D.sc_kind + tb;
-    const int Hg = P.grid_h, Wg = P.grid_w, LH = P.obs_h, LW = P.obs_w;
-    const int infl = (LW > LH ? LW : LH) / 2;
-    const int IH = LH + infl, IW = LW + infl;
-    const int nwords = (IH * IW + 31) / 32;
-
-    extern __shared__ double2 obs_smem[];
-    unsigned *s_box = (unsigned *)obs_smem;
-    unsigned *s_foot = s_box + nwords;
-    double *s_px = (double *)(s_foot + ((nwords + 1) & ~1));
-    double *s_py = s_px + MZ_MAXBOX * 4;
-    __shared__ int s_nbox;
-    __shared__ int s_bbx[MZ_MAXBOX][4];
-    __shared__ double s_fr[BP_MAX_SHIP_VERTS], s_fc[BP_MAX_SHIP_VERTS];
-    __shared__ int s_fcnt, s_fbb[4];
-    if (tid == 0) s_nbox = 0;
-    for (int w = tid; w < nwords; w += OBS_THREADS) { s_box[w] = 0u; s_foot[w] = 0u; }
-    __syncthreads();
-
-    const d2 sp = D.pxy[eb];
-    const double sa = D.ang[eb];
-    const d2 srot = D.rot[eb];
-    const int wx = (int)(sp.x * P.m_to_pix), wy = (int)(sp.y * P.m_to_pix);
-    const int gi0 = (int)((double)(0 + wy) - ((double)IH / 2)), gj0 = (int)((double)(0 + wx) - ((double)IW / 2));
-    const int gi1 = gi0 + IH - 1, gj1 = gj0 + IW - 1;
-    for (int s = tid; s < nb; s += OBS_THREADS) {
-        if (kind_ctype(kind[s]) != 2) continue;
-        const int n = nv[s];
-        const d2 *v = wv + (size_t)s * BP_MAXV;
-        double rmin = v[0].y * P.m_to_pix, rmax = rmin, cmin = v[0].x * P.m_to_pix, cmax = cmin;
-        for (int i = 1; i < n; i++) {
-            const double r = v[i].y * P.m_to_pix, cc = v[i].x * P.m_to_pix;
-            rmin = fmin(rmin, r); rmax = fmax(rmax, r); cmin = fmin(cmin, cc); cmax = fmax(cmax, cc);
-        }
-        long long minr = (long long)fmax(0.0, rmin), maxr = (long long)__builtin_ceil(rmax);
-        long long minc = (long long)fmax(0.0, cmin), maxc = (long long)__builtin_ceil(cmax);
-        if (maxr > Hg - 1) maxr = Hg - 1;
-        if (maxc > Wg - 1) maxc = Wg - 1;
-        if (maxr < gi0 || minr > gi1 || maxc < gj0 || minc > gj1 || maxr < minr || maxc < minc) continue;
-        const int slot = atomicAdd(&s_nbox, 1);
-        if (slot < MZ_MAXBOX && n <= 4) {
-            s_bbx[slot][0] = (int)max(minr, (long long)gi0); s_bbx[slot][1] = (int)min(maxr, (long long)gi1);
-            s_bbx[slot][2] = (int)max(minc, (long long)gj0); s_bbx[slot][3] = (int)min(maxc, (long long)gj1);
-            for (int i = 0; i < 4; i++) { s_px[slot * 4 + i] = v[i].x * P.m_to_pix; s_py[slot * 4 + i] = v[i].y * P.m_to_pix; }
-        }
-    }
-    if (tid == 0) {
-        const double ch = srot.x, sh = srot.y;
-        const double m2gx = (double)Wg / P.map_w, m2gy = (double)Hg / P.map_h;
-        int cnt = 0;
-        double rmin = BP_INF, rmax = -BP_INF, cmin = BP_INF, cmax = -BP_INF;
-        for (int i = 0; i < P.num_ship_verts; i++) {
-            const double vx = P.ship_verts[i][0] * ch + P.ship_verts[i][1] * -sh + sp.x;
-            const double vy = P.ship_verts[i][0] * sh + P.ship_verts[i][1] * ch + sp.y;
-            const double gx = vx * m2gx, gy = vy * m2gy;
-            if (gy < 0 || gy >= Hg || gx < 0 || gx >= Wg) continue;
-            s_fr[cnt] = gy; s_fc[cnt] = gx; cnt++;
-            rmin = fmin(rmin, gy); rmax = fmax(rmax, gy); cmin = fmin(cmin, gx); cmax = fmax(cmax, gx);
-        }
-        s_fcnt = cnt;
-        if (cnt > 0) {
-            s_fbb[0] = max((int)(long long)fmax(0.0, rmin), gi0); s_fbb[1] = min((int)(long long)__builtin_ceil(rmax), gi1);
-            s_fbb[2] = max((int)(long long)fmax(0.0, cmin), gj0); s_fbb[3] = min((int)(long long)__builtin_ceil(cmax), gj1);
-        }
-    }
-    __syncthreads();
-    const int nbox = min(s_nbox, MZ_MAXBOX);
-    if (tid == 0 && s_nbox > MZ_MAXBOX) atomicOr(&D.e_err[env], BP_ERR_LEVEL_OVERFLOW);
-
-    for (int kx = 0; kx < nbox; kx++) {
-        const int r0 = s_bbx[kx][0], r1 = s_bbx[kx][1], c0 = s_bbx[kx][2], c1 = s_bbx[kx][3];
-        const int wbox = c1 - c0 + 1, npx = (r1 - r0 + 1) * wbox;
-        for (int q = tid; q < npx; q += OBS_THREADS) {
-            const int rr = q / wbox, cc = q - rr * wbox;
-            const int gi = r0 + rr, gj = c0 + cc;
-            if (gi < 0 || gi >= Hg || gj < 0 || gj >= Wg) continue;
-            if (pip_arrays(s_px + kx * 4, s_py + kx * 4, 4, (double)gj, (double)gi)) {
-                const int bit = (gi - gi0) * IW + (gj - gj0);
-                atomicOr(&s_box[bit >> 5], 1u << (bit & 31));
-            }
-        }
-    }
-    if (s_fcnt > 0) {
-        const int r0 = s_fbb[0], r1 = s_fbb[1], c0 = s_fbb[2], c1 = s_fbb[3];
-        const int wbox = c1 - c0 + 1, npx = (r1 >= r0 && c1 >= c0) ? (r1 - r0 + 1) * wbox : 0;
-        for (int q = tid; q < npx; q += OBS_THREADS) {
-            const int rr = q / wbox, cc = q - rr * wbox;
-            const int gi = r0 + rr, gj = c0 + cc;
-            if (gi < 0 || gi >= Hg || gj < 0 || gj >= Wg) continue;
-            if (pip_arrays(s_fc, s_fr, s_fcnt, (double)gj, (double)gi)) {
-                const int bit = (gi - gi0) * IW + (gj - gj0);
-                atomicOr(&s_foot[bit >> 5], 1u << (bit & 31));
-            }
-        }
-    }
-    __syncthreads();
-    double rs, rc;
-    bp_sincos(sa - BP_PI / 2, rs, rc);
-    const double ctr = ((double)IH - 1) / 2;
-    const double oc0 = rc * ctr + rs * ctr, oc1 = -rs * ctr + rc * ctr;
-    const double off0 = ctr - oc0, off1 = ctr - oc1;
-    const int half = infl / 2;
-    const size_t plane = (size_t)LH * LW;
-    unsigned char *o = obs + (size_t)env * BP_OBS_C * plane;
-    const int nbits = IH * IW;
-    auto sample = [&](const double di, const double dj, unsigned &b0, unsigned &b1, unsigned &b2, unsigned &b3) {
-        double c0 = 0.0, c1 = 0.0;
-        c0 += di * rc; c0 += dj * rs; c0 += off0;
-        c1 += di * -rs; c1 += dj * rc; c1 += off1;
-        const bool outside = (c0 < 0 || c0 > IH - 1 || c1 < 0 || c1 > IW - 1);
-        const double c0c = outside ? 0.0 : c0, c1c = outside ? 0.0 : c1;
-        const double fl0 = __builtin_floor(c0c), fl1 = __builtin_floor(c1c);
-        const int s0 = (int)fl0, s1 = (int)fl1;
-        const double x0 = c0c - fl0, x1 = c1c - fl1;
-        const double w0[2] = {1.0 - x0, x0}, w1[2] = {1.0 - x1, x1};
-        double pm[4];
-        unsigned wf[4], wb[4];
-        bool in[4];
-        int sh[4];
-#pragma unroll
-        for (int k = 0; k < 4; k++) {
-            const int ii = s0 + (k >> 1), jj = s1 + (k & 1);
-            const int gi = gi0 + ii, gj = gj0 + jj;
-            in[k] = !(ii > IH - 1 || jj > IW - 1) && !(gi < 0 || gi >= Hg || gj < 0 || gj >= Wg);
-            const int gic = min(max(gi, 0), Hg - 1), gjc = min(max(gj, 0), Wg - 1);
-            const int bit = min(max(ii * IW + jj, 0), nbits - 1);
-            sh[k] = bit & 31;
-            pm[k] = *(const double *)((const char *)D.maze_obs_map + (size_t)((unsigned)(gic * Wg + gjc) * 8u));
-            wf[k] = s_foot[bit >> 5]; wb[k] = s_box[bit >> 5];
-        }
-        double t0 = 0.0, t1 = 0.0, t2 = 0.0, t3 = 0.0;
-#pragma unroll
-        for (int k = 0; k < 4; k++) {
-            const int a = k >> 1, b = k & 1;
-            const double ww = w0[a] * w1[b];
-            const bool f0 = in[k] && ((wf[k] >> sh[k]) & 1u) != 0u, f1 = in[k] && ((wb[k] >> sh[k]) & 1u) != 0u, f2 = in[k] && pm[k] < 0.0;
-            const double v3 = in[k] ? __builtin_fabs(pm[k]) : 1.0;
-            t0 += f0 ? ww : 0.0;
-            t1 += f1 ? ww : 0.0;
-            t2 += f2 ? ww : 0.0;
-            double q3 = v3;
-            q3 *= w0[a]; q3 *= w1[b]; t3 += q3;
-        }
-        if (outside) { t0 = 0.0; t1 = 0.0; t2 = 0.0; t3 = 1.0; }
-        b0 = (unsigned)(unsigned char)(t0 * 255); b1 = (unsigned)(unsigned char)(t1 * 255);
-        b2 = (unsigned)(unsigned char)(t2 * 255); b3 = (unsigned)(unsigned char)(t3 * 255);
-    };
-    if ((LW & 3) == 0) {
-        unsigned *o32 = (unsigned *)o;
-        const int wpr = LW / 4;
-        for (int w = tid; w < LH * wpr; w += OBS_THREADS) {
-            const int oi = w / wpr, oj = (w - oi * wpr) * 4;
-            const double di = (double)(half + oi), dj = (double)(half + oj);
-            unsigned p0 = 0, p1 = 0, p2 = 0, p3 = 0;
-#pragma unroll
-            for (int k = 0; k < 4; k++) {
-                unsigned b0, b1, b2, b3;
-                sample(di, dj + (double)k, b0, b1, b2, b3);
-                p0 |= b0 << (8 * k); p1 |= b1 << (8 * k); p2 |= b2 << (8 * k); p3 |= b3 << (8 * k);
-            }
-            const size_t wi = (size_t)oi * wpr + (oj >> 2);
-            o32[0 * (plane / 4) + wi] = p0; o32[1 * (plane / 4) + wi] = p1; o32[2 * (plane / 4) + wi] = p2; o32[3 * (plane / 4) + wi] = p3;
-        }
-    } else {
-        for (int px = tid; px < LH * LW; px += OBS_THREADS) {
-            const int oi = px / LW, oj = px - oi * LW;
-            unsigned b0, b1, b2, b3;
-            sample((double)(half + oi), (double)(half + oj), b0, b1, b2, b3);
-            o[0 * plane + px] = (unsigned char)b0; o[1 * plane + px] = (unsigned char)b1; o[2 * plane + px] = (unsigned char)b2; o[3 * plane + px] = (unsigned char)b3;
-        }
+#include "bp_observe_maze_body.hpp"
+}
+__global__ __launch_bounds__(OBS_THREADS) void k_observe_maze_list(const DevParams P, const DevPtrs D, const int *__restrict__ rlist,
+                                                                   const int *__restrict__ rcnt, unsigned char *__restrict__ obs)
+{
+    const int rn = min(rcnt[0], P.num_envs);
+    for (int ri = blockIdx.x; ri < rn; ri += gridDim.x) {
+        const int env = rlist[ri];
+#include "bp_observe_maze_body.hpp"
+        __syncthreads();
     }
 }
 
diff --git a/benchpush_amd/csrc/bp_observe_body.hpp b/benchpush_amd/csrc/bp_observe_body.hpp
--- /dev/null
+++ b/benchpush_amd/csrc/bp_observe_body.hpp
@@ -0,0 +1,215 @@
+    const int tid = threadIdx.x;
+    const int nbcap = P.nbcap;
+    const size_t eb = (size_t)env * nbcap;
+    const int nb = D.e_nb[env];
+    const d2 *wv = D.wv + eb * BP_MAXV;
+    const int *nv = D.sc_nv + (size_t)D.e_trial[env] * nbcap;
+    const int Hg = P.grid_h, Wg = P.grid_w, LH = P.obs_h, LW = P.obs_w;
+    const int npix = LH * LW;
+
+    extern __shared__ double2 obs_smem[];
+    unsigned char *s_img = (unsigned char *)obs_smem;
+    unsigned char *s_edt = s_img + ((npix + 15) & ~15);
+    double *s_px = (double *)(s_edt + ((LH + 15) & ~15));
+    double *s_py = s_px + OBS_CHUNK * BP_MAXV;
+    __shared__ int s_npass;
+    __shared__ unsigned short s_list[OBS_MAXCAND];
+    __shared__ int s_bbx[OBS_CHUNK][4];
+    __shared__ unsigned char s_cn[OBS_CHUNK];
+    __shared__ double s_fr[BP_MAX_SHIP_VERTS], s_fc[BP_MAX_SHIP_VERTS];
+    __shared__ int s_fcnt, s_fbb[4];
+    OPROF(0)
+    const double4 bb_first = D.bb[eb + min(1 + tid, nbcap - 1)];
+    if (tid == 0) s_npass = 0;
+    for (int w = tid; w < (npix + 3) / 4; w += OBS_THREADS_SHIP) ((unsigned *)s_img)[w] = 0u;
+    __syncthreads();
+    OPROF(1)
+
+    const d2 sp = D.pxy[eb];
+    const d2 srot = D.rot[eb];
+    const double m2gx = (double)Wg / P.map_w, m2gy = (double)Hg / P.map_h;
+    const int wx = (int)(sp.x * m2gx);
+    const int wy = (int)((sp.y + P.vshift) * m2gy);
+    const int gi0 = (int)((double)(0 + wy) - ((double)LH / 2)), gj0 = (int)((double)(0 + wx) - ((double)LW / 2));
+    const int gi1 = gi0 + LH - 1, gj1 = gj0 + LW - 1;
+    const int bh = (int)(P.map_h * P.m_to_pix), bw = (int)(P.map_w * P.m_to_pix);
+    for (int s = 1 + tid; s < nb; s += OBS_THREADS_SHIP) {
+        const double4 b = (s == 1 + tid) ? bb_first : D.bb[eb + s];
+        if (__builtin_floor(b.y * P.m_to_pix) - 1.0 > (double)gi1 || __builtin_ceil(b.w * P.m_to_pix) + 1.0 < (double)gi0 ||
+            __builtin_floor(b.x * P.m_to_pix) - 1.0 > (double)gj1 || __builtin_ceil(b.z * P.m_to_pix) + 1.0 < (double)gj0) continue;
+        const int slot = atomicAdd(&s_npass, 1);
+        if (slot < OBS_MAXCAND) s_list[slot] = (unsigned short)s;
+    }
+    LineSpec line;
+    long long hpx, hpy;
+    {
+        const double ch = srot.x, sh = srot.y;
+        if (tid == 0) {
+            int cnt = 0;
+            double rmin = BP_INF, rmax = -BP_INF, cmin = BP_INF, cmax = -BP_INF;
+            for (int i = 0; i < P.num_ship_verts; i++) {
+                const double vx = P.ship_verts[i][0] * ch + P.ship_verts[i][1] * -sh + sp.x;
+                const double vy = P.ship_verts[i][0] * sh + P.ship_verts[i][1] * ch + sp.y;
+                const double gx = vx * m2gx, gy = vy * m2gy;
+                if (gy < 0 || gy >= Hg || gx < 0 || gx >= Wg) continue;
+                s_fr[cnt] = gy; s_fc[cnt] = gx; cnt++;
+                rmin = fmin(rmin, gy); rmax = fmax(rmax, gy); cmin = fmin(cmin, gx); cmax = fmax(cmax, gx);
+            }
+            s_fcnt = cnt;
+            if (cnt > 0) {
+                s_fbb[0] = (int)(long long)fmax(0.0, rmin); s_fbb[1] = (int)(long long)__builtin_ceil(rmax);
+                s_fbb[2] = (int)(long long)fmax(0.0, cmin); s_fbb[3] = (int)(long long)__builtin_ceil(cmax);
+            }
+        }
+        line.valid = 0; hpx = hpy = 0;
+        if (tid >= 64 && tid < 128) {
+            const double hx = P.ship_head[0] * ch + P.ship_head[1] * -sh + sp.x, hy = P.ship_head[0] * sh + P.ship_head[1] * ch + sp.y;
+            const double tx = P.ship_tail[0] * ch + P.ship_tail[1] * -sh + sp.x, ty = P.ship_tail[0] * sh + P.ship_tail[1] * ch + sp.y;
+            hpx = to_u16(hx * m2gx); hpy = to_u16(hy * m2gy);
+            const long long tpx = to_u16(tx * m2gx), tpy = to_u16(ty * m2gy);
+            line = make_line(Wg, Hg, hpx, hpy, tpx, tpy);
+            hpx = hpx < 0 ? 0 : (hpx > Wg - 1 ? Wg - 1 : hpx);
+            hpy = hpy < 0 ? 0 : (hpy > Hg - 1 ? Hg - 1 : hpy);
+        }
+    }
+    const double g2m = P.map_h / (double)Hg;
+    for (int li = tid; li < LH; li += OBS_THREADS_SHIP) {
+        const int gi = gi0 + li;
+        unsigned char e = 255;
+        if (gi >= 0 && gi < Hg) {
+            double dd = P.goal_y - gi * g2m;
+            if (dd < 0) dd = 0;
+            e = (unsigned char)((dd / P.goal_y) * 255);
+        }
+        s_edt[li] = e;
+    }
+    __syncthreads();
+    OPROF(2)
+    const int ncand_all = min(s_npass, OBS_MAXCAND);
+    if (tid == 0 && s_npass > OBS_MAXCAND) atomicOr(&D.e_err[env], BP_ERR_LEVEL_OVERFLOW);
+    for (int cbase = 0; cbase < ncand_all; cbase += OBS_CHUNK) {
+    const int ncand = min(OBS_CHUNK, ncand_all - cbase);
+    for (int idx = tid; idx < ncand * BP_MAXV; idx += OBS_THREADS_SHIP) {
+        const int k = idx / BP_MAXV, q = idx - k * BP_MAXV;
+        const int s = s_list[cbase + k];
+        const d2 v = wv[(size_t)s * BP_MAXV + q];
+        const int n = nv[s];
+        if (q == 0) s_cn[k] = (unsigned char)n;
+        if (q < n) { s_px[idx] = v.x; s_py[idx] = v.y; }
+    }
+    __syncthreads();
+    OPROF(3)
+    if (tid < ncand) {
+        const int k = tid;
+        const int n = s_cn[k];
+        double *xp = s_px + k * BP_MAXV, *yp = s_py + k * BP_MAXV;
+        bool keep = true;
+        double d1 = 0.0, d2_ = 0.0, sx = 0.0, sy = 0.0;
+        double rmin = BP_INF, rmax = -BP_INF, cmin = BP_INF, cmax = -BP_INF;
+        double xq = xp[n - 1], yq = yp[n - 1];
+        for (int i = 0; i < n; i++) {
+            const double xi = xp[i], yi = yp[i];
+            const double a = xi * yq, b = yi * xq;
+            d1 += a; d2_ += b;
+            const double u = a - xq * yi;
+            sx += (xi + xq) * u;
+            sy += (yi + yq) * u;
+            const double r = yi * P.m_to_pix, cc = xi * P.m_to_pix;
+            xp[i] = cc; yp[i] = r;
+            rmin = fmin(rmin, r); rmax = fmax(rmax, r); cmin = fmin(cmin, cc); cmax = fmax(cmax, cc);
+            xq = xi; yq = yi;
+        }
+        {
+            const double A = 0.5 * __builtin_fabs(d1 - d2_);
+            const double f = 1.0 / (6.0 * A);
+            const double cx = __builtin_fabs(__builtin_fabs(f * sx)), cy = __builtin_fabs(__builtin_fabs(f * sy));
+            if (__builtin_fabs(sp.x - cx) > P.obs_range || __builtin_fabs(sp.y - cy) > P.obs_range) keep = false;
+        }
+        long long minr = (long long)fmax(0.0, rmin), maxr = (long long)__builtin_ceil(rmax);
+        long long minc = (long long)fmax(0.0, cmin), maxc = (long long)__builtin_ceil(cmax);
+        if (maxr > bh - 1) maxr = bh - 1;
+        if (maxc > bw - 1) maxc = bw - 1;
+        if (maxr < gi0 || minr > gi1 || maxc < gj0 || minc > gj1 || maxr < minr || maxc < minc) keep = false;
+        if (keep) {
+            s_bbx[k][0] = (int)max(minr, (long long)gi0); s_bbx[k][1] = (int)min(maxr, (long long)gi1);
+            s_bbx[k][2] = (int)max(minc, (long long)gj0); s_bbx[k][3] = (int)min(maxc, (long long)gj1);
+        } else { s_bbx[k][0] = 0; s_bbx[k][1] = -1; s_bbx[k][2] = 0; s_bbx[k][3] = -1; }
+    }
+    __syncthreads();
+    OPROF(4)
+    {
+        int TPC = OBS_THREADS_SHIP / OBS_CHUNK;
+        while (TPC * ncand * 2 <= OBS_THREADS_SHIP) TPC *= 2;
+        const int k = tid / TPC, sub = tid - k * TPC;
+        if (k < ncand && s_bbx[k][1] >= s_bbx[k][0]) {
+            const int c0 = max(s_bbx[k][2], 0), c1 = min(s_bbx[k][3], Wg - 1);
+            const int n = s_cn[k];
+            const double *xp = s_px + k * BP_MAXV, *yp = s_py + k * BP_MAXV;
+            for (int gi = s_bbx[k][0] + sub; gi <= s_bbx[k][1]; gi += TPC) {
+                if (gi < 0 || gi >= Hg) continue;
+                raster_row_convex<false>(xp, yp, n, gi, c0, c1, s_img + (gi - gi0) * LW - gj0, (unsigned char)OBS_F_OCC);
+            }
+        }
+    }
+    __syncthreads();
+    }
+    OPROF(5)
+    if (tid < 64) {
+        if (s_fcnt > 0) {
+            const int r0 = max(s_fbb[0], max(gi0, 0)), r1 = min(s_fbb[1], min(gi1, Hg - 1));
+            const int c0 = max(s_fbb[2], max(gj0, 0)), c1 = min(s_fbb[3], min(gj1, Wg - 1));
+            if (c1 >= c0)
+                for (int gi = r0 + tid; gi <= r1; gi += 64)
+                    raster_row_convex<true>(s_fc, s_fr, s_fcnt, gi, c0, c1, s_img, (unsigned char)OBS_F_SHIP, (gi - gi0) * LW - gj0);
+        }
+    } else if (tid < 128) {
+        const int l2 = tid - 64;
+        if (line.valid) {
+            const long long dmaj = line.vert ? line.dy : line.dx, dmin = line.vert ? line.dx : line.dy;
+            for (long long t = l2; t <= dmaj; t += 64) {
+                const long long mt = (dmaj == 0) ? 0 : ((dmaj < 32768 && dmin < 32768)
+                                         ? (long long)(((unsigned)(2 * dmin * t) + (unsigned)dmaj - 1u) / (unsigned)(2 * dmaj))
+                                         : (2 * dmin * t + dmaj - 1) / (2 * dmaj));
+                const long long ax = line.vert ? mt : t, ay = line.vert ? t : mt;
+                const long long gj = line.x0 + ax * line.sx, gi = line.y0 + ay * line.sy;
+                if (gi >= gi0 && gi <= gi1 && gj >= gj0 && gj <= gj1 && gi >= 0 && gi < Hg && gj >= 0 && gj < Wg) {
+                    const int b = ((int)gi - gi0) * LW + ((int)gj - gj0);
+                    obs_or_bytes((unsigned *)s_img, b, b, (unsigned char)OBS_F_LINE);
+                }
+            }
+        }
+        if (l2 == 0 && hpy >= gi0 && hpy <= gi1 && hpx >= gj0 && hpx <= gj1) {
+            const int b = ((int)hpy - gi0) * LW + ((int)hpx - gj0);
+            obs_or_bytes((unsigned *)s_img, b, b, (unsigned char)OBS_F_HEAD);
+        }
+    }
+    __syncthreads();
+    OPROF(6)
+    const size_t plane = (size_t)npix;
+    unsigned *o32 = (unsigned *)(obs + (size_t)env * BP_OBS_C * plane);
+    const int nwords = npix / 4;
+    const int WP = LW / 2, G = OBS_THREADS_SHIP / WP;
+    const int g = tid / WP, j = tid - g * WP;
+    const int ljlo = max(0, -gj0), ljhi = min(LW - 1, Wg - 1 - gj0);
+    if (g < G) {
+        const int bs = LW - 4 * j;
+        const unsigned mlo = obs_upto(bs);
+        const unsigned mA = mlo & obs_upto(ljhi - 4 * j + 1) & ~obs_upto(ljlo - 4 * j);
+        const unsigned mB = ~mlo & obs_upto(bs + ljhi + 1) & ~obs_upto(bs + ljlo);
+        for (int rp = g; 2 * rp < LH; rp += G) {
+            const int w = rp * WP + j;
+            const unsigned f = ((const unsigned *)s_img)[w];
+            const int giA = gi0 + 2 * rp, giB = giA + 1;
+            const unsigned rowA = (giA >= 0 && giA < Hg) ? 0xFFFFFFFFu : 0u, rowB = (giB >= 0 && giB < Hg) ? 0xFFFFFFFFu : 0u;
+            const unsigned inb = (rowA & mA) | (rowB & mB);
+            const unsigned e2 = ((const unsigned short *)s_edt)[rp];
+            const unsigned eA = (e2 & 0xFFu) * 0x01010101u, eB = (e2 >> 8) * 0x01010101u;
+            const unsigned e = ((eA & mlo) | (eB & ~mlo)) & inb;
+            const unsigned ship = (f >> 1) & 0x01010101u, ln = (f >> 2) & 0x01010101u, hd = (f >> 3) & 0x01010101u;
+            o32[w] = inb & (0x7F7F7F7Fu + ship * 0x80u);
+            o32[nwords + w] = e | ~inb;
+            o32[2 * nwords + w] = inb & ((ln & ~hd) * 127u + hd * 255u);
+            o32[3 * nwords + w] = (f & 0x01010101u) * 255u;
+        }
+    }
+    OPROF(7)
diff --git a/benchpush_amd/csrc/bp_observe_maze_body.hpp b/benchpush_amd/csrc/bp_observe_maze_body.hpp
--- /dev/null
+++ b/benchpush_amd/csrc/bp_observe_maze_body.hpp
@@ -0,0 +1,178 @@
+    const int tid = threadIdx.x;
+    const int nbcap = P.nbcap;
+    const size_t eb = (size_t)env * nbcap;
+    const int nb = D.e_nb[env];
+    const size_t tb = (size_t)D.e_trial[env] * nbcap;
+    const d2 *wv = D.wv + eb * BP_MAXV;
+    const int *nv = D.sc_nv + tb;
+    const int *kind = D.sc_kind + tb;
+    const int Hg = P.grid_h, Wg = P.grid_w, LH = P.obs_h, LW = P.obs_w;
+    const int infl = (LW > LH ? LW : LH) / 2;
+    const int IH = LH + infl, IW = LW + infl;
+    const int nwords = (IH * IW + 31) / 32;
+
+    extern __shared__ double2 obs_smem[];
+    unsigned *s_box = (unsigned *)obs_smem;
+    unsigned *s_foot = s_box + nwords;
+    double *s_px = (double *)(s_foot + ((nwords + 1) & ~1));
+    double *s_py = s_px + MZ_MAXBOX * 4;
+    __shared__ int s_nbox;
+    __shared__ int s_bbx[MZ_MAXBOX][4];
+    __shared__ double s_fr[BP_MAX_SHIP_VERTS], s_fc[BP_MAX_SHIP_VERTS];
+    __shared__ int s_fcnt, s_fbb[4];
+    if (tid == 0) s_nbox = 0;
+    for (int w = tid; w < nwords; w += OBS_THREADS) { s_box[w] = 0u; s_foot[w] = 0u; }
+    __syncthreads();
+
+    const d2 sp = D.pxy[eb];
+    const double sa = D.ang[eb];
+    const d2 srot = D.rot[eb];
+    const int wx = (int)(sp.x * P.m_to_pix), wy = (int)(sp.y * P.m_to_pix);
+    const int gi0 = (int)((double)(0 + wy) - ((double)IH / 2)), gj0 = (int)((double)(0 + wx) - ((double)IW / 2));
+    const int gi1 = gi0 + IH - 1, gj1 = gj0 + IW - 1;
+    for (int s = tid; s < nb; s += OBS_THREADS) {
+        if (kind_ctype(kind[s]) != 2) continue;
+        const int n = nv[s];
+        const d2 *v = wv + (size_t)s * BP_MAXV;
+        double rmin = v[0].y * P.m_to_pix, rmax = rmin, cmin = v[0].x * P.m_to_pix, cmax = cmin;
+        for (int i = 1; i < n; i++) {
+            const double r = v[i].y * P.m_to_pix, cc = v[i].x * P.m_to_pix;
+            rmin = fmin(rmin, r); rmax = fmax(rmax, r); cmin = fmin(cmin, cc); cmax = fmax(cmax, cc);
+        }
+        long long minr = (long long)fmax(0.0, rmin), maxr = (long long)__builtin_ceil(rmax);
+        long long minc = (long long)fmax(0.0, cmin), maxc = (long long)__builtin_ceil(cmax);
+        if (maxr > Hg - 1) maxr = Hg - 1;
+        if (maxc > Wg - 1) maxc = Wg - 1;
+        if (maxr < gi0 || minr > gi1 || maxc < gj0 || minc > gj1 || maxr < minr || maxc < minc) continue;
+        const int slot = atomicAdd(&s_nbox, 1);
+        if (slot < MZ_MAXBOX && n <= 4) {
+            s_bbx[slot][0] = (int)max(minr, (long long)gi0); s_bbx[slot][1] = (int)min(maxr, (long long)gi1);
+            s_bbx[slot][2] = (int)max(minc, (long long)gj0); s_bbx[slot][3] = (int)min(maxc, (long long)gj1);
+            for (int i = 0; i < 4; i++) { s_px[slot * 4 + i] = v[i].x * P.m_to_pix; s_py[slot * 4 + i] = v[i].y * P.m_to_pix; }
+        }
+    }
+    if (tid == 0) {
+        const double ch = srot.x, sh = srot.y;
+        const double m2gx = (double)Wg / P.map_w, m2gy = (double)Hg / P.map_h;
+        int cnt = 0;
+        double rmin = BP_INF, rmax = -BP_INF, cmin = BP_INF, cmax = -BP_INF;
+        for (int i = 0; i < P.num_ship_verts; i++) {
+            const double vx = P.ship_verts[i][0] * ch + P.ship_verts[i][1] * -sh + sp.x;
+            const double vy = P.ship_verts[i][0] * sh + P.ship_verts[i][1] * ch + sp.y;
+            const double gx = vx * m2gx, gy = vy * m2gy;
+            if (gy < 0 || gy >= Hg || gx < 0 || gx >= Wg) continue;
+            s_fr[cnt] = gy; s_fc[cnt] = gx; cnt++;
+            rmin = fmin(rmin, gy); rmax = fmax(rmax, gy); cmin = fmin(cmin, gx); cmax = fmax(cmax, gx);
+        }
+        s_fcnt = cnt;
+        if (cnt > 0) {
+            s_fbb[0] = max((int)(long long)fmax(0.0, rmin), gi0); s_fbb[1] = min((int)(long long)__builtin_ceil(rmax), gi1);
+            s_fbb[2] = max((int)(long long)fmax(0.0, cmin), gj0); s_fbb[3] = min((int)(long long)__builtin_ceil(cmax), gj1);
+        }
+    }
+    __syncthreads();
+    const int nbox = min(s_nbox, MZ_MAXBOX);
+    if (tid == 0 && s_nbox > MZ_MAXBOX) atomicOr(&D.e_err[env], BP_ERR_LEVEL_OVERFLOW);
+
+    for (int kx = 0; kx < nbox; kx++) {
+        const int r0 = s_bbx[kx][0], r1 = s_bbx[kx][1], c0 = s_bbx[kx][2], c1 = s_bbx[kx][3];
+        const int wbox = c1 - c0 + 1, npx = (r1 - r0 + 1) * wbox;
+        for (int q = tid; q < npx; q += OBS_THREADS) {
+            const int rr = q / wbox, cc = q - rr * wbox;
+            const int gi = r0 + rr, gj = c0 + cc;
+            if (gi < 0 || gi >= Hg || gj < 0 || gj >= Wg) continue;
+            if (pip_arrays(s_px + kx * 4, s_py + kx * 4, 4, (double)gj, (double)gi)) {
+                const int bit = (gi - gi0) * IW + (gj - gj0);
+                atomicOr(&s_box[bit >> 5], 1u << (bit & 31));
+            }
+        }
+    }
+    if (s_fcnt > 0) {
+        const int r0 = s_fbb[0], r1 = s_fbb[1], c0 = s_fbb[2], c1 = s_fbb[3];
+        const int wbox = c1 - c0 + 1, npx = (r1 >= r0 && c1 >= c0) ? (r1 - r0 + 1) * wbox : 0;
+        for (int q = tid; q < npx; q += OBS_THREADS) {
+            const int rr = q / wbox, cc = q - rr * wbox;
+            const int gi = r0 + rr, gj = c0 + cc;
+            if (gi < 0 || gi >= Hg || gj < 0 || gj >= Wg) continue;
+            if (pip_arrays(s_fc, s_fr, s_fcnt, (double)gj, (double)gi)) {
+                const int bit = (gi - gi0) * IW + (gj - gj0);
+                atomicOr(&s_foot[bit >> 5], 1u << (bit & 31));
+            }
+        }
+    }
+    __syncthreads();
+    double rs, rc;
+    bp_sincos(sa - BP_PI / 2, rs, rc);
+    const double ctr = ((double)IH - 1) / 2;
+    const double oc0 = rc * ctr + rs * ctr, oc1 = -rs * ctr + rc * ctr;
+    const double off0 = ctr - oc0, off1 = ctr - oc1;
+    const int half = infl / 2;
+    const size_t plane = (size_t)LH * LW;
+    unsigned char *o = obs + (size_t)env * BP_OBS_C * plane;
+    const int nbits = IH * IW;
+    auto sample = [&](const double di, const double dj, unsigned &b0, unsigned &b1, unsigned &b2, unsigned &b3) {
+        double c0 = 0.0, c1 = 0.0;
+        c0 += di * rc; c0 += dj * rs; c0 += off0;
+        c1 += di * -rs; c1 += dj * rc; c1 += off1;
+        const bool outside = (c0 < 0 || c0 > IH - 1 || c1 < 0 || c1 > IW - 1);
+        const double c0c = outside ? 0.0 : c0, c1c = outside ? 0.0 : c1;
+        const double fl0 = __builtin_floor(c0c), fl1 = __builtin_floor(c1c);
+        const int s0 = (int)fl0, s1 = (int)fl1;
+        const double x0 = c0c - fl0, x1 = c1c - fl1;
+        const double w0[2] = {1.0 - x0, x0}, w1[2] = {1.0 - x1, x1};
+        double pm[4];
+        unsigned wf[4], wb[4];
+        bool in[4];
+        int sh[4];
+#pragma unroll
+        for (int k = 0; k < 4; k++) {
+            const int ii = s0 + (k >> 1), jj = s1 + (k & 1);
+            const int gi = gi0 + ii, gj = gj0 + jj;
+            in[k] = !(ii > IH - 1 || jj > IW - 1) && !(gi < 0 || gi >= Hg || gj < 0 || gj >= Wg);
+            const int gic = min(max(gi, 0), Hg - 1), gjc = min(max(gj, 0), Wg - 1);
+            const int bit = min(max(ii * IW + jj, 0), nbits - 1);
+            sh[k] = bit & 31;
+            pm[k] = *(const double *)((const char *)D.maze_obs_map + (size_t)((unsigned)(gic * Wg + gjc) * 8u));
+            wf[k] = s_foot[bit >> 5]; wb[k] = s_box[bit >> 5];
+        }
+        double t0 = 0.0, t1 = 0.0, t2 = 0.0, t3 = 0.0;
+#pragma unroll
+        for (int k = 0; k < 4; k++) {
+            const int a = k >> 1, b = k & 1;
+            const double ww = w0[a] * w1[b];
+            const bool f0 = in[k] && ((wf[k] >> sh[k]) & 1u) != 0u, f1 = in[k] && ((wb[k] >> sh[k]) & 1u) != 0u, f2 = in[k] && pm[k] < 0.0;
+            const double v3 = in[k] ? __builtin_fabs(pm[k]) : 1.0;
+            t0 += f0 ? ww : 0.0;
+            t1 += f1 ? ww : 0.0;
+            t2 += f2 ? ww : 0.0;
+            double q3 = v3;
+            q3 *= w0[a]; q3 *= w1[b]; t3 += q3;
+        }
+        if (outside) { t0 = 0.0; t1 = 0.0; t2 = 0.0; t3 = 1.0; }
+        b0 = (unsigned)(unsigned char)(t0 * 255); b1 = (unsigned)(unsigned char)(t1 * 255);
+        b2 = (unsigned)(unsigned char)(t2 * 255); b3 = (unsigned)(unsigned char)(t3 * 255);
+    };
+    if ((LW & 3) == 0) {
+        unsigned *o32 = (unsigned *)o;
+        const int wpr = LW / 4;
+        for (int w = tid; w < LH * wpr; w += OBS_THREADS) {
+            const int oi = w / wpr, oj = (w - oi * wpr) * 4;
+            const double di = (double)(half + oi), dj = (double)(half + oj);
+            unsigned p0 = 0, p1 = 0, p2 = 0, p3 = 0;
+#pragma unroll
+            for (int k = 0; k < 4; k++) {
+                unsigned b0, b1, b2, b3;
+                sample(di, dj + (double)k, b0, b1, b2, b3);
+                p0 |= b0 << (8 * k); p1 |= b1 << (8 * k); p2 |= b2 << (8 * k); p3 |= b3 << (8 * k);
+            }
+            const size_t wi = (size_t)oi * wpr + (oj >> 2);
+            o32[0 * (plane / 4) + wi] = p0; o32[1 * (plane / 4) + wi] = p1; o32[2 * (plane / 4) + wi] = p2; o32[3 * (plane / 4) + wi] = p3;
+        }
+    } else {
+        for (int px = tid; px < LH * LW; px += OBS_THREADS) {
+            const int oi = px / LW, oj = px - oi * LW;
+            unsigned b0, b1, b2, b3;
+            sample((double)(half + oi), (double)(half + oj), b0, b1, b2, b3);
+            o[0 * plane + px] = (unsigned char)b0; o[1 * plane + px] = (unsigned char)b1; o[2 * plane + px] = (unsigned char)b2; o[3 * plane + px] = (unsigned char)b3;
+        }
+    }
```

Result: no change. 300,600, median of 3 (+0.3%).
